# sxyu/volrend

Measured on AMD Instinct MI355X. Metric: Mrays/s at 800x800, NeRF-synthetic-like SH16 (synthetic C1), higher is better.
Workload: dtype f32; 1 GPU; C1: synthetic lego-like PlenOctree, depth 9, SH16, 2025715 nodes, 2.24 GB in HBM, 800x800, fx=fy=1111.111, 200-pose orbit, default RenderOptions; fp_mode=strict, launches=38, pcie_inclusive=False, launch_streams=1, parallelism=single GPU

## Files before the change

include/volrend_hip.h:

```cpp
#ifndef VOLREND_HIP_H_
#define VOLREND_HIP_H_

#include <stddef.h>
#include <stdint.h>

#ifdef __cplusplus
extern "C" {
#endif

#define VR_ABI_VERSION 3

enum {
    VR_OK = 0,
    VR_ERR_INVALID_ARGUMENT = 1,
    VR_ERR_HIP = 2,
    VR_ERR_NO_DEVICE = 3,
    VR_ERR_BAD_TREE = 4,
    VR_ERR_UNSUPPORTED = 5,
    VR_ERR_OUT_OF_MEMORY = 6
};

enum { VR_FORMAT_RGBA = 0, VR_FORMAT_SH = 1, VR_FORMAT_SG = 2, VR_FORMAT_ASG = 3 };

enum { VR_FP_STRICT = 0, VR_FP_FMA = 1 };

#define VR_MAX_BASIS 25

typedef struct VrTreeOpaque* vr_tree_t;

typedef struct VrTreeDesc {
    const int32_t* child;
    const uint16_t* data;
    const float* extra;
    uint64_t extra_count;
    float offset[3];
    float scale[3];
    int32_t N;
    int64_t capacity;
    int32_t data_dim;
    int32_t format;
    int32_t basis_dim;
    float ndc_width;
    float ndc_height;
    float ndc_focal;
    int32_t memory;
} VrTreeDesc;

typedef struct VrQuantDesc {
    const uint16_t* quant_colors;
    const uint16_t* quant_map;
    const uint16_t* sigma;
    const uint16_t* data_retained;
    int32_t n_quant;
    int32_t n_retained;
} VrQuantDesc;

typedef struct VrTreeInfo {
    int64_t capacity;
    int32_t N, data_dim, format, basis_dim;
    int32_t max_depth;
    int32_t device;
    uint64_t device_bytes;
    uint64_t leaf_stride;
    int32_t query_mode;
    int32_t top_levels;
    int32_t brick_levels;
    int32_t brick_blocked;
} VrTreeInfo;

#define VR_QUERY_LOOKUP 0
#define VR_QUERY_DESCENT 1
int vr_query_mode_for(int N, int max_depth, int64_t capacity);

typedef struct VrCamera {
    float transform[12];
    int32_t width, height;
    float fx, fy;
} VrCamera;

typedef struct VrRenderOptions {
    float step_size;
    float sigma_thresh;
    float stop_thresh;
    float background_brightness;
    float render_bbox[6];
    int32_t basis_minmax[2];
    float rot_dirs[3];
    int32_t show_grid;
    int32_t grid_max_depth;
    int32_t render_depth;
    int32_t enable_probe;
    float probe[3];
    int32_t probe_disp_size;
} VrRenderOptions;

enum { VR_LAYOUT_FRAME = 0, VR_LAYOUT_COMPACT = 1 };

typedef struct VrFrame {
    void* rgba;
    int64_t pitch;
    const float* depth;
    float* accum;
    int32_t offscreen;
    int32_t layout;
    int32_t tile_w, tile_h;
    int32_t rank, world;
    int32_t fp_mode;
    int32_t reserved;
    uint64_t* counters;
} VrFrame;

typedef struct VrCounters {
    uint64_t rays, rays_hit_box, samples, child_reads, hit_samples, alg_bytes, early_stops;
} VrCounters;

int vr_abi_version(void);
const char* vr_last_error(void);
int vr_device_count(int* count);
int vr_set_device(int device);
int vr_device_name(int device, char* name, size_t name_len);

void vr_default_tree_desc(VrTreeDesc* desc);
int vr_tree_upload(const VrTreeDesc* desc, vr_tree_t* out);
int vr_tree_upload_quantized(const VrTreeDesc* desc, const VrQuantDesc* quant, vr_tree_t* out);
int vr_decode_quantized(const VrTreeDesc* desc, const VrQuantDesc* quant, uint16_t* data_out);
int vr_tree_clone(vr_tree_t src, int device, vr_tree_t* out);
int vr_tree_free(vr_tree_t tree);
int vr_tree_info(vr_tree_t tree, VrTreeInfo* info);
enum { VR_DATA_F16 = 0, VR_DATA_F32 = 1 };
int vr_tree_update_data(vr_tree_t tree, const void* data_dev, int dtype, void* stream);
int vr_tree_read_data(vr_tree_t tree, void* data_dev, int dtype, void* stream);
enum { VR_STEP_SGD = 0, VR_STEP_ADAM = 1 };
typedef struct VrStep {
    float*    master;
    float*    grad;
    uint32_t* touched;
    float*    m;
    float*    v;
    int32_t   kind;
    float     lr, lr_sigma;
    float     beta1, beta2, eps;
    int32_t   step;
} VrStep;
int vr_tree_step(vr_tree_t tree, const VrStep* s, void* stream);
enum { VR_REFINE_COPY = 0, VR_REFINE_ZERO = 1 };
#define VR_REFINE_MAX_ARRAYS 8
typedef struct VrRefineArray {
    const void* src;
    void*       dst;
    int32_t elem_bytes;
    int32_t dim;
    int32_t fill;
    int32_t reserved;
} VrRefineArray;
typedef struct VrRefine {
    const int32_t*  child;
    const uint32_t* sel;
    int32_t* child_out;
    int32_t* src_slot;
    const VrRefineArray* arrays;
    void*   workspace;
    int64_t workspace_bytes;
    int64_t capacity;
    int64_t n_new;
    int32_t N;
    int32_t n_arrays;
} VrRefine;
int64_t vr_refine_workspace(int N, int64_t capacity);
int vr_refine_plan(const VrRefine* r, int64_t* n_new, void* stream);
int vr_refine_apply(const VrRefine* r, void* stream);

void vr_default_options(VrRenderOptions* opt);
void vr_default_frame(VrFrame* frame);
int64_t vr_compact_bytes(int width, int height, int tile_w, int tile_h, int world);
int vr_render(vr_tree_t tree, const VrCamera* cam, const VrRenderOptions* opt,
              const VrFrame* frame, void* stream);
#define VR_MAX_BATCH 512
int vr_render_batch(vr_tree_t tree, int n_frames, const VrCamera* cams,
                    const VrRenderOptions* opt, const VrFrame* frames, void* stream);
enum { VR_DEPTH_TREE = 0, VR_DEPTH_WORLD = 1 };
typedef struct VrAov {
    float*  depth;
    float*  transmittance;
    int64_t pitch;
} VrAov;
int vr_render_aov(vr_tree_t tree, int n_frames, const VrCamera* cams, const VrRenderOptions* opt,
                  const VrFrame* frames, const VrAov* aovs, int depth_units, void* stream);
typedef struct VrLeafWeights {
    float*    max_weight;
    uint32_t* hits;
} VrLeafWeights;
int vr_accumulate_weights(vr_tree_t tree, int n_frames, const VrCamera* cams,
                          const VrRenderOptions* opt, int fp_mode, const VrLeafWeights* out, void* stream);
int vr_render_backward(vr_tree_t tree, int n_frames, const VrCamera* cams, const VrRenderOptions* opt,
                       int fp_mode, const float* grad_accum, float* grad_data, void* stream);
typedef struct VrRays {
    const float* origins;
    const float* dirs;
} VrRays;
typedef struct VrRayOut {
    void*  rgba;
    float* accum;
} VrRayOut;
int vr_render_rays(vr_tree_t tree, int64_t n, const VrRays* rays, const VrRenderOptions* opt, int fp_mode,
                   const VrRayOut* out, void* stream);
int vr_accumulate_weights_rays(vr_tree_t tree, int64_t n, const VrRays* rays, const VrRenderOptions* opt,
                               int fp_mode, const VrLeafWeights* out, void* stream);
int vr_render_backward_rays(vr_tree_t tree, int64_t n, const VrRays* rays, const VrRenderOptions* opt,
                            int fp_mode, const float* grad_accum, float* grad_data, void* stream);
int vr_render_backward_touched(vr_tree_t tree, int n_frames, const VrCamera* cams, const VrRenderOptions* opt,
                               int fp_mode, const float* grad_accum, float* grad_data, uint32_t* touched,
                               void* stream);
int vr_render_backward_rays_touched(vr_tree_t tree, int64_t n, const VrRays* rays, const VrRenderOptions* opt,
                                    int fp_mode, const float* grad_accum, float* grad_data, uint32_t* touched,
                                    void* stream);
typedef struct VrFit {
    const float* target;
    float        grad_scale;
    float*       grad_data;
    uint32_t*    touched;
    float*       sq_err;
    float*       accum;
} VrFit;
int vr_fit_rays(vr_tree_t tree, int64_t n, const VrRays* rays, const VrRenderOptions* opt,
                int fp_mode, const VrFit* fit, void* stream);
typedef struct VrRayOrder {
    int          bits;
    uint32_t*    order;
    uint32_t*    keys;
    float*       origins_out;
    float*       dirs_out;
    const float* payload;
    float*       payload_out;
    int          payload_dim;
} VrRayOrder;
int64_t vr_order_rays_workspace(int64_t n);
int vr_order_rays(vr_tree_t tree, int64_t n, const VrRays* rays, const VrRenderOptions* opt, int fp_mode,
                  const VrRayOrder* out, void* workspace, size_t workspace_bytes, void* stream);
int vr_reserve_rays(vr_tree_t tree, int64_t n, int n_slots);
int vr_reserve(vr_tree_t tree, int width, int height, int n_frames);
int vr_reserve_tiles(vr_tree_t tree, int width, int height, int n_frames, int tile_w, int tile_h,
                     int world, int n_slots);
int vr_tree_status(vr_tree_t tree, uint32_t* status, int reset);
int vr_tree_status_on(vr_tree_t tree, uint32_t* status, int reset, void* stream);
int vr_set_tuning(const char* key, int value);
int vr_tree_set_tuning(vr_tree_t tree, const char* key, int value);
int vr_sched_stats(vr_tree_t tree, uint64_t out[8], int reset);
int vr_tree_cull_stats(vr_tree_t tree, uint64_t out[2], int reset);
int vr_touch_enable(vr_tree_t tree, int enable);
int vr_touch_count(vr_tree_t tree, uint64_t out[4], int reset);
int vr_touch_read(vr_tree_t tree, int which, uint32_t* host_words, uint64_t n_words,
                  uint64_t* bitmap_words, uint64_t* granule_bytes);
int vr_assemble_tiles(void* frame_rgba, int64_t pitch, const void* gathered, int width,
                      int height, int tile_w, int tile_h, int world, void* stream);
int vr_assemble_tiles_batch(void* frames_rgba, int64_t frame_stride, int64_t pitch,
                            const void* gathered, int64_t rank_stride, int64_t in_frame_stride,
                            int n_frames, int width, int height, int tile_w, int tile_h, int world,
                            void* stream);
int vr_probe_coeffs(vr_tree_t tree, const VrRenderOptions* opt, float* out_dev, void* stream);

enum { VR_SPACE_WORLD = 0, VR_SPACE_TREE = 1 };

typedef struct VrQueryOut {
    float* sigma;
    int32_t* depth;
    float* local;
    float* coeffs;
    float* rgb;
} VrQueryOut;

int vr_query_points(vr_tree_t tree, int64_t n, const float* xyz_dev, const float* dirs_dev, int space,
                    const VrQueryOut* out, void* stream);
int vr_query_grid(vr_tree_t tree, const float lo[3], const float hi[3], const int32_t res[3],
                  const float dir[3], int space, const VrQueryOut* out, void* stream);

int vr_read_back(void* host_rgba, const void* dev_rgba, int64_t pitch, int width, int height,
                 void* stream);
int vr_stream_sync(void* stream);

#ifdef __cplusplus
}
#endif
#endif
```

volrend_amd/_abi.py:

```python
from __future__ import annotations

import ctypes as C
import os

HERE = os.path.dirname(os.path.abspath(__file__))
LIB_PATH = os.environ.get("VOLREND_HIP_LIB") or os.path.join(HERE, "libvolrend_hip.so")

VR_OK = 0
FORMAT_RGBA, FORMAT_SH, FORMAT_SG, FORMAT_ASG = 0, 1, 2, 3
FORMATS = {"RGBA": FORMAT_RGBA, "SH": FORMAT_SH, "SG": FORMAT_SG, "ASG": FORMAT_ASG}
FP_STRICT, FP_FMA = 0, 1
QUERY_LOOKUP, QUERY_DESCENT = 0, 1
LAYOUT_FRAME, LAYOUT_COMPACT = 0, 1
SPACE_WORLD, SPACE_TREE = 0, 1
SPACES = {"world": SPACE_WORLD, "tree": SPACE_TREE}
DEPTH_TREE, DEPTH_WORLD = 0, 1
DEPTH_UNITS = {"tree": DEPTH_TREE, "world": DEPTH_WORLD}
DATA_F16, DATA_F32 = 0, 1
STEP_SGD, STEP_ADAM = 0, 1
STEP_KINDS = {"sgd": STEP_SGD, "adam": STEP_ADAM}
MAX_BASIS = 25
ORDER_MAX_BITS, ORDER_MAX_PAYLOAD = 5, 8
REFINE_COPY, REFINE_ZERO = 0, 1
REFINE_FILLS = {"copy": REFINE_COPY, "zero": REFINE_ZERO}
REFINE_MAX_ARRAYS = 8


class VrTreeDesc(C.Structure):
    _fields_ = [("child", C.c_void_p), ("data", C.c_void_p), ("extra", C.c_void_p),
                ("extra_count", C.c_uint64), ("offset", C.c_float * 3), ("scale", C.c_float * 3),
                ("N", C.c_int32), ("capacity", C.c_int64), ("data_dim", C.c_int32),
                ("format", C.c_int32), ("basis_dim", C.c_int32), ("ndc_width", C.c_float),
                ("ndc_height", C.c_float), ("ndc_focal", C.c_float), ("memory", C.c_int32)]


class VrQuantDesc(C.Structure):
    _fields_ = [("quant_colors", C.c_void_p), ("quant_map", C.c_void_p), ("sigma", C.c_void_p),
                ("data_retained", C.c_void_p), ("n_quant", C.c_int32), ("n_retained", C.c_int32)]


class VrTreeInfo(C.Structure):
    _fields_ = [("capacity", C.c_int64), ("N", C.c_int32), ("data_dim", C.c_int32),
                ("format", C.c_int32), ("basis_dim", C.c_int32), ("max_depth", C.c_int32),
                ("device", C.c_int32), ("device_bytes", C.c_uint64), ("leaf_stride", C.c_uint64),
                ("query_mode", C.c_int32), ("top_levels", C.c_int32), ("brick_levels", C.c_int32),
                ("brick_blocked", C.c_int32)]


class VrCamera(C.Structure):
    _fields_ = [("transform", C.c_float * 12), ("width", C.c_int32), ("height", C.c_int32),
                ("fx", C.c_float), ("fy", C.c_float)]


class VrRenderOptions(C.Structure):
    _fields_ = [("step_size", C.c_float), ("sigma_thresh", C.c_float), ("stop_thresh", C.c_float),
                ("background_brightness", C.c_float), ("render_bbox", C.c_float * 6),
                ("basis_minmax", C.c_int32 * 2), ("rot_dirs", C.c_float * 3),
                ("show_grid", C.c_int32), ("grid_max_depth", C.c_int32),
                ("render_depth", C.c_int32), ("enable_probe", C.c_int32),
                ("probe", C.c_float * 3), ("probe_disp_size", C.c_int32)]


class VrFrame(C.Structure):
    _fields_ = [("rgba", C.c_void_p), ("pitch", C.c_int64), ("depth", C.c_void_p),
                ("accum", C.c_void_p), ("offscreen", C.c_int32), ("layout", C.c_int32),
                ("tile_w", C.c_int32), ("tile_h", C.c_int32), ("rank", C.c_int32),
                ("world", C.c_int32), ("fp_mode", C.c_int32), ("reserved", C.c_int32),
                ("counters", C.c_void_p)]


class VrAov(C.Structure):
    _fields_ = [("depth", C.c_void_p), ("transmittance", C.c_void_p), ("pitch", C.c_int64)]


class VrLeafWeights(C.Structure):
    _fields_ = [("max_weight", C.c_void_p), ("hits", C.c_void_p)]


class VrRays(C.Structure):
    _fields_ = [("origins", C.c_void_p), ("dirs", C.c_void_p)]


class VrRayOut(C.Structure):
    _fields_ = [("rgba", C.c_void_p), ("accum", C.c_void_p)]


class VrFit(C.Structure):
    _fields_ = [("target", C.c_void_p), ("grad_scale", C.c_float), ("grad_data", C.c_void_p),
                ("touched", C.c_void_p), ("sq_err", C.c_void_p), ("accum", C.c_void_p)]


class VrRayOrder(C.Structure):
    _fields_ = [("bits", C.c_int), ("order", C.c_void_p), ("keys", C.c_void_p), ("origins_out", C.c_void_p),
                ("dirs_out", C.c_void_p), ("payload", C.c_void_p), ("payload_out", C.c_void_p),
                ("payload_dim", C.c_int)]


class VrStep(C.Structure):
    _fields_ = [("master", C.c_void_p), ("grad", C.c_void_p), ("touched", C.c_void_p), ("m", C.c_void_p),
                ("v", C.c_void_p), ("kind", C.c_int32), ("lr", C.c_float), ("lr_sigma", C.c_float),
                ("beta1", C.c_float), ("beta2", C.c_float), ("eps", C.c_float), ("step", C.c_int32)]


class VrRefineArray(C.Structure):
    _fields_ = [("src", C.c_void_p), ("dst", C.c_void_p), ("elem_bytes", C.c_int32), ("dim", C.c_int32),
                ("fill", C.c_int32), ("reserved", C.c_int32)]


class VrRefine(C.Structure):
    _fields_ = [("child", C.c_void_p), ("sel", C.c_void_p), ("child_out", C.c_void_p), ("src_slot", C.c_void_p),
                ("arrays", C.POINTER(VrRefineArray)), ("workspace", C.c_void_p), ("workspace_bytes", C.c_int64),
                ("capacity", C.c_int64), ("n_new", C.c_int64), ("N", C.c_int32), ("n_arrays", C.c_int32)]


class VrQueryOut(C.Structure):
    _fields_ = [("sigma", C.c_void_p), ("depth", C.c_void_p), ("local", C.c_void_p),
                ("coeffs", C.c_void_p), ("rgb", C.c_void_p)]


ABI_VERSION = 3
MAX_BATCH = 512

COUNTER_FIELDS = ("rays", "rays_hit_box", "samples", "child_reads", "hit_samples", "alg_bytes",
                  "early_stops")


PROTOTYPES = {
    "vr_abi_version": (C.c_int, []),
    "vr_last_error": (C.c_char_p, []),
    "vr_device_count": (C.c_int, [C.POINTER(C.c_int)]),
    "vr_set_device": (C.c_int, [C.c_int]),
    "vr_device_name": (C.c_int, [C.c_int, C.c_char_p, C.c_size_t]),
    "vr_default_tree_desc": (None, [C.POINTER(VrTreeDesc)]),
    "vr_tree_upload": (C.c_int, [C.POINTER(VrTreeDesc), C.POINTER(C.c_void_p)]),
    "vr_tree_upload_quantized": (C.c_int, [C.POINTER(VrTreeDesc), C.POINTER(VrQuantDesc),
                                           C.POINTER(C.c_void_p)]),
    "vr_decode_quantized": (C.c_int, [C.POINTER(VrTreeDesc), C.POINTER(VrQuantDesc), C.c_void_p]),
    "vr_tree_clone": (C.c_int, [C.c_void_p, C.c_int, C.POINTER(C.c_void_p)]),
    "vr_tree_free": (C.c_int, [C.c_void_p]),
    "vr_tree_info": (C.c_int, [C.c_void_p, C.POINTER(VrTreeInfo)]),
    "vr_tree_update_data": (C.c_int, [C.c_void_p, C.c_void_p, C.c_int, C.c_void_p]),
    "vr_tree_read_data": (C.c_int, [C.c_void_p, C.c_void_p, C.c_int, C.c_void_p]),
    "vr_query_mode_for": (C.c_int, [C.c_int, C.c_int, C.c_int64]),
    "vr_default_options": (None, [C.POINTER(VrRenderOptions)]),
    "vr_default_frame": (None, [C.POINTER(VrFrame)]),
    "vr_compact_bytes": (C.c_int64, [C.c_int, C.c_int, C.c_int, C.c_int, C.c_int]),
    "vr_render": (C.c_int, [C.c_void_p, C.POINTER(VrCamera), C.POINTER(VrRenderOptions),
                            C.POINTER(VrFrame), C.c_void_p]),
    "vr_render_batch": (C.c_int, [C.c_void_p, C.c_int, C.POINTER(VrCamera),
                                  C.POINTER(VrRenderOptions), C.POINTER(VrFrame), C.c_void_p]),
    "vr_render_aov": (C.c_int, [C.c_void_p, C.c_int, C.POINTER(VrCamera), C.POINTER(VrRenderOptions),
                                C.POINTER(VrFrame), C.POINTER(VrAov), C.c_int, C.c_void_p]),
    "vr_accumulate_weights": (C.c_int, [C.c_void_p, C.c_int, C.POINTER(VrCamera), C.POINTER(VrRenderOptions),
                                        C.c_int, C.POINTER(VrLeafWeights), C.c_void_p]),
    "vr_render_backward": (C.c_int, [C.c_void_p, C.c_int, C.POINTER(VrCamera), C.POINTER(VrRenderOptions),
                                     C.c_int, C.c_void_p, C.c_void_p, C.c_void_p]),
    "vr_render_backward_touched": (C.c_int, [C.c_void_p, C.c_int, C.POINTER(VrCamera), C.POINTER(VrRenderOptions),
                                             C.c_int, C.c_void_p, C.c_void_p, C.c_void_p, C.c_void_p]),
    "vr_render_backward_rays_touched": (C.c_int, [C.c_void_p, C.c_int64, C.POINTER(VrRays), C.POINTER(VrRenderOptions),
                                                  C.c_int, C.c_void_p, C.c_void_p, C.c_void_p, C.c_void_p]),
    "vr_tree_step": (C.c_int, [C.c_void_p, C.POINTER(VrStep), C.c_void_p]),
    "vr_refine_workspace": (C.c_int64, [C.c_int, C.c_int64]),
    "vr_refine_plan": (C.c_int, [C.POINTER(VrRefine), C.POINTER(C.c_int64), C.c_void_p]),
    "vr_refine_apply": (C.c_int, [C.POINTER(VrRefine), C.c_void_p]),
    "vr_render_rays": (C.c_int, [C.c_void_p, C.c_int64, C.POINTER(VrRays), C.POINTER(VrRenderOptions), C.c_int,
                                 C.POINTER(VrRayOut), C.c_void_p]),
    "vr_accumulate_weights_rays": (C.c_int, [C.c_void_p, C.c_int64, C.POINTER(VrRays), C.POINTER(VrRenderOptions),
                                             C.c_int, C.POINTER(VrLeafWeights), C.c_void_p]),
    "vr_render_backward_rays": (C.c_int, [C.c_void_p, C.c_int64, C.POINTER(VrRays), C.POINTER(VrRenderOptions),
                                          C.c_int, C.c_void_p, C.c_void_p, C.c_void_p]),
    "vr_fit_rays": (C.c_int, [C.c_void_p, C.c_int64, C.POINTER(VrRays), C.POINTER(VrRenderOptions), C.c_int,
                              C.POINTER(VrFit), C.c_void_p]),
    "vr_order_rays_workspace": (C.c_int64, [C.c_int64]),
    "vr_order_rays": (C.c_int, [C.c_void_p, C.c_int64, C.POINTER(VrRays), C.POINTER(VrRenderOptions), C.c_int,
                                C.POINTER(VrRayOrder), C.c_void_p, C.c_size_t, C.c_void_p]),
    "vr_reserve_rays": (C.c_int, [C.c_void_p, C.c_int64, C.c_int]),
    "vr_reserve": (C.c_int, [C.c_void_p, C.c_int, C.c_int, C.c_int]),
    "vr_reserve_tiles": (C.c_int, [C.c_void_p, C.c_int, C.c_int, C.c_int, C.c_int, C.c_int, C.c_int,
                                   C.c_int]),
    "vr_tree_status": (C.c_int, [C.c_void_p, C.POINTER(C.c_uint32), C.c_int]),
    "vr_tree_status_on": (C.c_int, [C.c_void_p, C.POINTER(C.c_uint32), C.c_int, C.c_void_p]),
    "vr_set_tuning": (C.c_int, [C.c_char_p, C.c_int]),
    "vr_tree_set_tuning": (C.c_int, [C.c_void_p, C.c_char_p, C.c_int]),
    "vr_sched_stats": (C.c_int, [C.c_void_p, C.POINTER(C.c_uint64 * 8), C.c_int]),
    "vr_tree_cull_stats": (C.c_int, [C.c_void_p, C.POINTER(C.c_uint64 * 2), C.c_int]),
    "vr_touch_enable": (C.c_int, [C.c_void_p, C.c_int]),
    "vr_touch_count": (C.c_int, [C.c_void_p, C.POINTER(C.c_uint64 * 4), C.c_int]),
    "vr_touch_read": (C.c_int, [C.c_void_p, C.c_int, C.c_void_p, C.c_uint64, C.POINTER(C.c_uint64),
                                C.POINTER(C.c_uint64)]),
    "vr_assemble_tiles": (C.c_int, [C.c_void_p, C.c_int64, C.c_void_p, C.c_int, C.c_int, C.c_int,
                                    C.c_int, C.c_int, C.c_void_p]),
    "vr_assemble_tiles_batch": (C.c_int, [C.c_void_p, C.c_int64, C.c_int64, C.c_void_p, C.c_int64,
                                          C.c_int64, C.c_int, C.c_int, C.c_int, C.c_int, C.c_int,
                                          C.c_int, C.c_void_p]),
    "vr_probe_coeffs": (C.c_int, [C.c_void_p, C.POINTER(VrRenderOptions), C.c_void_p, C.c_void_p]),
    "vr_query_points": (C.c_int, [C.c_void_p, C.c_int64, C.c_void_p, C.c_void_p, C.c_int,
                                  C.POINTER(VrQueryOut), C.c_void_p]),
    "vr_query_grid": (C.c_int, [C.c_void_p, C.POINTER(C.c_float * 3), C.POINTER(C.c_float * 3),
                                C.POINTER(C.c_int32 * 3), C.POINTER(C.c_float * 3), C.c_int,
                                C.POINTER(VrQueryOut), C.c_void_p]),
    "vr_read_back": (C.c_int, [C.c_void_p, C.c_void_p, C.c_int64, C.c_int, C.c_int, C.c_void_p]),
    "vr_stream_sync": (C.c_int, [C.c_void_p]),
}

_lib = None


class VolrendError(RuntimeError):
    def __init__(self, code: int, msg: str):
        super().__init__(f"volrend_hip error {code}: {msg}")
        self.code = code


def lib():
    global _lib
    if _lib is None:
        if not os.path.exists(LIB_PATH):
            raise RuntimeError(
                f"{LIB_PATH} not found: the HIP library is mandatory (no CPU fallback). "
                "Build it with `python -m volrend_amd.build`.")
        L = C.CDLL(LIB_PATH)
        for name, (res, args) in PROTOTYPES.items():
            fn = getattr(L, name)
            fn.restype = res
            fn.argtypes = args
        if L.vr_abi_version() != ABI_VERSION:
            raise RuntimeError("libvolrend_hip.so ABI version mismatch")
        _lib = L
    return _lib


def check(rc: int) -> None:
    if rc != VR_OK:
        raise VolrendError(rc, (lib().vr_last_error() or b"").decode("utf-8", "replace"))
```

volrend_amd/_tree.py:

```python
from __future__ import annotations

import ctypes as C
import os

import numpy as np

from . import _abi, _ops
from ._args import F16, I32, Buf, _stream_ptr, check


class _CurrentDevice:

    def info(self) -> dict:
        import torch
        return {"device": int(torch.cuda.current_device())}


def parse_data_format(s: str):
    idx = next((i for i, ch in enumerate(s) if not ch.isalpha()), -1)
    if idx < 0:
        return "RGBA", -1
    head = s[:idx]
    try:
        dim = int("".join(ch for ch in s[idx:] if ch.isdigit() or ch == "-") or "0")
    except ValueError:
        dim = 0
    return (head if head in ("ASG", "SG", "SH") else "RGBA"), dim


class N3Tree:

    def __init__(self, path: str | None = None, upload: bool = True):
        self.N = 0
        self.data_dim = 0
        self.data_format = ("RGBA", -1)
        self.capacity = 0
        self.scale = np.zeros(3, np.float32)
        self.offset = np.zeros(3, np.float32)
        self.use_ndc = False
        self.ndc_width = self.ndc_height = self.ndc_focal = 0.0
        self.child_ = None
        self.data_ = None
        self.extra_ = None
        self.quant_ = None
        self._handle = C.c_void_p()
        self._loaded = False
        if path is not None:
            self.open(path, upload=upload)

    @classmethod
    def from_arrays(cls, child, data, offset, invradius3, data_format: str, extra=None,
                    ndc=None, upload: bool = True) -> "N3Tree":
        t = cls()
        t._set_arrays(child, data, offset, invradius3, data_format, extra)
        if ndc:
            t.use_ndc = True
            t.ndc_width, t.ndc_height, t.ndc_focal = map(float, ndc)
        if upload:
            t.load_device()
        return t

    @classmethod
    def from_synth(cls, tree, upload: bool = True, ndc=None) -> "N3Tree":
        return cls.from_arrays(tree.child, tree.data, tree.offset, tree.invradius3,
                               tree.data_format, tree.extra, ndc=ndc, upload=upload)

    def _set_arrays(self, child, data, offset, invradius3, data_format, extra, data_dim=None):
        child = np.ascontiguousarray(child, dtype=np.int32)
        if child.ndim != 4 or not (child.shape[1] == child.shape[2] == child.shape[3]):
            raise RuntimeError("child must be int32 [capacity, N, N, N]")
        self.N = int(child.shape[1])
        self.capacity = int(child.shape[0])
        self.child_ = child.reshape(self.capacity, self.N, self.N, self.N)
        self.quant_ = None
        if data is None:
            self.data_ = None
            self.data_dim = int(data_dim)
        else:
            data = np.asarray(data)
            if data.dtype != np.float16:
                raise RuntimeError("data must be stored in half precision")
            self.data_ = np.ascontiguousarray(data)
            self.data_dim = int(self.data_.shape[-1])
            if self.data_.size != self.capacity * self.N ** 3 * self.data_dim:
                raise RuntimeError("data does not have capacity * N^3 * data_dim values")
        self.data_format = parse_data_format(data_format)
        self.scale = np.asarray(invradius3, dtype=np.float32).reshape(3).copy()
        self.offset = np.asarray(offset, dtype=np.float32).reshape(3).copy()
        self.extra_ = None if extra is None else np.ascontiguousarray(extra, dtype=np.float32)

    def open(self, path: str, upload: bool = True, device_decode: bool = True) -> None:
        if not path.endswith(".npz"):
            raise ValueError("tree file must end in .npz")
        if not os.path.exists(path):
            raise FileNotFoundError(f"Can't load because file does not exist: {path}")
        z = np.load(path)
        data_dim = int(z["data_dim"])
        if "data_format" in z.files:
            fmt = str(z["data_format"])
        else:
            fmt = "RGBA" if data_dim == 4 else f"SH{(data_dim - 1) // 3}"
        if "invradius3" in z.files:
            scale = z["invradius3"].astype(np.float32)
        else:
            scale = np.full(3, float(z["invradius"]), dtype=np.float32)
        child = z["child"]
        extra = z["extra_data"] if "extra_data" in z.files else None
        if "quant_colors" in z.files and upload and device_decode:
            self._set_arrays(child, None, z["offset"], scale, fmt, extra, data_dim=data_dim)
            self.quant_ = _quant_arrays(z, child)
        else:
            if "quant_colors" in z.files:
                data = _decode_quantised(z, child, data_dim)
            else:
                data = z["data"]
            self._set_arrays(child, data, z["offset"], scale, fmt, extra)
            if self.data_dim != data_dim:
                raise RuntimeError("data_dim does not match the data array")
        pb = path[:-4] + "_poses_bounds.npy"
        if os.path.exists(pb):
            arr = np.load(pb).reshape(-1)
            self.use_ndc = True
            self.ndc_height, self.ndc_width, self.ndc_focal = float(arr[4]), float(arr[9]), float(
                arr[14])
        if upload:
            self.load_device()

    @classmethod
    def from_device_arrays(cls, child_dev, data_dev, offset, invradius3, data_format: str, extra=None,
                           ndc=None) -> "N3Tree":
        shape = tuple(getattr(child_dev, "shape", ()))
        if len(shape) != 4 or not (shape[1] == shape[2] == shape[3]):
            raise ValueError("child_dev must be an int32 tensor [capacity, N, N, N]")
        dshape = tuple(getattr(data_dev, "shape", ()))
        if len(dshape) != 5 or dshape[:4] != shape or dshape[4] < 1:
            raise ValueError(f"data_dev must be a float16 tensor [capacity, N, N, N, data_dim] over {shape}, not {dshape}")
        c = check(_CurrentDevice(), [Buf("child_dev", child_dev, (I32,), shape), Buf("data_dev", data_dev, (F16,), dshape)])
        t = cls()
        t.capacity, t.N, t.data_dim = int(shape[0]), int(shape[1]), int(dshape[4])
        t.child_ = child_dev.cpu().numpy().reshape(shape)
        t.data_format = parse_data_format(data_format) if isinstance(data_format, str) else tuple(data_format)
        t.scale = np.asarray(invradius3, dtype=np.float32).reshape(3).copy()
        t.offset = np.asarray(offset, dtype=np.float32).reshape(3).copy()
        t.extra_ = None if extra is None else np.ascontiguousarray(extra, dtype=np.float32)
        if ndc:
            t.use_ndc = True
            t.ndc_width, t.ndc_height, t.ndc_focal = map(float, ndc)
        t._upload(c.ptr["child_dev"], c.ptr["data_dev"], memory=1)
        return t

    def load_device(self) -> None:
        self.free_device()
        if self.data_ is None and self.quant_ is None:
            raise RuntimeError("tree has no data (clear_cpu_memory was called)")
        self._upload(self.child_.ctypes.data, None if self.data_ is None else self.data_.ctypes.data, memory=0)

    def _upload(self, child_ptr, data_ptr, memory: int) -> None:
        L = _abi.lib()
        self.free_device()
        d = _abi.VrTreeDesc()
        L.vr_default_tree_desc(C.byref(d))
        d.child = child_ptr
        if data_ptr is not None:
            d.data = data_ptr
        if self.extra_ is not None:
            d.extra = self.extra_.ctypes.data
            d.extra_count = self.extra_.size
        for i in range(3):
            d.offset[i] = float(self.offset[i])
            d.scale[i] = float(self.scale[i])
        d.N = self.N
        d.capacity = self.capacity
        d.data_dim = self.data_dim
        d.format = _abi.FORMATS[self.data_format[0]]
        d.basis_dim = self.data_format[1]
        d.ndc_width = self.ndc_width if self.use_ndc else -1.0
        d.ndc_height = self.ndc_height
        d.ndc_focal = self.ndc_focal
        d.memory = memory
        h = C.c_void_p()
        if data_ptr is None:
            _abi.check(L.vr_tree_upload_quantized(C.byref(d), C.byref(self._quant_desc()),
                                                  C.byref(h)))
        else:
            _abi.check(L.vr_tree_upload(C.byref(d), C.byref(h)))
        self._handle = h
        self._loaded = True

    def _quant_desc(self) -> "_abi.VrQuantDesc":
        q = _abi.VrQuantDesc()
        a = self.quant_
        q.n_quant = a["quant_map"].shape[0]
        q.quant_colors = a["quant_colors"].ctypes.data
        q.quant_map = a["quant_map"].ctypes.data
        q.sigma = a["sigma"].ctypes.data
        if a["data_retained"] is not None:
            q.n_retained = a["data_retained"].shape[0]
            q.data_retained = a["data_retained"].ctypes.data
        return q

    def decode_host(self, on_device: bool = False) -> np.ndarray:
        if self.data_ is None and self.quant_ is not None:
            shape = (self.capacity, self.N, self.N, self.N, self.data_dim)
            if on_device:
                d = _abi.VrTreeDesc()
                _abi.lib().vr_default_tree_desc(C.byref(d))
                d.N, d.capacity, d.data_dim, d.memory = self.N, self.capacity, self.data_dim, 0
                out = np.empty(shape, np.float16)
                _abi.check(_abi.lib().vr_decode_quantized(C.byref(d), C.byref(self._quant_desc()),
                                                          out.ctypes.data))
                self.data_ = out
            else:
                a = self.quant_
                self.data_ = _decode_arrays(a["quant_colors"], a["quant_map"], a["sigma"],
                                            a["data_retained"], self.data_dim).reshape(shape)
        return self.data_

    def clone_to(self, device: int) -> "N3Tree":
        t = N3Tree()
        for k in ("N", "data_dim", "data_format", "capacity", "scale", "offset", "use_ndc",
                  "ndc_width", "ndc_height", "ndc_focal", "child_"):
            setattr(t, k, getattr(self, k))
        h = C.c_void_p()
        _abi.check(_abi.lib().vr_tree_clone(self.handle, int(device), C.byref(h)))
        t._handle = h
        t._loaded = True
        return t

    def free_device(self) -> None:
        if self._handle:
            _abi.lib().vr_tree_free(self._handle)
            self._handle = C.c_void_p()
        self._loaded = False

    def is_device_loaded(self) -> bool:
        return self._loaded

    def clear_cpu_memory(self) -> None:
        self.data_ = None
        self.quant_ = None

    def sched_stats(self, reset: bool = True) -> dict:
        out = (C.c_uint64 * 8)()
        _abi.check(_abi.lib().vr_sched_stats(self._handle, C.byref(out), 1 if reset else 0))
        names = ("march_rounds", "march_lanes", "shade_rounds", "shade_lanes", "distinct_leaves",
                 "retire_rounds", "retired", "iterations")
        return dict(zip(names, [int(v) for v in out]))

    def cull_stats(self, reset: bool = True) -> dict:
        out = (C.c_uint64 * 2)()
        _abi.check(_abi.lib().vr_tree_cull_stats(self.handle, C.byref(out), 1 if reset else 0))
        return {"blocks": int(out[0]), "culled": int(out[1])}

    def touch_enable(self, enable: bool = True) -> None:
        _abi.check(_abi.lib().vr_touch_enable(self.handle, 1 if enable else 0))

    def touch_count(self, reset: bool = True) -> dict:
        out = (C.c_uint64 * 4)()
        _abi.check(_abi.lib().vr_touch_count(self.handle, C.byref(out), 1 if reset else 0))
        return dict(zip(("leaves", "nodes", "top", "bricks"), [int(v) for v in out]))

    def touch_read(self, which: int):
        words, gran = C.c_uint64(0), C.c_uint64(0)
        _abi.check(_abi.lib().vr_touch_read(self.handle, int(which), None, 0, C.byref(words), C.byref(gran)))
        out = np.zeros(int(words.value), dtype=np.uint32)
        if out.size:
            _abi.check(_abi.lib().vr_touch_read(self.handle, int(which), out.ctypes.data, out.size, None, None))
        return out, int(gran.value)

    def reserve(self, width: int, height: int, n_frames: int, shard: "TileShard | None" = None,
                n_slots: int = 2) -> None:
        if shard is None and n_slots == 2:
            _abi.check(_abi.lib().vr_reserve(self.handle, int(width), int(height), int(n_frames)))
        else:
            tw, th, world = (shard.tile_w, shard.tile_h, shard.world) if shard else (0, 0, 1)
            _abi.check(_abi.lib().vr_reserve_tiles(self.handle, int(width), int(height),
                                                   int(n_frames), tw, th, world, int(n_slots)))

    def set_tuning(self, **kw) -> None:
        for k, v in kw.items():
            _abi.check(_abi.lib().vr_tree_set_tuning(self.handle, k.encode(), int(v)))

    def status(self, reset: bool = False, stream=None) -> int:
        out = C.c_uint32(0)
        if stream is not None:
            _abi.check(_abi.lib().vr_tree_status_on(self.handle, C.byref(out), 1 if reset else 0,
                                                    _stream_ptr(stream)))
        else:
            _abi.check(_abi.lib().vr_tree_status(self.handle, C.byref(out), 1 if reset else 0))
        return int(out.value)

    def reserve_rays(self, n: int, n_slots: int = 2) -> None:
        _abi.check(_abi.lib().vr_reserve_rays(self.handle, int(n), int(n_slots)))

    query, query_grid = _ops.query_points, _ops.query_grid
    accumulate_weights, render_backward = _ops.accumulate_weights, _ops.render_backward
    render_rays, accumulate_weights_rays = _ops.render_rays, _ops.accumulate_weights_rays
    render_backward_rays, touched_words = _ops.render_backward_rays, _ops.touched_words
    fit_rays, order_rays = _ops.fit_rays, _ops.order_rays
    step, update_data, read_data = _ops.tree_step, _ops.update_data, _ops.read_data
    refine = _ops.refine

    def info(self) -> dict:
        i = _abi.VrTreeInfo()
        _abi.check(_abi.lib().vr_tree_info(self._handle, C.byref(i)))
        return {n: int(getattr(i, n)) for n, _ in i._fields_}

    @property
    def handle(self):
        if not self._loaded:
            raise RuntimeError("tree is not on the device (call load_device)")
        return self._handle

    def __del__(self):
        try:
            self.free_device()
        except Exception:
            pass


def _quant_arrays(z, child) -> dict:
    qc = z["quant_colors"]
    if qc.dtype != np.float16:
        raise RuntimeError("codebook must be stored in half precision")
    qm = z["quant_map"]
    n_q = qm.shape[0]
    if qc.shape[0] != n_q:
        raise RuntimeError("codebook and map basis numbers does not match")
    cap, N = qm.shape[1], child.shape[1]
    if cap != child.shape[0] or qc.shape[1:] != (65536, 3):
        raise RuntimeError("quantised arrays do not match the tree")
    n_slots = cap * N * N * N
    retained = z["data_retained"] if "data_retained" in z.files else None
    return dict(
        quant_colors=np.ascontiguousarray(qc),
        quant_map=np.ascontiguousarray(qm.reshape(n_q, n_slots), dtype=np.uint16),
        sigma=np.ascontiguousarray(z["sigma"].reshape(n_slots), dtype=np.float16),
        data_retained=None if retained is None else np.ascontiguousarray(
            retained.reshape(retained.shape[0], n_slots, 3), dtype=np.float16))


def _decode_arrays(qc, qm, sigma, retained, data_dim: int) -> np.ndarray:
    n_q, n_slots = qm.shape
    n_ret = 0 if retained is None else retained.shape[0]
    n_basis = n_q + n_ret
    data = np.zeros((n_slots, data_dim), dtype=np.float16)
    for j in range(n_q):
        cols = qc[j][qm[j].astype(np.int64)]
        for c in range(3):
            data[:, j + n_ret + c * n_basis] = cols[:, c]
    data[:, data_dim - 1] = sigma
    for j in range(n_ret):
        for c in range(3):
            data[:, j + c * n_basis] = retained[j, :, c]
    return data


def _decode_quantised(z, child, data_dim: int) -> np.ndarray:
    a = _quant_arrays(z, child)
    cap, N = child.shape[0], child.shape[1]
    return _decode_arrays(a["quant_colors"], a["quant_map"], a["sigma"], a["data_retained"],
                          data_dim).reshape(cap, N, N, N, data_dim)
```

volrend_amd/csrc/vr_api.cpp:

```cpp
#include <hip/hip_runtime.h>

#include <climits>
#include <cstdarg>
#include <cstdio>
#include <cstdlib>
#include <cstring>
#include <mutex>

#include "vr_host.h"
#include "vr_tree_walk.h"

namespace {

thread_local char g_err[512] = "";

enum KnobRange { kClamp, kClamp64, kFlag, kAutoFlag };
struct Knob { const char *key, *env; int Tuning::*field; KnobRange range; int lo, hi; bool fixed_at_upload; };
const Knob kKnobs[] = {
    {"march_max", "VR_MARCH_MAX", &Tuning::march_max, kClamp, 1, INT_MAX, false},
    {"refill_min", "VR_REFILL_MIN", &Tuning::refill_min, kClamp, 1, 64, false},
    {"drain_flush", "VR_DRAIN_FLUSH", &Tuning::drain_flush, kClamp, 0, 64, false},
    {"waves_per_cu", "VR_WAVES_PER_CU", &Tuning::waves_per_cu, kClamp, 0, 64, false},
    {"frame_group", "VR_FRAME_GROUP", &Tuning::frame_group, kClamp, 0, INT_MAX, false},
    {"super_block", "VR_SUPER_BLOCK", &Tuning::super_block, kClamp, 0, 64, false},
    {"records_nt", "VR_RECORDS_NT", &Tuning::records_nt, kAutoFlag, 0, 0, false},
    {"xcd_queues", "VR_XCD_QUEUES", &Tuning::xcd_queues, kFlag, 0, 0, false},
    {"chunk_max", "VR_CHUNK_MAX", &Tuning::chunk_max, kClamp64, 0, INT_MAX, false},
    {"raygen_waves", "VR_RAYGEN_WAVES", &Tuning::raygen_waves, kClamp, 0, INT_MAX, false},
    {"top_levels", "VR_TOP_LEVELS", &Tuning::top_levels, kClamp, INT_MIN, INT_MAX, true},
    {"brick_levels", "VR_BRICK_LEVELS", &Tuning::brick_levels, kClamp, INT_MIN, INT_MAX, true},
    {"brick_blocked", "VR_BRICK_BLOCKED", &Tuning::brick_blocked, kAutoFlag, 0, 0, true},
    {"max_iter", "VR_MAX_ITER", &Tuning::max_iter, kClamp, 1, INT_MAX, false},
    {"weights_check", "VR_WEIGHTS_CHECK", &Tuning::weights_check, kFlag, 0, 0, false},
    {"block_cull", "VR_BLOCK_CULL", &Tuning::block_cull, kFlag, 0, 0, false},
};

const Knob* find_knob(const char* key) {
    for (const Knob& k : kKnobs)
        if (!strcmp(key, k.key)) return &k;
    return nullptr;
}

void set_knob(Tuning& tn, const Knob& k, int v) {
    const int clamped = v < k.lo ? k.lo : (v > k.hi ? k.hi : v);
    tn.*k.field = k.range == kFlag       ? v != 0
                  : k.range == kAutoFlag ? (v < 0 ? -1 : v != 0)
                  : k.range == kClamp64  ? (clamped > 0 && clamped < 64 ? 64 : clamped & ~63)
                                         : clamped;
}

std::mutex g_tuning_mutex;
Tuning& default_tuning_locked() {
    static Tuning tn = [] {
        Tuning x;
        for (const Knob& k : kKnobs)
            if (const char* e = getenv(k.env)) set_knob(x, k, atoi(e));
        return x;
    }();
    return tn;
}

uint64_t touch_granule(int which) {
    return which == 0 ? (1ull << vr::kTouchLeafShift) : 128ull;
}
size_t touch_words(uint64_t array_bytes, int which) {
    const uint64_t g = touch_granule(which);
    return (size_t)(((array_bytes + g - 1) / g + 31) / 32);
}

}

int fail(int code, const char* fmt, ...) {
    va_list ap;
    va_start(ap, fmt);
    vsnprintf(g_err, sizeof(g_err), fmt, ap);
    va_end(ap);
    return code;
}

Tuning default_tuning() {
    std::lock_guard<std::mutex> g(g_tuning_mutex);
    return default_tuning_locked();
}

extern "C" {

int vr_abi_version(void) { return VR_ABI_VERSION; }

const char* vr_last_error(void) { return g_err; }

int vr_device_count(int* count) {
    if (!count) return fail(VR_ERR_INVALID_ARGUMENT, "count is NULL");
    int n = 0;
    hipError_t e = hipGetDeviceCount(&n);
    if (e != hipSuccess) {
        *count = 0;
        return fail(VR_ERR_NO_DEVICE, "hipGetDeviceCount: %s", hipGetErrorString(e));
    }
    *count = n;
    return VR_OK;
}

int vr_set_device(int device) {
    if (device < 0) return VR_OK;
    HIP_TRY(hipSetDevice(device));
    return VR_OK;
}

int vr_device_name(int device, char* name, size_t name_len) {
    if (!name || name_len == 0) return fail(VR_ERR_INVALID_ARGUMENT, "name buffer is NULL");
    hipDeviceProp_t prop;
    if (device < 0) HIP_TRY(hipGetDevice(&device));
    HIP_TRY(hipGetDeviceProperties(&prop, device));
    snprintf(name, name_len, "%s", prop.gcnArchName);
    return VR_OK;
}

void vr_default_tree_desc(VrTreeDesc* d) {
    if (!d) return;
    memset(d, 0, sizeof(*d));
    d->N = 2;
    d->format = VR_FORMAT_RGBA;
    d->basis_dim = -1;
    d->ndc_width = -1.f;
}

int vr_tree_info(vr_tree_t t, VrTreeInfo* info) {
    if (!t || !info) return fail(VR_ERR_INVALID_ARGUMENT, "tree/info is NULL");
    info->capacity = t->desc.capacity;
    info->N = t->desc.N;
    info->data_dim = t->desc.data_dim;
    info->format = t->desc.format;
    info->basis_dim = t->desc.basis_dim;
    info->max_depth = t->max_depth;
    info->device = t->device;
    info->device_bytes = t->device_bytes;
    info->leaf_stride = (uint64_t)t->leaf_stride_h * 2u;
    info->query_mode = t->top_levels > 0 ? VR_QUERY_LOOKUP : VR_QUERY_DESCENT;
    info->top_levels = t->top_levels;
    info->brick_levels = t->brick_levels;
    info->brick_blocked = t->brick_blocked;
    return VR_OK;
}

int vr_query_mode_for(int N, int max_depth, int64_t capacity) {
    return lookup_applies(N, max_depth, capacity) ? VR_QUERY_LOOKUP : VR_QUERY_DESCENT;
}

void vr_default_options(VrRenderOptions* o) {
    if (!o) return;
    memset(o, 0, sizeof(*o));
    o->step_size = 1e-4f;
    o->sigma_thresh = 1e-2f;
    o->stop_thresh = 1e-2f;
    o->background_brightness = 1.f;
    o->render_bbox[3] = o->render_bbox[4] = o->render_bbox[5] = 1.f;
    o->basis_minmax[0] = 0;
    o->basis_minmax[1] = VR_MAX_BASIS - 1;
    o->grid_max_depth = 4;
    o->probe[2] = 1.f;
    o->probe_disp_size = 100;
}

void vr_default_frame(VrFrame* f) {
    if (!f) return;
    memset(f, 0, sizeof(*f));
    f->offscreen = 1;
    f->layout = VR_LAYOUT_FRAME;
    f->world = 1;
    f->fp_mode = VR_FP_STRICT;
}

int64_t vr_compact_bytes(int width, int height, int tile_w, int tile_h, int world) {
    vr::KParams g;
    if (tile_geometry(width, height, tile_w, tile_h, 0, world, g) != VR_OK) return -1;
    return (int64_t)g.n_local_tiles * g.tile_w * g.tile_h * 4;
}

int vr_set_tuning(const char* key, int value) {
    if (!key) return fail(VR_ERR_INVALID_ARGUMENT, "key is NULL");
    const Knob* k = find_knob(key);
    if (!k) return fail(VR_ERR_INVALID_ARGUMENT, "unknown tuning key '%s'", key);
    std::lock_guard<std::mutex> g(g_tuning_mutex);
    set_knob(default_tuning_locked(), *k, value);
    return VR_OK;
}

int vr_tree_set_tuning(vr_tree_t t, const char* key, int value) {
    if (!t || !key) return fail(VR_ERR_INVALID_ARGUMENT, "tree/key is NULL");
    const Knob* k = find_knob(key);
    if (!k) return fail(VR_ERR_INVALID_ARGUMENT, "unknown tuning key '%s'", key);
    if (k->fixed_at_upload)
        return fail(VR_ERR_INVALID_ARGUMENT, "'%s' is fixed at upload (vr_set_tuning before it)", key);
    std::lock_guard<std::mutex> g(t->launch_mutex);
    set_knob(t->tn, *k, value);
    return VR_OK;
}

int vr_sched_stats(vr_tree_t t, uint64_t out[vr::kSchedStats], int reset) {
    if (!t || !out) return fail(VR_ERR_INVALID_ARGUMENT, "NULL argument");
    DeviceGuard guard(t->device);
    HIP_TRY(hipMemcpy(out, t->sched_stats.get(), vr::kSchedStats * sizeof(uint64_t), hipMemcpyDeviceToHost));
    if (reset) HIP_TRY(hipMemset(t->sched_stats.get(), 0, vr::kSchedStats * sizeof(uint64_t)));
    return VR_OK;
}

int vr_tree_cull_stats(vr_tree_t t, uint64_t out[2], int reset) {
    if (!t || !out) return fail(VR_ERR_INVALID_ARGUMENT, "NULL argument");
    DeviceGuard guard(t->device);
    uint64_t lines[vr::kCullStatLines * vr::kCullStatStride];
    HIP_TRY(hipMemcpy(lines, t->cull_stats.get(), sizeof(lines), hipMemcpyDeviceToHost));
    if (reset) HIP_TRY(hipMemset(t->cull_stats.get(), 0, sizeof(lines)));
    out[0] = out[1] = 0;
    for (int i = 0; i < vr::kCullStatLines; ++i) {
        out[0] += lines[i * vr::kCullStatStride];
        out[1] += lines[i * vr::kCullStatStride + 1];
    }
    return VR_OK;
}

int vr_tree_status(vr_tree_t t, uint32_t* status, int reset) {
    if (!t || !status) return fail(VR_ERR_INVALID_ARGUMENT, "NULL argument");
    DeviceGuard guard(t->device);
    HIP_TRY(hipMemcpy(status, t->status.get(), sizeof(uint32_t), hipMemcpyDeviceToHost));
    if (reset) HIP_TRY(hipMemset(t->status.get(), 0, sizeof(uint32_t)));
    return VR_OK;
}

int vr_tree_status_on(vr_tree_t t, uint32_t* status, int reset, void* stream) {
    if (!t || !status) return fail(VR_ERR_INVALID_ARGUMENT, "NULL argument");
    DeviceGuard guard(t->device);
    hipStream_t hs = static_cast<hipStream_t>(stream);
    thread_local uint32_t* pinned = nullptr;
    if (!pinned) HIP_TRY(hipHostMalloc((void**)&pinned, sizeof(uint32_t), hipHostMallocPortable));
    HIP_TRY(hipMemcpyAsync(pinned, t->status.get(), sizeof(uint32_t), hipMemcpyDeviceToHost, hs));
    if (reset) HIP_TRY(hipMemsetAsync(t->status.get(), 0, sizeof(uint32_t), hs));
    HIP_TRY(hipStreamSynchronize(hs));
    *status = *pinned;
    return VR_OK;
}

int vr_touch_enable(vr_tree_t t, int enable) {
    if (!t) return fail(VR_ERR_INVALID_ARGUMENT, "tree is NULL");
    DeviceGuard guard(t->device);
    std::lock_guard<std::mutex> lock(t->launch_mutex);
    HIP_TRY(hipDeviceSynchronize());
    for (int i = 0; i < 4; ++i) {
        HIP_TRY(t->touch[i].reset());
        const size_t words = touch_words(t->arrays[i].bytes(), i);
        if (enable && words) {
            HIP_TRY(t->touch[i].alloc(words * sizeof(uint32_t)));
            HIP_TRY(hipMemset(t->touch[i].get(), 0, words * sizeof(uint32_t)));
        }
    }
    if (enable && !t->touch_out) HIP_TRY(t->touch_out.alloc(4 * sizeof(unsigned long long)));
    return VR_OK;
}

int vr_touch_count(vr_tree_t t, uint64_t out[4], int reset) {
    if (!t || !out) return fail(VR_ERR_INVALID_ARGUMENT, "NULL argument");
    if (!t->touch_out) return fail(VR_ERR_INVALID_ARGUMENT, "vr_touch_enable(tree, 1) first");
    DeviceGuard guard(t->device);
    std::lock_guard<std::mutex> lock(t->launch_mutex);
    HIP_TRY(hipDeviceSynchronize());
    HIP_TRY(hipMemset(t->touch_out.get(), 0, 4 * sizeof(unsigned long long)));
    for (int i = 0; i < 4; ++i) {
        if (!t->touch[i]) continue;
        const size_t words = touch_words(t->arrays[i].bytes(), i);
        HIP_TRY(vr::launch_popcount(t->touch[i].get<uint32_t>(), words,
                                    t->touch_out.get<unsigned long long>() + i, nullptr));
        if (reset) HIP_TRY(hipMemsetAsync(t->touch[i].get(), 0, words * sizeof(uint32_t), nullptr));
    }
    HIP_TRY(hipMemcpy(out, t->touch_out.get(), 4 * sizeof(uint64_t), hipMemcpyDeviceToHost));
    return VR_OK;
}

int vr_touch_read(vr_tree_t t, int which, uint32_t* host_words, uint64_t n_words,
                  uint64_t* bitmap_words, uint64_t* granule_bytes) {
    if (!t || which < 0 || which > 3) return fail(VR_ERR_INVALID_ARGUMENT, "tree / array index");
    if (!t->touch_out) return fail(VR_ERR_INVALID_ARGUMENT, "vr_touch_enable(tree, 1) first");
    DeviceGuard guard(t->device);
    std::lock_guard<std::mutex> lock(t->launch_mutex);
    const uint64_t words = t->touch[which] ? touch_words(t->arrays[which].bytes(), which) : 0;
    if (bitmap_words) *bitmap_words = words;
    if (granule_bytes) *granule_bytes = touch_granule(which);
    const uint64_t n = n_words < words ? n_words : words;
    if (host_words && n) {
        HIP_TRY(hipDeviceSynchronize());
        HIP_TRY(hipMemcpy(host_words, t->touch[which].get(), n * sizeof(uint32_t), hipMemcpyDeviceToHost));
    }
    return VR_OK;
}

int vr_assemble_tiles(void* frame_rgba, int64_t pitch, const void* gathered, int width, int height,
                      int tile_w, int tile_h, int world, void* stream) {
    if (world < 1) world = 1;
    const int64_t rank_bytes = vr_compact_bytes(width, height, tile_w, tile_h, world);
    if (rank_bytes < 0) return VR_ERR_INVALID_ARGUMENT;
    return vr_assemble_tiles_batch(frame_rgba, 0, pitch, gathered, rank_bytes, 0, 1, width, height,
                                   tile_w, tile_h, world, stream);
}

int vr_assemble_tiles_batch(void* frames_rgba, int64_t frame_stride, int64_t pitch,
                            const void* gathered, int64_t rank_stride, int64_t in_frame_stride,
                            int n_frames, int width, int height, int tile_w, int tile_h, int world,
                            void* stream) {
    if (!frames_rgba || !gathered) return fail(VR_ERR_INVALID_ARGUMENT, "NULL buffer");
    if (n_frames < 1) return fail(VR_ERR_INVALID_ARGUMENT, "n_frames must be positive");
    if (world < 1) world = 1;
    vr::KParams g;
    if (int rc = tile_geometry(width, height, tile_w, tile_h, 0, world, g)) return rc;
    HIP_TRY(vr::launch_assemble(static_cast<uint8_t*>(frames_rgba),
                                pitch ? pitch : (int64_t)width * 4,
                                static_cast<const uint8_t*>(gathered), width, height, g.tile_w, g.tile_h, world,
                                n_frames, frame_stride, rank_stride, in_frame_stride,
                                static_cast<hipStream_t>(stream)));
    return VR_OK;
}

int vr_probe_coeffs(vr_tree_t t, const VrRenderOptions* opt, float* out_dev, void* stream) {
    if (!t || !opt || !out_dev) return fail(VR_ERR_INVALID_ARGUMENT, "NULL argument");
    DeviceGuard guard(t->device);
    vr::KParams k;
    memset(&k, 0, sizeof(k));
    fill_tree_params(k, t);
    HIP_TRY(vr::launch_probe(k, opt->probe, out_dev, static_cast<hipStream_t>(stream)));
    return VR_OK;
}

int vr_read_back(void* host_rgba, const void* dev_rgba, int64_t pitch, int width, int height,
                 void* stream) {
    if (!host_rgba || !dev_rgba) return fail(VR_ERR_INVALID_ARGUMENT, "NULL buffer");
    if (pitch == 0) pitch = (int64_t)width * 4;
    HIP_TRY(hipMemcpy2DAsync(host_rgba, (size_t)width * 4, dev_rgba, (size_t)pitch,
                             (size_t)width * 4, (size_t)height, hipMemcpyDeviceToHost,
                             static_cast<hipStream_t>(stream)));
    return VR_OK;
}

int vr_stream_sync(void* stream) {
    HIP_TRY(hipStreamSynchronize(static_cast<hipStream_t>(stream)));
    return VR_OK;
}

}
```

volrend_amd/csrc/vr_dev_march.h:

```cpp
#pragma once
#include <type_traits>
#include "vr_device_math.h"
#include "vr_internal.h"
#include "vr_dev_layout.h"
#include "vr_dev_query.h"
#include "vr_dev_rays.h"

namespace vr {

namespace {

enum { kQueryN2 = 0, kQueryN2Blocked = 1, kQueryGeneric = 2 };
inline int query_kind(const KParams& p) {
    return !uses_lookup(p) ? kQueryGeneric : (p.brick_blocked ? kQueryN2Blocked : kQueryN2);
}
template <typename F>
void dispatch_query(int query, F&& f) {
    if (query == kQueryGeneric) f(std::integral_constant<int, kQueryGeneric>());
    else if (query == kQueryN2Blocked) f(std::integral_constant<int, kQueryN2Blocked>());
    else f(std::integral_constant<int, kQueryN2>());
}

struct WeightRecord {
    static constexpr int kWords = kWeightRayWords;
    static constexpr bool kShade = false;
};
struct GradRecord {
    static constexpr int kWords = kGradRayWords;
    static constexpr bool kShade = true;
};

template <int GW, typename Record>
__device__ __forceinline__ void store_march_record(const KParams& p, bool valid, int lane, int wave, const Ray& nr,
                                                   const float* vdir, uint32_t pixel) {
    const unsigned long long m_valid = __builtin_amdgcn_ballot_w64(valid);
    const uint32_t my_base = reserve_ray_slots<GW>(p, m_valid, lane, wave);
    if (!valid) return;
    uint32_t* rb = ray_slot(p.ray_buf_rw, Record::kWords, my_base + lane_rank(m_valid));
    store_march_words(rb, nr);
    if constexpr (Record::kShade) {
#pragma unroll
        for (int i = 0; i < 3; ++i) ray_word(rb, kGradRayVdir + i) = f2u(vdir[i]);
        ray_word(rb, kGradRayPixel) = pixel;
    }
}

template <int FMA, int GW, typename Record>
__global__ __launch_bounds__(kWave* GW) void march_raygen_kernel(const KParams p) {
    const int lane = threadIdx.x & (kWave - 1);
    const int wave = threadIdx.x >> 6;
    const uint32_t id = (uint32_t)(((int64_t)blockIdx.x * GW + wave) * kWave + lane);
    bool valid = false;
    Ray nr;
    nr.alive = false;
    float vdir[3] = {0.f, 0.f, 0.f};
    uint32_t pixel = 0;
    if (id < p.total_rays) {
        const PixelRef r = locate(p, id);
        if (r.in_image) {
            setup_ray<FMA>(p, r, nr, vdir);
            valid = nr.alive;
            pixel = ((uint32_t)r.frame * (uint32_t)p.height + (uint32_t)r.y) * (uint32_t)p.width + (uint32_t)r.x;
        }
    }
    store_march_record<GW, Record>(p, valid, lane, wave, nr, vdir, pixel);
}

template <int FMA, int GW, typename Record>
__global__ __launch_bounds__(kWave* GW) void march_raygen_rays_kernel(const KParams p, const RayList rl) {
    const int lane = threadIdx.x & (kWave - 1);
    const int wave = threadIdx.x >> 6;
    uint32_t id;
    Ray nr;
    float vdir[3] = {0.f, 0.f, 0.f};
    const bool valid = list_ray<FMA, GW>(p, rl, lane, wave, id, nr, vdir) && nr.alive;
    store_march_record<GW, Record>(p, valid, lane, wave, nr, vdir, id);
}

template <typename Launch>
void launch_raygen_waves(const KParams& p, int gen_waves, Launch&& launch) {
    const int gw = gen_waves >= 16 ? 16 : 4;
    const dim3 grid((unsigned)((p.n_wave_blocks * p.n_frames + gw - 1) / gw)), block(kWave * gw);
    if (gw == 16) launch(std::integral_constant<int, 16>(), grid, block);
    else launch(std::integral_constant<int, 4>(), grid, block);
}
template <int FMA, typename Record>
void launch_march_raygen(const KParams& p, int gen_waves, hipStream_t s, const RayList* rays) {
    launch_raygen_waves(p, gen_waves, [&](auto gw, dim3 grid, dim3 block) {
        constexpr int GW = decltype(gw)::value;
        if (rays) hipLaunchKernelGGL((march_raygen_rays_kernel<FMA, GW, Record>), grid, block, 0, s, p, *rays);
        else hipLaunchKernelGGL((march_raygen_kernel<FMA, GW, Record>), grid, block, 0, s, p);
    });
}

struct MarchFeed {
    bool exhausted;
    uint32_t chunk_next, chunk_end;
    uint32_t progress_round;
};
template <typename Load, typename Reset>
__device__ __forceinline__ MarchFeed march_refill(const KParams& p, int lane, int ray_words, uint32_t rounds,
                                                  MarchFeed feed, bool& active, float* cen, float* dir, float* invdir,
                                                  float& t, float& tmax, float& delta_scale, float& light, Cursor& cur,
                                                  Load&& load, Reset&& reset) {
    const bool done = active && !(t < tmax);
    const unsigned long long m_done = __builtin_amdgcn_ballot_w64(done);
    const unsigned long long m_busy = __builtin_amdgcn_ballot_w64(t < tmax);
    const int n_avail = kWave - __builtin_popcountll(m_busy);
    if (!(n_avail > 0 && (m_busy == 0ull || (!feed.exhausted && n_avail >= p.refill_min)))) return feed;
    if (m_done != 0ull) feed.progress_round = (uint32_t)__builtin_amdgcn_readfirstlane((int)rounds);
    if (!feed.exhausted && feed.chunk_next >= feed.chunk_end) {
        uint32_t lo, hi;
        grab_chunk(p, lane, lo, hi);
        lo = __builtin_amdgcn_readfirstlane(lo);
        hi = __builtin_amdgcn_readfirstlane(hi);
        if (hi == lo) {
            feed.exhausted = true;
        } else {
            feed.chunk_next = lo;
            feed.chunk_end = hi;
        }
    }
    const bool vacant = !(t < tmax);
    bool take = false;
    if (!feed.exhausted) {
        const uint32_t r = feed.chunk_next + lane_rank(~m_busy);
        const uint32_t c_end = feed.chunk_end;
        const uint32_t left = feed.chunk_end - feed.chunk_next;
        feed.chunk_next += (uint32_t)n_avail < left ? (uint32_t)n_avail : left;
        if (vacant && r < c_end) {
            take = true;
            const uint32_t* rs = ray_slot(p.ray_buf, ray_words, r);
#pragma unroll
            for (int i = 0; i < 3; ++i) {
                cen[i] = u2f(ray_word(rs, kRayCen + i));
                dir[i] = u2f(ray_word(rs, kRayDir + i));
                invdir[i] = u2f(ray_word(rs, kRayInvDir + i));
            }
            t = u2f(ray_word(rs, kRayT));
            tmax = u2f(ray_word(rs, kRayTmax));
            delta_scale = u2f(ray_word(rs, kRayDeltaScale));
            load(rs, r);
        }
    }
    if (vacant) {
        active = take;
        if (!take) {
            t = 0.f;
            tmax = -1.f;
        }
        light = 1.f;
        cur = Cursor();
        reset();
    }
    return feed;
}

__device__ __forceinline__ bool sample_guard(const KParams& p, uint32_t rounds, uint32_t& progress_round, float& t,
                                             float tmax) {
    if (rounds - progress_round < (uint32_t)p.max_iter) return false;
    progress_round = rounds;
    if (!(t < tmax)) return false;
    t = tmax;
    if (p.status) atomicOr(p.status, 1u);
    return true;
}

template <int FMA, int QUERY>
__device__ __forceinline__ uint32_t march_sample(const KParams& p, float t, const float* cen, const float* dir,
                                                 const float* invdir, Cursor& cur, float& delta_t, float& sigma) {
    using P = Policy<FMA>;
    constexpr bool N2 = QUERY != kQueryGeneric;
    float pos[3];
    pos[0] = P::madd(t, dir[0], cen[0]);
    pos[1] = P::madd(t, dir[1], cen[1]);
    pos[2] = P::madd(t, dir[2], cen[2]);
    float cube_sz = 0.f;
    int levels;
    uint32_t word, leaf;
    if (N2) leaf = query_n2<false, (QUERY == kQueryN2Blocked ? 1 : 0)>(p, pos, &levels, &word, cur);
    else leaf = (uint32_t)query_generic<FMA, false>(p, pos, &cube_sz, &levels, &word);
    const float dda = dda_unit<FMA>(pos, invdir);
    const float t_subcube = N2 ? __builtin_amdgcn_ldexpf(dda, -levels) : dda / cube_sz;
    delta_t = t_subcube + p.step_size;
    sigma = h2f((uint16_t)(word & 0xFFFFu));
    return leaf;
}

__device__ __forceinline__ float sample_weight(float light, float delta_t, float delta_scale, float sigma, float& att) {
    att = vr_expf_nonan(-delta_t * delta_scale * sigma);
    return light * (1.f - att);
}

template <bool N2>
__device__ __forceinline__ uint32_t file_node_index(const KParams& p, uint32_t leaf) {
    return N2 ? (leaf >> 3) : leaf / (uint32_t)p.N3;
}
template <bool N2>
__device__ __forceinline__ uint32_t file_slot(const KParams& p, uint32_t node, uint32_t leaf) {
    return N2 ? ((node << 3) | (leaf & 7u)) : node * (uint32_t)p.N3 + leaf % (uint32_t)p.N3;
}

}

}
```

volrend_amd/csrc/vr_host.h:

```cpp
#pragma once
#include <hip/hip_runtime.h>

#include <mutex>
#include <vector>

#include "vr_internal.h"
#include "vr_launch_plan.h"

#pragma GCC visibility push(hidden)

#include "volrend/internal/hip_owners.hpp"
using volrend::internal::DeviceBuffer;
using volrend::internal::DeviceEvent;
using volrend::internal::DeviceGuard;

int fail(int code, const char* fmt, ...);
inline int hip_code(hipError_t e) { return e == hipErrorOutOfMemory ? VR_ERR_OUT_OF_MEMORY : VR_ERR_HIP; }

#define HIP_TRY(expr)                                                                                 \
    do {                                                                                              \
        hipError_t e_ = (expr);                                                                       \
        if (e_ != hipSuccess)                                                                         \
            return fail(hip_code(e_), "%s failed: %s (%s:%d)", #expr, hipGetErrorString(e_), __FILE__, \
                        __LINE__);                                                                    \
    } while (0)

Tuning default_tuning();

constexpr unsigned kLaunchSlots = 8;

struct LaunchSlot {
    DeviceEvent done;
    bool used = false;
    hipStream_t last_stream = nullptr;
    bool growing = false;
    DeviceBuffer rays;
};

enum TreeArray { kLeaves = 0, kNodes = 1, kTop = 2, kBricks = 3 };

struct TreeShape {
    VrTreeDesc desc{};
    int32_t max_depth = 0;
    int leaf_stride_h = 0;
    int top_levels = 0, brick_levels = 0, n_bricks = 0;
    int brick_blocked = 0;
    int occ_levels = -1;
    uint64_t device_bytes = 0;
};

struct VrTreeOpaque : TreeShape {
    int device = 0;
    DeviceBuffer arrays[4];
    DeviceBuffer extra, status, sched_stats;
    DeviceBuffer occ;
    DeviceBuffer cull_stats;
    DeviceBuffer touch[4];
    DeviceBuffer touch_out;
    DeviceBuffer probe_buf;
    DeviceBuffer slot_frames;
    DeviceBuffer slot_heads;
    DeviceBuffer slot_aovs;
    std::vector<int32_t> file_node;
    DeviceBuffer file_node_dev;
    std::vector<int32_t> brick_root;
    DeviceBuffer brick_root_dev;
    DeviceBuffer node_of_file_dev;
    LaunchSlot slots[kLaunchSlots];
    unsigned launch_seq = 0;
    std::mutex launch_mutex;
    Tuning tn;
    int n_cus = 256;
};

void fill_tree_params(vr::KParams& k, const VrTreeOpaque* t);

int tile_geometry(int width, int height, int tile_w, int tile_h, int rank, int world, vr::KParams& k);
int launch_geometry(int width, int height, int tile_w, int tile_h, int rank, int world, int n_frames,
                    vr::KParams& k);
int list_geometry(const char* what, int64_t n, vr::KParams& k);

inline size_t ray_buffer_bytes(uint32_t total_rays, int words_per_ray) {
    return vr::ray_slots(total_rays) * (size_t)words_per_ray * sizeof(uint32_t);
}
inline size_t list_pixel_bytes(uint32_t total_rays) { return (size_t)total_rays * 4; }
inline uint32_t block_mask_words(const vr::KParams& k) {
    const uint64_t blocks = (uint64_t)k.tiles_x * (uint64_t)(k.tile_w / 8) * (uint64_t)k.tiles_y * (uint64_t)(k.tile_h / 8);
    return (uint32_t)(((blocks + 127) / 128) * 4);
}
inline size_t block_mask_bytes(const vr::KParams& k, int n_frames) {
    return (size_t)block_mask_words(k) * sizeof(uint32_t) * (size_t)n_frames;
}
hipError_t refresh_occupancy(const VrTreeOpaque* t, hipStream_t hs);

int acquire_slot(VrTreeOpaque* t, std::unique_lock<std::mutex>& guard, hipStream_t hs, vr::KParams& k,
                 size_t need, unsigned& slot);

class SlotTurn {
    LaunchSlot* slot_ = nullptr;
    hipStream_t stream_ = nullptr;
public:
    int begin(LaunchSlot& ls, hipStream_t hs);
    ~SlotTurn();
};

int ensure_device_table(VrTreeOpaque* t, DeviceBuffer& dev, const std::vector<int32_t>& host, size_t entries,
                        const char* name);
int ensure_file_nodes(VrTreeOpaque* t);

#pragma GCC visibility pop
```

volrend_amd/csrc/vr_internal.h:

```cpp
#pragma once
#include <hip/hip_runtime.h>
#include <stdint.h>

#include "volrend_hip.h"

namespace vr {

constexpr int kMaxBatch = 512;
constexpr int kTableChunk = 48;
constexpr int kTouchLeafShift = 7;

enum { BASIS_RGBA = -1, BASIS_1 = 1, BASIS_4 = 4, BASIS_9 = 9, BASIS_16 = 16, BASIS_25 = 25 };
__host__ __device__ inline int basis_flavour(int format, int basis_dim) {
    if (format == VR_FORMAT_RGBA || basis_dim < 0) return BASIS_RGBA;
    switch (basis_dim) {
        case 25: return BASIS_25;
        case 16: return BASIS_16;
        case 9: return BASIS_9;
        case 4: return BASIS_4;
        default: return BASIS_1;
    }
}
__host__ __device__ inline int basis_words(int flavour) { return flavour == BASIS_RGBA ? 0 : flavour; }
__host__ __device__ inline bool ray_vdir(int format, int flavour) {
    return format == VR_FORMAT_SH && basis_words(flavour) > 3;
}
__host__ __device__ inline int ray_tail_words(int format, int flavour) {
    return ray_vdir(format, flavour) ? 3 : basis_words(flavour);
}

enum {
    kRayCen = 0,
    kRayDir = 3,
    kRayInvDir = 6,
    kRayT = 9,
    kRayTmax = 10,
    kRayDeltaScale = 11,
    kRayXy = 12,
    kRayPixelLo = 13,
    kRayPixelHi = 14,
    kRayFrame = 15,
    kRayWords = 16,
    kRayTail = kRayWords,
};
__host__ __device__ inline uint32_t ray_groups16(uint32_t total_rays) { return ((total_rays >> 6) + 15u) >> 4; }
__host__ __device__ inline size_t ray_slots(uint32_t total_rays) { return (size_t)ray_groups16(total_rays) * 16 * 64; }

constexpr int kMaxQueues = 8;
constexpr int kMaxQueuesShift = 3;
constexpr int kQueueStride = 16;
constexpr int kQueueHead = 0;
constexpr int kQueueCount = 1;
constexpr int kSlotHeaderWords = 16;
constexpr int kSlotWords = 160;
static_assert(kMaxQueues == 1 << kMaxQueuesShift, "queues are picked with shifts and masks");
static_assert(kSlotWords >= kSlotHeaderWords + kMaxQueues * kQueueStride, "a slot holds its header and every queue");

enum {
    kStatMarchRounds = 0,
    kStatMarchLanes,
    kStatShadeRounds,
    kStatShadeLanes,
    kStatDistinctLeaves,
    kStatRetireRounds,
    kStatRetiredRays,
    kStatIterations,
    kSchedStats
};
static_assert(kSchedStats == 8, "vr_sched_stats(out[8]) is public ABI");

struct FrameDesc {
    float xf[12];
    uint8_t* rgba;
    float* accum;
    const float* depth;
    VrCounters* counters;
};

struct FrameTable {
    int32_t first;
    int32_t n;
    FrameDesc f[kTableChunk];
};

struct KParams {
    const uint32_t* nodes;
    const uint16_t* leaves;
    const uint2* top;
    const uint32_t* bricks;
    const float* extra;
    float offset[3];
    float scale[3];
    int32_t N, N3;
    int64_t capacity;
    int32_t data_dim;
    int32_t format;
    int32_t basis_dim;
    int32_t leaf_stride_h;
    int32_t max_depth;
    int32_t top_levels;
    int32_t brick_levels;
    int32_t brick_blocked;
    float ndc_width, ndc_height, ndc_focal;
    int32_t width, height;
    float fx, fy;
    float step_size, sigma_thresh, stop_thresh, background_brightness;
    float bbox[6];
    int32_t basis_min, basis_max;
    int32_t render_depth;
    int32_t enable_probe;
    int32_t probe_disp_size;
    const float* probe_coeffs;
    int32_t rot_enabled;
    float rot_k[3];
    float rot_cos, rot_sin;
    const FrameDesc* frames;
    int32_t n_frames;
    int64_t pitch;
    int32_t offscreen;
    int32_t layout;
    int32_t tile_w, tile_h;
    int32_t tiles_x, tiles_y;
    int32_t rank, world;
    int32_t n_local_tiles;
    int32_t wblocks_per_tile_x;
    int32_t wblocks_per_tile;
    int64_t n_wave_blocks;
    uint32_t total_rays;
    uint32_t* queue_head;
    int32_t n_queues;
    int32_t chunk_max;
    const uint32_t* ray_buf;
    uint32_t* ray_buf_rw;
    int32_t basis_words;
    int32_t ray_tail_words;
    int32_t ray_vdir;
    int32_t refill_min;
    int32_t march_max;
    int32_t drain_flush;
    int32_t max_iter;
    int32_t instrumented;
    int32_t any_accum;
    int32_t records_nt;
    int32_t frame_group;
    int32_t super_block;
    uint32_t* status;
    unsigned long long* sched_stats;
    uint32_t* touch[4];
};

inline bool uses_lookup(const KParams& p) { return p.N == 2 && p.top_levels > 0; }
inline bool needs_full(const KParams& p) {
    return p.format == VR_FORMAT_SG || p.format == VR_FORMAT_ASG || p.instrumented || p.render_depth;
}

inline unsigned persistent_grid(int64_t total_blocks, int n_cus, int waves_per_cu) {
    int64_t want = total_blocks / 2;
    if (want < 256) want = 256;
    if (want > total_blocks) want = total_blocks;
    const int64_t cap = (int64_t)n_cus * waves_per_cu;
    return (unsigned)(want < cap ? want : cap);
}

struct AovDesc {
    float* depth;
    float* transmittance;
};
struct AovParams {
    const AovDesc* planes;
    int64_t pitch;
    int32_t depth_world;
};
struct AovTable {
    int32_t first;
    int32_t n;
    AovDesc f[kTableChunk];
};

constexpr int kOccMaxLevels = 7;
constexpr int kOccHeaderWords = 4;
constexpr int kCullStatLines = 16;
constexpr int kCullStatStride = 8;
constexpr int kMaskMaxWords = 4096;
__host__ __device__ inline size_t occ_bitmap_words(int g) { return g >= 2 ? ((size_t)1 << (3 * g)) / 32 : 1; }
__host__ __device__ inline size_t occ_words(int g) { return kOccHeaderWords + occ_bitmap_words(g) + ((size_t)1 << (3 * g)); }
struct CullParams {
    const uint32_t* mask;
    uint32_t words_per_frame;
    uint32_t nbx;
    unsigned long long* stats;
};
struct MaskParams {
    uint32_t* mask;
    uint32_t words_per_frame, nbx, nby;
    const uint32_t* occ;
    int32_t levels;
    int32_t groups_per_frame;
};
hipError_t launch_block_mask(const KParams& p, const MaskParams& m, hipStream_t stream);
hipError_t launch_build_occupancy(const uint32_t* nodes, int levels, uint32_t* occ, hipStream_t stream);

constexpr int kWeightRayWords = kRayDeltaScale + 1;
static_assert(kWeightRayWords <= kRayWords, "a slot reserved for colour rays holds the weight rays of the same shape");
struct WeightParams {
    uint32_t* max_weight;
    uint32_t* hits;
    const int32_t* file_node;
};

constexpr int kRayListShift = 15;
constexpr int kRayListWidth = 1 << kRayListShift;
struct RayList {
    const float* origins;
    const float* dirs;
    int64_t n;
};
__host__ __device__ inline uint32_t ray_list_slots(int64_t n) { return (uint32_t)(((n + 63) >> 6) << 6); }

hipError_t launch_weights(const KParams& p, const WeightParams& w, int fp_mode, int n_cus, int waves_override,
                          int gen_waves, bool check_first, hipStream_t stream, const RayList* rays = nullptr);

enum {
    kGradRayVdir = kWeightRayWords,
    kGradRayPixel = kGradRayVdir + 3,
    kGradRayWords = kGradRayPixel + 1,
};
static_assert(kGradRayWords <= kRayWords, "a slot reserved for colour rays holds the backward rays of the same shape");
struct GradParams {
    const float* grad_accum;
    float* grad_data;
    const int32_t* file_node;
    uint32_t* touched;
};

hipError_t launch_grad(const KParams& p, const GradParams& g, int fp_mode, int n_cus, int waves_override,
                       int gen_waves, hipStream_t stream, const RayList* rays = nullptr);

struct FitParams {
    const float* target;
    float* grad_data;
    const int32_t* file_node;
    uint32_t* touched;
    float* sq_err;
    float* accum;
    float bg, grad_scale;
};
hipError_t launch_fit(const KParams& p, const FitParams& f, int fp_mode, int n_cus, int waves_override, int gen_waves,
                      hipStream_t stream, const RayList* rays);

struct UpdateArgs {
    uint32_t* nodes;
    uint16_t* leaves;
    const int32_t* file_node;
    void* data;
    int64_t capacity;
    int32_t N3, data_dim;
    int32_t stride_h;
    int32_t f32;
};
hipError_t launch_update_values(const UpdateArgs& a, int n_cus, hipStream_t stream);
hipError_t launch_read_values(const UpdateArgs& a, int n_cus, hipStream_t stream);
hipError_t launch_refresh_lookup(const uint32_t* nodes, const int32_t* brick_root, int n_bricks, uint2* top,
                                 uint32_t* bricks, int top_levels, int brick_levels, hipStream_t stream);

struct StepArgs {
    uint32_t* nodes;
    uint16_t* leaves;
    const int32_t* node_of_file;
    float* master;
    float* grad;
    float* m;
    float* v;
    uint32_t* touched;
    int64_t n_words;
    int64_t n_slots;
    int32_t N3, data_dim;
    int32_t stride_h;
    int32_t adam;
    float lr, lr_sigma;
    float beta1, beta2, omb1, omb2, sbc2, eps;
};
hipError_t launch_step_values(const StepArgs& a, int n_cus, hipStream_t stream);

hipError_t launch_prepare_aov(const AovParams& a, const AovTable& tbl, hipStream_t stream);
hipError_t launch_render_aov(const KParams& p, const AovParams& a, const CullParams& cull, int fp_mode, int n_cus,
                             int waves_override, int gen_waves, hipStream_t stream);
hipError_t launch_prepare(const KParams& p, const FrameTable& tbl, hipStream_t stream, uint32_t* mask = nullptr,
                          uint32_t words_per_frame = 0);
hipError_t launch_render(const KParams& p, const CullParams& cull, int fp_mode, int n_cus, int waves_override,
                         int gen_waves, hipStream_t stream, const RayList* rays = nullptr);
hipError_t launch_probe(const KParams& p, const float probe[3], float* out_dev,
                        hipStream_t stream);

int leaf_stride_halfs(int data_dim);
hipError_t launch_relayout(const int32_t* child, const uint16_t* data, const int32_t* perm,
                           uint32_t* nodes, uint16_t* leaves, int64_t n_slots, int N3,
                           int data_dim, int stride_h, hipStream_t stream);
hipError_t launch_decode_quant(const uint16_t* colors, const uint16_t* map, const uint16_t* sigma,
                               const uint16_t* retained, uint16_t* data, int64_t n_slots,
                               int n_quant, int n_ret, int data_dim, hipStream_t stream);
hipError_t launch_build_lookup(const uint32_t* nodes, const int32_t* brick_root, int n_bricks,
                               uint2* top, uint32_t* bricks, int top_levels, int brick_levels,
                               int brick_blocked, uint32_t* error_flag, hipStream_t stream);
hipError_t launch_popcount(const uint32_t* words, uint64_t n_words, unsigned long long* out,
                           hipStream_t stream);
hipError_t launch_assemble(uint8_t* frame, int64_t pitch, const uint8_t* gathered, int width,
                           int height, int tile_w, int tile_h, int world, int n_frames,
                           int64_t out_stride, int64_t rank_stride, int64_t in_stride,
                           hipStream_t stream);

}
```

volrend_amd/csrc/vr_launch.cpp:

```cpp
#include <hip/hip_runtime.h>

#include <cmath>
#include <cstring>
#include <mutex>

#include "vr_host.h"

static_assert(kPlanQueues == vr::kMaxQueues, "vr_launch_plan.h restates the queue count of vr_internal.h");

namespace {

float host_norm3(const float* d, int fma) {
    float s;
    if (fma) {
        s = std::fmaf(d[0], d[0], d[1] * d[1]);
        s = std::fmaf(d[2], d[2], s);
    } else {
        s = d[0] * d[0] + d[1] * d[1];
        s = d[2] * d[2] + s;
    }
    return std::sqrt(s);
}

}

void fill_tree_params(vr::KParams& k, const VrTreeOpaque* t) {
    k.nodes = t->arrays[kNodes].get<uint32_t>();
    k.leaves = t->arrays[kLeaves].get<uint16_t>();
    k.top = t->arrays[kTop].get<uint2>();
    k.bricks = t->arrays[kBricks].get<uint32_t>();
    k.top_levels = t->top_levels;
    k.brick_levels = t->brick_levels;
    k.brick_blocked = t->brick_blocked;
    k.extra = t->extra.get<float>();
    for (int i = 0; i < 3; ++i) {
        k.offset[i] = t->desc.offset[i];
        k.scale[i] = t->desc.scale[i];
    }
    k.N = t->desc.N;
    k.N3 = t->desc.N * t->desc.N * t->desc.N;
    k.capacity = t->desc.capacity;
    k.data_dim = t->desc.data_dim;
    k.format = t->desc.format;
    k.basis_dim = t->desc.basis_dim;
    k.leaf_stride_h = t->leaf_stride_h;
    k.max_depth = t->max_depth;
    k.ndc_width = t->desc.ndc_width;
    k.ndc_height = t->desc.ndc_height;
    k.ndc_focal = t->desc.ndc_focal;
    k.status = t->status.get<uint32_t>();
    k.sched_stats = t->sched_stats.get<unsigned long long>();
    for (int i = 0; i < 4; ++i) k.touch[i] = t->touch[i].get<uint32_t>();
}

int tile_geometry(int width, int height, int tile_w, int tile_h, int rank, int world, vr::KParams& k) {
    if (width <= 0 || height <= 0) return fail(VR_ERR_INVALID_ARGUMENT, "empty image");
    if (tile_w == 0 && tile_h == 0) {
        tile_w = (width + 7) & ~7;
        tile_h = (height + 7) & ~7;
    }
    if (tile_w <= 0 || tile_h <= 0 || (tile_w & 7) || (tile_h & 7))
        return fail(VR_ERR_INVALID_ARGUMENT, "tile size %dx%d must be positive multiples of 8",
                    tile_w, tile_h);
    k.tile_w = tile_w;
    k.tile_h = tile_h;
    k.tiles_x = (width + tile_w - 1) / tile_w;
    k.tiles_y = (height + tile_h - 1) / tile_h;
    k.rank = rank;
    k.world = world < 1 ? 1 : world;
    k.n_local_tiles = (int32_t)(((int64_t)k.tiles_x * k.tiles_y - rank + k.world - 1) / k.world);
    k.wblocks_per_tile_x = tile_w / 8;
    k.wblocks_per_tile = (tile_w / 8) * (tile_h / 8);
    k.n_wave_blocks = (int64_t)k.n_local_tiles * k.wblocks_per_tile;
    return VR_OK;
}

int launch_geometry(int width, int height, int tile_w, int tile_h, int rank, int world, int n_frames,
                    vr::KParams& k) {
    if (width < 1 || height < 1 || width > 65535 || height > 65535)
        return fail(VR_ERR_INVALID_ARGUMENT, "image size %dx%d outside [1, 65535]", width, height);
    if (int rc = tile_geometry(width, height, tile_w, tile_h, rank, world, k)) return rc;
    const int64_t total = k.n_wave_blocks * 64 * n_frames;
    if (total >= (1ll << 30))
        return fail(VR_ERR_INVALID_ARGUMENT, "batch of %lld rays exceeds the 2^30-ray queue",
                    (long long)total);
    k.total_rays = (uint32_t)total;
    return VR_OK;
}

int list_geometry(const char* what, int64_t n, vr::KParams& k) {
    if (n < 0 || n >= (1ll << 30))
        return fail(VR_ERR_INVALID_ARGUMENT, "%s: n=%lld outside [0, 2^30)", what, (long long)n);
    k.total_rays = vr::ray_list_slots(n);
    k.n_wave_blocks = k.total_rays >> 6;
    k.n_frames = n > 0 ? 1 : 0;
    k.width = vr::kRayListWidth;
    k.height = (int32_t)((n + vr::kRayListWidth - 1) >> vr::kRayListShift);
    k.fx = k.fy = 1.f;
    k.pitch = (int64_t)k.width * 4;
    k.tile_w = k.width;
    k.tile_h = (k.height + 7) & ~7;
    k.tiles_x = k.tiles_y = k.world = k.n_local_tiles = 1;
    return VR_OK;
}

namespace {

struct Views {
    const VrCamera* cams = nullptr;
    int n_frames = 0;
    vr::RayList list{};
    bool is_list = false;
    const vr::RayList* rays() const { return is_list ? &list : nullptr; }
};

int check_focal(const VrCamera& cam) {
    if (!(cam.fx != 0.f) || !(cam.fy != 0.f)) return fail(VR_ERR_INVALID_ARGUMENT, "focal length must be non-zero");
    return VR_OK;
}
int check_intrinsics(const VrCamera* cams, int i) {
    if (cams[i].width != cams[0].width || cams[i].height != cams[0].height || cams[i].fx != cams[0].fx ||
        cams[i].fy != cams[0].fy)
        return fail(VR_ERR_INVALID_ARGUMENT, "frame %d: intrinsics differ within the batch", i);
    return VR_OK;
}

int check_step_size(const VrRenderOptions* opt) {
    if (!(opt->step_size > 0.f))
        return fail(VR_ERR_INVALID_ARGUMENT, "step_size must be positive (got %g)", (double)opt->step_size);
    return VR_OK;
}

int pose_geometry(const VrCamera& cam, int tile_w, int tile_h, int rank, int world, int n_frames, vr::KParams& k) {
    if (int rc = launch_geometry(cam.width, cam.height, tile_w, tile_h, rank, world, n_frames, k)) return rc;
    k.width = cam.width;
    k.height = cam.height;
    k.fx = cam.fx;
    k.fy = cam.fy;
    k.n_frames = n_frames;
    return VR_OK;
}

int validate_batch(vr_tree_t t, int n_frames, const VrCamera* cams, const VrRenderOptions* opt,
                   const VrFrame* frames, vr::KParams& k) {
    if (!t || !cams || !opt || !frames) return fail(VR_ERR_INVALID_ARGUMENT, "NULL argument");
    if (n_frames < 1 || n_frames > VR_MAX_BATCH)
        return fail(VR_ERR_INVALID_ARGUMENT, "n_frames=%d outside [1,%d]", n_frames, VR_MAX_BATCH);
    const VrFrame* f = &frames[0];
    const VrCamera* cam = &cams[0];
    if (f->fp_mode != VR_FP_STRICT && f->fp_mode != VR_FP_FMA)
        return fail(VR_ERR_INVALID_ARGUMENT, "unknown fp_mode %d", f->fp_mode);
    if (f->layout != VR_LAYOUT_FRAME && f->layout != VR_LAYOUT_COMPACT)
        return fail(VR_ERR_INVALID_ARGUMENT, "unknown layout %d", f->layout);
    const int world = f->world < 1 ? 1 : f->world;
    if (f->rank < 0 || f->rank >= world)
        return fail(VR_ERR_INVALID_ARGUMENT, "rank %d outside world %d", f->rank, world);
    if (int rc = pose_geometry(*cam, f->tile_w, f->tile_h, f->rank, world, n_frames, k))
        return rc;
    k.pitch = f->pitch ? f->pitch : (int64_t)cam->width * 4;
    if (k.pitch < (int64_t)cam->width * 4 || k.pitch * cam->height >= (1ll << 32))
        return fail(VR_ERR_INVALID_ARGUMENT, "pitch %lld unusable for a %dx%d frame",
                    (long long)k.pitch, cam->width, cam->height);
    if (int rc = check_focal(*cam)) return rc;

    bool instrumented = false, any_accum = false;
    for (int i = 0; i < n_frames; ++i) {
        const VrFrame& fi = frames[i];
        if (!fi.rgba) return fail(VR_ERR_INVALID_ARGUMENT, "frame %d: rgba is NULL", i);
        if (int rc = check_intrinsics(cams, i)) return rc;
        if (fi.pitch != f->pitch || fi.offscreen != f->offscreen || fi.layout != f->layout ||
            fi.tile_w != f->tile_w || fi.tile_h != f->tile_h || fi.rank != f->rank ||
            fi.world != f->world || fi.fp_mode != f->fp_mode)
            return fail(VR_ERR_INVALID_ARGUMENT, "frame %d: layout/shard/fp_mode differ within the batch", i);
        instrumented = instrumented || fi.counters != nullptr;
        any_accum = any_accum || fi.accum != nullptr;
    }

    if (int rc = check_step_size(opt)) return rc;
    k.instrumented = instrumented ? 1 : 0;
    k.any_accum = any_accum ? 1 : 0;
    return VR_OK;
}

void fill_march_params(vr::KParams& k, const VrRenderOptions* opt) {
    k.step_size = opt->step_size;
    k.sigma_thresh = opt->sigma_thresh;
    k.stop_thresh = opt->stop_thresh;
    memcpy(k.bbox, opt->render_bbox, sizeof(k.bbox));
}

void fill_caller_params(vr::KParams& k, const VrRenderOptions* opt, const VrFrame* f) {
    fill_march_params(k, opt);
    k.background_brightness = opt->background_brightness;
    k.basis_min = opt->basis_minmax[0];
    k.basis_max = opt->basis_minmax[1];
    k.render_depth = opt->render_depth != 0;
    k.enable_probe = opt->enable_probe != 0;
    k.probe_disp_size = opt->probe_disp_size;

    const float angle = host_norm3(opt->rot_dirs, f->fp_mode == VR_FP_FMA);
    if ((double)angle < 1e-6) {
        k.rot_enabled = 0;
    } else {
        k.rot_enabled = 1;
        for (int i = 0; i < 3; ++i) k.rot_k[i] = opt->rot_dirs[i] / angle;
        k.rot_cos = cosf(angle);
        k.rot_sin = sinf(angle);
    }
    k.offscreen = f->offscreen != 0;
    k.layout = f->layout;
}

void fill_tuning_params(vr::KParams& k, const VrTreeOpaque* t, const Tuning& tn, const LaunchPlan& plan) {
    k.records_nt = plan.records_nt;
    k.march_max = tn.march_max;
    k.refill_min = tn.refill_min;
    k.drain_flush = tn.drain_flush;
    k.max_iter = tn.max_iter;
    k.frame_group = plan.frame_group;
    k.super_block = plan.super_block;
    k.n_queues = plan.n_queues;
    k.chunk_max = plan.chunk_max;
    const int flavour = vr::basis_flavour(t->desc.format, t->desc.basis_dim);
    k.basis_words = vr::basis_words(flavour);
    k.ray_tail_words = vr::ray_tail_words(t->desc.format, flavour);
    k.ray_vdir = vr::ray_vdir(t->desc.format, flavour) ? 1 : 0;
}

int record_words(LaunchKind kind, int ray_tail_words) {
    return kind == LaunchKind::kWeights ? vr::kWeightRayWords
           : kind == LaunchKind::kBackward ? vr::kGradRayWords : vr::kRayWords + ray_tail_words;
}
bool needs_file_order(LaunchKind kind) { return kind == LaunchKind::kWeights || kind == LaunchKind::kBackward; }

struct Turn { const vr::KParams& k; const Tuning& tn; int gen_waves; unsigned slot; hipStream_t hs; void* extra; };

template <typename Enqueue>
int run_launch(VrTreeOpaque* t, LaunchKind kind, const Views& v, size_t extra_bytes, vr::KParams& k, void* stream,
               Enqueue&& enqueue) {
    DeviceGuard device_guard(t->device);
    hipStream_t hs = static_cast<hipStream_t>(stream);
    std::unique_lock<std::mutex> guard(t->launch_mutex);
    if (needs_file_order(kind))
        if (int rc = ensure_file_nodes(t)) return rc;
    if (k.n_frames == 0) return VR_OK;
    const Tuning tn = t->tn;
    const LaunchPlan plan = plan_launch(kind, v.is_list ? RaySource::kList : RaySource::kFrames, k.n_frames, v.list.n,
                                        tn, t->arrays[kTop].bytes() + t->arrays[kBricks].bytes());
    fill_tuning_params(k, t, tn, plan);
    const size_t records = ray_buffer_bytes(k.total_rays, record_words(kind, k.ray_tail_words));
    unsigned slot;
    if (int rc = acquire_slot(t, guard, hs, k, records + extra_bytes, slot)) return rc;
    fill_tree_params(k, t);
    SlotTurn turn;
    if (int rc = turn.begin(t->slots[slot], hs)) return rc;
    void* const extra = extra_bytes ? t->slots[slot].rays.get<char>() + records : nullptr;
    return enqueue(Turn{k, tn, plan.raygen_waves, slot, hs, extra});
}

int validate_aov(int n_frames, const VrCamera* cams, const VrRenderOptions* opt, const VrFrame* frames,
                 const VrAov* aovs, int depth_units, vr::AovParams& a) {
    if (!aovs) return fail(VR_ERR_INVALID_ARGUMENT, "aovs is NULL");
    if (depth_units != VR_DEPTH_TREE && depth_units != VR_DEPTH_WORLD)
        return fail(VR_ERR_INVALID_ARGUMENT, "unknown depth_units %d", depth_units);
    const int64_t row = (int64_t)cams[0].width * 4;
    const int64_t pitch = aovs[0].pitch ? aovs[0].pitch : row;
    for (int i = 0; i < n_frames; ++i) {
        if (!aovs[i].depth && !aovs[i].transmittance)
            return fail(VR_ERR_INVALID_ARGUMENT, "frame %d: both AOV planes are NULL", i);
        const int64_t pi = aovs[i].pitch ? aovs[i].pitch : row;
        if (pi < row || (pi & 3))
            return fail(VR_ERR_INVALID_ARGUMENT, "frame %d: AOV pitch %lld unusable for rows of %d floats", i,
                        (long long)aovs[i].pitch, cams[0].width);
        if (pi != pitch) return fail(VR_ERR_INVALID_ARGUMENT, "frame %d: AOV pitch differs within the batch", i);
    }
    if (opt->render_depth)
        return fail(VR_ERR_UNSUPPORTED, "vr_render_aov with render_depth: the depth visualisation already is that launch");
    if (opt->enable_probe)
        return fail(VR_ERR_UNSUPPORTED, "vr_render_aov with enable_probe: pixels under the probe disc are not traced");
    for (int i = 0; i < n_frames; ++i)
        if (frames[i].counters)
            return fail(VR_ERR_UNSUPPORTED, "frame %d: vr_render_aov has no instrumented flavour (counters)", i);
    a.pitch = pitch;
    a.depth_world = depth_units == VR_DEPTH_WORLD;
    return VR_OK;
}

int enqueue_tables(const vr::KParams& k, const Views& v, hipStream_t hs, const VrFrame* frames = nullptr,
                   const VrAov* aovs = nullptr, const vr::AovParams& a = vr::AovParams{},
                   const vr::MaskParams& m = vr::MaskParams{}) {
    for (int first = 0; first < k.n_frames; first += vr::kTableChunk) {
        vr::FrameTable tbl;
        memset(&tbl, 0, sizeof(tbl));
        tbl.first = first;
        tbl.n = k.n_frames - first < vr::kTableChunk ? k.n_frames - first : vr::kTableChunk;
        for (int i = 0; i < tbl.n; ++i) {
            if (!v.is_list) memcpy(tbl.f[i].xf, v.cams[first + i].transform, sizeof(tbl.f[i].xf));
            if (!frames) continue;
            tbl.f[i].rgba = static_cast<uint8_t*>(frames[first + i].rgba);
            tbl.f[i].accum = frames[first + i].accum;
            tbl.f[i].depth = frames[first + i].depth;
            tbl.f[i].counters = reinterpret_cast<VrCounters*>(frames[first + i].counters);
        }
        HIP_TRY(vr::launch_prepare(k, tbl, hs, m.mask, m.words_per_frame));
        if (aovs) {
            vr::AovTable at;
            memset(&at, 0, sizeof(at));
            at.first = first;
            at.n = tbl.n;
            for (int i = 0; i < at.n; ++i) {
                at.f[i].depth = aovs[first + i].depth;
                at.f[i].transmittance = aovs[first + i].transmittance;
            }
            HIP_TRY(vr::launch_prepare_aov(a, at, hs));
        }
    }
    return VR_OK;
}

bool culls_blocks(const VrTreeOpaque* t, const vr::KParams& k, const Tuning& tn, const VrRenderOptions* opt) {
    if (!tn.block_cull || !t->occ || !vr::uses_lookup(k) || vr::needs_full(k)) return false;
    if (opt->sigma_thresh < 0.f || k.ndc_width > 0) return false;
    for (int i = 0; i < 3; ++i)
        if (!(opt->render_bbox[i] >= 0.f) || !(opt->render_bbox[i + 3] <= 1.f)) return false;
    return block_mask_words(k) <= (uint32_t)vr::kMaskMaxWords;
}

int render_launch(vr_tree_t t, int n_frames, const VrCamera* cams, const VrRenderOptions* opt,
                  const VrFrame* frames, const VrAov* aovs, int depth_units, bool want_aov, void* stream) {
    vr::KParams k;
    memset(&k, 0, sizeof(k));
    vr::AovParams a;
    memset(&a, 0, sizeof(a));
    if (int rc = validate_batch(t, n_frames, cams, opt, frames, k)) return rc;
    if (want_aov)
        if (int rc = validate_aov(n_frames, cams, opt, frames, aovs, depth_units, a)) return rc;
    fill_caller_params(k, opt, &frames[0]);
    const Views v{cams, n_frames};
    const size_t mask_bytes = t->occ ? block_mask_bytes(k, n_frames) : 0;
    return run_launch(t, want_aov ? LaunchKind::kAov : LaunchKind::kColour, v, mask_bytes, k, stream, [&](const Turn& u) -> int {
        a.planes = t->slot_aovs.get<vr::AovDesc>() + (size_t)u.slot * vr::kMaxBatch;
        if (u.k.enable_probe)
            HIP_TRY(vr::launch_probe(u.k, opt->probe, const_cast<float*>(u.k.probe_coeffs), u.hs));
        vr::MaskParams m{};
        vr::CullParams cull{};
        if (u.extra && culls_blocks(t, u.k, u.tn, opt)) {
            m.mask = static_cast<uint32_t*>(u.extra);
            m.words_per_frame = block_mask_words(u.k);
            m.nbx = (uint32_t)(u.k.tiles_x * (u.k.tile_w / 8));
            m.nby = (uint32_t)(u.k.tiles_y * (u.k.tile_h / 8));
            m.occ = t->occ.get<uint32_t>();
            m.levels = t->occ_levels;
            const int groups = 2048 / n_frames;
            m.groups_per_frame = groups < 4 ? 4 : (groups > 128 ? 128 : groups);
            cull = vr::CullParams{m.mask, m.words_per_frame, m.nbx, t->cull_stats.get<unsigned long long>()};
        }
        if (int rc = enqueue_tables(u.k, v, u.hs, frames, want_aov ? aovs : nullptr, a, m)) return rc;
        if (m.mask) HIP_TRY(vr::launch_block_mask(u.k, m, u.hs));
        if (want_aov)
            HIP_TRY(vr::launch_render_aov(u.k, a, cull, frames[0].fp_mode, t->n_cus, u.tn.waves_per_cu, u.gen_waves, u.hs));
        else
            HIP_TRY(vr::launch_render(u.k, cull, frames[0].fp_mode, t->n_cus, u.tn.waves_per_cu, u.gen_waves, u.hs));
        return VR_OK;
    });
}

int validate_march(int n_frames, const VrCamera* cams, const VrRenderOptions* opt, int fp_mode, vr::KParams& k) {
    if (fp_mode != VR_FP_STRICT && fp_mode != VR_FP_FMA)
        return fail(VR_ERR_INVALID_ARGUMENT, "unknown fp_mode %d", fp_mode);
    if (n_frames < 0 || n_frames > VR_MAX_BATCH)
        return fail(VR_ERR_INVALID_ARGUMENT, "n_frames=%d outside [0,%d]", n_frames, VR_MAX_BATCH);
    if (int rc = check_step_size(opt)) return rc;
    if (n_frames == 0) return VR_OK;
    if (int rc = pose_geometry(cams[0], 0, 0, 0, 1, n_frames, k)) return rc;
    if (int rc = check_focal(cams[0])) return rc;
    for (int i = 1; i < n_frames; ++i)
        if (int rc = check_intrinsics(cams, i)) return rc;
    return VR_OK;
}

int validate_weights(vr_tree_t t, int n_frames, const VrCamera* cams, const VrRenderOptions* opt, int fp_mode,
                     const VrLeafWeights* out, vr::KParams& k) {
    if (!t || !opt || !out || (n_frames > 0 && !cams)) return fail(VR_ERR_INVALID_ARGUMENT, "NULL argument");
    if (!out->max_weight && !out->hits) return fail(VR_ERR_INVALID_ARGUMENT, "both outputs are NULL");
    return validate_march(n_frames, cams, opt, fp_mode, k);
}

int validate_rays(const char* what, vr_tree_t t, int64_t n, const VrRays* rays, const VrRenderOptions* opt,
                  int fp_mode, const void* out, vr::KParams& k, Views& v) {
    if (!t || !rays || !rays->origins || !rays->dirs || !opt || !out)
        return fail(VR_ERR_INVALID_ARGUMENT, "%s: NULL argument", what);
    if (fp_mode != VR_FP_STRICT && fp_mode != VR_FP_FMA)
        return fail(VR_ERR_INVALID_ARGUMENT, "%s: unknown fp_mode %d", what, fp_mode);
    if (int rc = list_geometry(what, n, k)) return rc;
    if (int rc = check_step_size(opt)) return rc;
    v.list = vr::RayList{rays->origins, rays->dirs, n};
    v.is_list = true;
    return VR_OK;
}

template <typename Launch>
int march_launch(vr_tree_t t, LaunchKind kind, const Views& v, const VrRenderOptions* opt, vr::KParams& k, void* stream,
                 Launch&& launch) {
    fill_march_params(k, opt);
    k.offscreen = 1;
    k.layout = VR_LAYOUT_FRAME;
    k.pitch = (int64_t)k.width * 4;
    return run_launch(t, kind, v, 0, k, stream, [&](const Turn& u) -> int {
        if (int rc = enqueue_tables(u.k, v, u.hs)) return rc;
        HIP_TRY(launch(u));
        return VR_OK;
    });
}

int weights_launch(vr_tree_t t, const Views& v, const VrRenderOptions* opt, int fp_mode, const VrLeafWeights* out,
                   vr::KParams& k, void* stream) {
    return march_launch(t, LaunchKind::kWeights, v, opt, k, stream, [&](const Turn& u) {
        vr::WeightParams w;
        w.max_weight = reinterpret_cast<uint32_t*>(out->max_weight);
        w.hits = out->hits;
        w.file_node = t->file_node_dev.get<int32_t>();
        return vr::launch_weights(u.k, w, fp_mode, t->n_cus, u.tn.waves_per_cu, u.gen_waves, u.tn.weights_check != 0,
                                  u.hs, v.rays());
    });
}


int check_backward_options(const char* what, const VrRenderOptions* opt) {
    if (opt->render_depth)
        return fail(VR_ERR_UNSUPPORTED, "%s with render_depth: the depth visualisation has no derivative here", what);
    if (opt->enable_probe)
        return fail(VR_ERR_UNSUPPORTED, "%s with enable_probe: pixels under the probe disc are not traced", what);
    if (!(opt->rot_dirs[0] == 0.f) || !(opt->rot_dirs[1] == 0.f) || !(opt->rot_dirs[2] == 0.f))
        return fail(VR_ERR_UNSUPPORTED, "%s with rot_dirs: the view direction is not rotated", what);
    return VR_OK;
}

int validate_backward(const char* what, vr_tree_t t, int n_frames, const VrCamera* cams, const VrRenderOptions* opt,
                      int fp_mode, const float* grad_accum, const float* grad_data, vr::KParams& k) {
    if (!t || !opt || !grad_accum || !grad_data || (n_frames > 0 && !cams))
        return fail(VR_ERR_INVALID_ARGUMENT, "NULL argument");
    if (int rc = validate_march(n_frames, cams, opt, fp_mode, k)) return rc;
    return check_backward_options(what, opt);
}

int check_backward_tree(const VrTreeOpaque* t, const VrRenderOptions* opt, const char* what) {
    const int format = t->desc.format, basis_dim = t->desc.basis_dim;
    if (format == VR_FORMAT_SG || format == VR_FORMAT_ASG)
        return fail(VR_ERR_UNSUPPORTED, "%s: SG / ASG trees are not supported", what);
    if (vr::basis_flavour(format, basis_dim) != vr::BASIS_RGBA &&
        (opt->basis_minmax[0] > 0 || opt->basis_minmax[1] < basis_dim - 1))
        return fail(VR_ERR_UNSUPPORTED, "%s: basis_minmax [%d, %d] leaves out basis functions of the tree (%d)", what,
                    opt->basis_minmax[0], opt->basis_minmax[1], basis_dim);
    return VR_OK;
}

int backward_launch(const char* what, vr_tree_t t, const Views& v, const VrRenderOptions* opt, int fp_mode,
                    const float* grad_accum, float* grad_data, uint32_t* touched, vr::KParams& k, void* stream) {
    if (int rc = check_backward_tree(t, opt, what)) return rc;
    return march_launch(t, LaunchKind::kBackward, v, opt, k, stream, [&](const Turn& u) {
        vr::GradParams g;
        g.grad_accum = grad_accum;
        g.grad_data = grad_data;
        g.file_node = t->file_node_dev.get<int32_t>();
        g.touched = touched;
        return vr::launch_grad(u.k, g, fp_mode, t->n_cus, u.tn.waves_per_cu, u.gen_waves, u.hs, v.rays());
    });
}

int backward_rays(const char* what, vr_tree_t t, int64_t n, const VrRays* rays, const VrRenderOptions* opt,
                  int fp_mode, const float* grad_accum, float* grad_data, uint32_t* touched, void* stream) {
    vr::KParams k;
    memset(&k, 0, sizeof(k));
    Views v;
    if (!grad_accum) return fail(VR_ERR_INVALID_ARGUMENT, "%s: NULL argument", what);
    if (int rc = validate_rays(what, t, n, rays, opt, fp_mode, grad_data, k, v)) return rc;
    if (int rc = check_backward_options(what, opt)) return rc;
    return backward_launch(what, t, v, opt, fp_mode, grad_accum, grad_data, touched, k, stream);
}

}

extern "C" {

int vr_render_backward(vr_tree_t t, int n_frames, const VrCamera* cams, const VrRenderOptions* opt, int fp_mode,
                       const float* grad_accum, float* grad_data, void* stream) {
    vr::KParams k;
    memset(&k, 0, sizeof(k));
    if (int rc = validate_backward("vr_render_backward", t, n_frames, cams, opt, fp_mode, grad_accum, grad_data, k)) return rc;
    return backward_launch("vr_render_backward", t, Views{cams, n_frames}, opt, fp_mode, grad_accum, grad_data, nullptr,
                           k, stream);
}

int vr_render_backward_touched(vr_tree_t t, int n_frames, const VrCamera* cams, const VrRenderOptions* opt, int fp_mode,
                               const float* grad_accum, float* grad_data, uint32_t* touched, void* stream) {
    vr::KParams k;
    memset(&k, 0, sizeof(k));
    if (!touched) return fail(VR_ERR_INVALID_ARGUMENT, "vr_render_backward_touched: NULL argument");
    if (int rc = validate_backward("vr_render_backward_touched", t, n_frames, cams, opt, fp_mode, grad_accum, grad_data, k))
        return rc;
    return backward_launch("vr_render_backward_touched", t, Views{cams, n_frames}, opt, fp_mode, grad_accum, grad_data,
                           touched, k, stream);
}

int vr_render_backward_rays(vr_tree_t t, int64_t n, const VrRays* rays, const VrRenderOptions* opt, int fp_mode,
                            const float* grad_accum, float* grad_data, void* stream) {
    return backward_rays("vr_render_backward_rays", t, n, rays, opt, fp_mode, grad_accum, grad_data, nullptr, stream);
}

int vr_render_backward_rays_touched(vr_tree_t t, int64_t n, const VrRays* rays, const VrRenderOptions* opt, int fp_mode,
                                    const float* grad_accum, float* grad_data, uint32_t* touched, void* stream) {
    if (!touched) return fail(VR_ERR_INVALID_ARGUMENT, "vr_render_backward_rays_touched: NULL argument");
    return backward_rays("vr_render_backward_rays_touched", t, n, rays, opt, fp_mode, grad_accum, grad_data, touched,
                         stream);
}

int vr_fit_rays(vr_tree_t t, int64_t n, const VrRays* rays, const VrRenderOptions* opt, int fp_mode, const VrFit* fit,
                void* stream) {
    const char* const what = "vr_fit_rays";
    vr::KParams k;
    memset(&k, 0, sizeof(k));
    Views v;
    if (int rc = validate_rays(what, t, n, rays, opt, fp_mode, fit, k, v)) return rc;
    if (!fit->target || !fit->grad_data) return fail(VR_ERR_INVALID_ARGUMENT, "%s: NULL argument", what);
    if (!std::isfinite(fit->grad_scale))
        return fail(VR_ERR_INVALID_ARGUMENT, "%s: grad_scale must be finite (got %g)", what, (double)fit->grad_scale);
    if (int rc = check_backward_options(what, opt)) return rc;
    if (int rc = check_backward_tree(t, opt, what)) return rc;
    return march_launch(t, LaunchKind::kBackward, v, opt, k, stream, [&](const Turn& u) {
        vr::FitParams f;
        f.target = fit->target;
        f.grad_data = fit->grad_data;
        f.file_node = t->file_node_dev.get<int32_t>();
        f.touched = fit->touched;
        f.sq_err = fit->sq_err;
        f.accum = fit->accum;
        f.bg = opt->background_brightness;
        f.grad_scale = fit->grad_scale;
        return vr::launch_fit(u.k, f, fp_mode, t->n_cus, u.tn.waves_per_cu, u.gen_waves, u.hs, v.rays());
    });
}

int vr_accumulate_weights(vr_tree_t t, int n_frames, const VrCamera* cams, const VrRenderOptions* opt,
                          int fp_mode, const VrLeafWeights* out, void* stream) {
    vr::KParams k;
    memset(&k, 0, sizeof(k));
    if (int rc = validate_weights(t, n_frames, cams, opt, fp_mode, out, k)) return rc;
    return weights_launch(t, Views{cams, n_frames}, opt, fp_mode, out, k, stream);
}

int vr_accumulate_weights_rays(vr_tree_t t, int64_t n, const VrRays* rays, const VrRenderOptions* opt, int fp_mode,
                               const VrLeafWeights* out, void* stream) {
    vr::KParams k;
    memset(&k, 0, sizeof(k));
    Views v;
    if (int rc = validate_rays("vr_accumulate_weights_rays", t, n, rays, opt, fp_mode, out, k, v)) return rc;
    if (!out->max_weight && !out->hits)
        return fail(VR_ERR_INVALID_ARGUMENT, "vr_accumulate_weights_rays: both outputs are NULL");
    return weights_launch(t, v, opt, fp_mode, out, k, stream);
}

int vr_render_rays(vr_tree_t t, int64_t n, const VrRays* rays, const VrRenderOptions* opt, int fp_mode,
                   const VrRayOut* out, void* stream) {
    vr::KParams k;
    memset(&k, 0, sizeof(k));
    Views v;
    if (int rc = validate_rays("vr_render_rays", t, n, rays, opt, fp_mode, out, k, v)) return rc;
    if (!out->rgba && !out->accum) return fail(VR_ERR_INVALID_ARGUMENT, "vr_render_rays: both outputs are NULL");
    if (opt->render_depth)
        return fail(VR_ERR_UNSUPPORTED, "vr_render_rays with render_depth: the depth visualisation is not what a ray list is for");
    if (opt->enable_probe)
        return fail(VR_ERR_UNSUPPORTED, "vr_render_rays with enable_probe: the probe disc is a set of pixel positions");
    if (n == 0) return VR_OK;
    VrFrame f;
    memset(&f, 0, sizeof(f));
    f.offscreen = 1;
    f.layout = VR_LAYOUT_FRAME;
    f.fp_mode = fp_mode;
    f.accum = out->accum;
    fill_caller_params(k, opt, &f);
    k.any_accum = out->accum ? 1 : 0;
    const size_t pixel_bytes = out->rgba ? 0 : list_pixel_bytes(k.total_rays);
    return run_launch(t, LaunchKind::kColour, v, pixel_bytes, k, stream, [&](const Turn& u) -> int {
        f.rgba = out->rgba ? out->rgba : u.extra;
        if (int rc = enqueue_tables(u.k, v, u.hs, &f)) return rc;
        HIP_TRY(vr::launch_render(u.k, vr::CullParams{}, fp_mode, t->n_cus, u.tn.waves_per_cu, u.gen_waves, u.hs, v.rays()));
        return VR_OK;
    });
}

int vr_render_batch(vr_tree_t t, int n_frames, const VrCamera* cams, const VrRenderOptions* opt,
                    const VrFrame* frames, void* stream) {
    return render_launch(t, n_frames, cams, opt, frames, nullptr, 0, false, stream);
}

int vr_render_aov(vr_tree_t t, int n_frames, const VrCamera* cams, const VrRenderOptions* opt,
                  const VrFrame* frames, const VrAov* aovs, int depth_units, void* stream) {
    return render_launch(t, n_frames, cams, opt, frames, aovs, depth_units, true, stream);
}

int vr_render(vr_tree_t t, const VrCamera* cam, const VrRenderOptions* opt, const VrFrame* f,
              void* stream) {
    return vr_render_batch(t, 1, cam, opt, f, stream);
}

}
```

volrend_amd/csrc/vr_launch_plan.cpp:

```cpp
#include "vr_launch_plan.h"

namespace {

constexpr int kColourChunkCap = 256, kGuidedChunkCap = 4096;

int raygen_waves(const Tuning& tn, int n_frames) {
    return tn.raygen_waves > 0 ? tn.raygen_waves : (n_frames <= 2 ? 4 : 16);
}
constexpr int64_t kRayListSmall = 2 * 800 * 800;
int raygen_waves_list(const Tuning& tn, int64_t n) {
    return tn.raygen_waves > 0 ? (tn.raygen_waves >= 16 ? 16 : 4) : (n <= kRayListSmall ? 4 : 16);
}

}

LaunchPlan plan_launch(LaunchKind kind, RaySource source, int n_frames, int64_t list_rays, const Tuning& tn,
                       uint64_t lookup_bytes) {
    const bool colour = kind == LaunchKind::kColour || kind == LaunchKind::kAov;
    const bool list = source == RaySource::kList;
    LaunchPlan p;
    p.chunk_max = tn.chunk_max > 0 ? tn.chunk_max : colour ? kColourChunkCap : kGuidedChunkCap;
    p.super_block = tn.super_block > 0 ? tn.super_block : (colour && !list && n_frames > 2) ? 4 : 1;
    p.raygen_waves = list ? raygen_waves_list(tn, list_rays) : raygen_waves(tn, n_frames);
    p.records_nt = tn.records_nt >= 0 ? tn.records_nt : lookup_bytes > (128ull << 20);
    p.frame_group = tn.frame_group < 1 || tn.frame_group > n_frames ? n_frames : tn.frame_group;
    p.n_queues = tn.xcd_queues ? kPlanQueues : 1;
    return p;
}
```

volrend_amd/csrc/vr_launch_plan.h:

```cpp
#pragma once
#include <cstdint>

#pragma GCC visibility push(hidden)

struct Tuning {
    int march_max = 12;
    int refill_min = 20;
    int drain_flush = 16;
    int waves_per_cu = 0;
    int frame_group = 0;
    int super_block = 0;
    int records_nt = -1;
    int xcd_queues = 1;
    int chunk_max = 0;
    int raygen_waves = 0;
    int top_levels = 0;
    int brick_levels = 3;
    int brick_blocked = -1;
    int max_iter = 1 << 22;
    int weights_check = 1;
    int block_cull = 1;
};

enum class LaunchKind { kColour, kAov, kWeights, kBackward };
enum class RaySource { kFrames, kList };

constexpr int kPlanQueues = 8;

struct LaunchPlan {
    int chunk_max, super_block, records_nt, frame_group, n_queues;
    int raygen_waves;
};

LaunchPlan plan_launch(LaunchKind kind, RaySource source, int n_frames, int64_t list_rays, const Tuning& tn,
                       uint64_t lookup_bytes);

#pragma GCC visibility pop
```

volrend_amd/csrc/vr_render.hip:

```cpp
#include "vr_device_math.h"
#include "vr_internal.h"
#include "vr_dev_layout.h"
#include "vr_dev_shade.h"
#include "vr_dev_query.h"
#include "vr_dev_rays.h"

namespace vr {

namespace {

constexpr int kSh16Waves = 5;
constexpr int kSh25Waves = 4;
constexpr int kSh9Waves = 7;
constexpr int kSh16Rows = 64;

constexpr int kRing = 128;

template <int BASIS>
struct Stage {
    static constexpr bool kEnabled = BASIS > 1;
    static constexpr int kVec = kEnabled ? RecTraits<BASIS>::kDwords / 4 : 1;
    static constexpr int kRow = kVec * 16;
    static constexpr int kPerInstr = kWave / kVec;
    static constexpr int kPass = !kEnabled ? kWave
                                 : (kRow * kWave <= 5504 ? kWave
                                    : (BASIS == BASIS_16 ? kSh16Rows : kWave / 2));
    static constexpr int kPasses = (BASIS == BASIS_25) ? 2 : 1;
    static constexpr int kShade = kPass * kPasses;
    static constexpr int kInstr = (kPass + kPerInstr - 1) / kPerInstr;
    static constexpr int kBytes = (kEnabled && kPass * kRow > 768) ? kPass * kRow : 768;
};
typedef __attribute__((address_space(1))) const void* vr_gptr_t;
typedef __attribute__((address_space(3))) void* vr_lptr_t;
constexpr int kOwnerQ = 4;

template <int BASIS, bool NT, int RING = kRing>
__device__ __forceinline__ void issue_records(const KParams& p, char* stage, const uint32_t* it_leaf,
                                              uint32_t ring_head, int lane, int n, int pass) {
    using ST = Stage<BASIS>;
#pragma unroll
    for (int k = 0; k < ST::kInstr; ++k) {
        const int rin = k * ST::kPerInstr + lane / ST::kVec;
        const int item = pass * ST::kPass + rin;
        if (lane < ST::kPerInstr * ST::kVec && rin < ST::kPass && item < n) {
            const uint32_t leaf = it_leaf[(ring_head + (uint32_t)item) & (RING - 1)];
            const char* src = reinterpret_cast<const char*>(p.leaves) +
                              (uint64_t)leaf * (uint32_t)(p.leaf_stride_h * 2) + (lane % ST::kVec) * 16;
            __builtin_amdgcn_global_load_lds(
                (vr_gptr_t)src,
                (vr_lptr_t)((__attribute__((address_space(3))) char*)stage + k * ST::kPerInstr * ST::kRow),
                16, 0, NT ? 2  : 0);
        }
    }
}

template <int BASIS, int MODE>
constexpr int min_waves_per_eu() {
    if (MODE != MODE_FAST) return BASIS == BASIS_25 ? 3 : 4;
    return BASIS == BASIS_25 ? kSh25Waves : BASIS == BASIS_16 ? kSh16Waves : BASIS == BASIS_9 ? kSh9Waves : 8;
}
template <int BASIS, int MODE>
constexpr bool aov_depth_in_lds() {
    return MODE == MODE_FAST && (BASIS == BASIS_9 || BASIS == BASIS_16 || BASIS == BASIS_25);
}
template <int BASIS, int MODE, bool AOV = false>
constexpr int waves_per_cu() {
    const int lds = ((kRing * 9 + kWave * 4 + (AOV && aov_depth_in_lds<BASIS, MODE>() ? kWave * 4 : 0) +
                      Stage<BASIS>::kBytes + 511) / 512) * 512;
    const int by_lds = 163840 / lds, by_reg = 4 * min_waves_per_eu<BASIS, MODE>();
    return by_lds < by_reg ? by_lds : by_reg;
}

__device__ __forceinline__ void store_aov(const AovParams& a, int frame, uint32_t xy, float d, float tr) {
    const AovDesc pl = a.planes[frame];
    const int64_t off = (int64_t)(xy >> 16) * a.pitch + (int64_t)(xy & 0xFFFFu) * 4;
    typedef __attribute__((address_space(1))) float vr_gfloat_t;
    if (pl.depth) *(vr_gfloat_t*)(reinterpret_cast<char*>(pl.depth) + off) = d;
    if (pl.transmittance) *(vr_gfloat_t*)(reinterpret_cast<char*>(pl.transmittance) + off) = tr;
}

template <int FMA, bool FULL>
__device__ __forceinline__ void store_colour_ray(const KParams& p, uint32_t slot, const Ray& nr, uint32_t xy,
                                                 uint8_t* px, int frame, const float* vdir) {
    uint32_t* rb = ray_slot(p.ray_buf_rw, kRayWords + p.ray_tail_words, slot);
#pragma unroll
    for (int i = 0; i < 3; ++i) {
        ray_word(rb, kRayCen + i) = f2u(nr.cen[i]);
        ray_word(rb, kRayDir + i) = f2u(nr.dir[i]);
        ray_word(rb, kRayInvDir + i) = f2u(nr.invdir[i]);
    }
    ray_word(rb, kRayT) = f2u(nr.t);
    ray_word(rb, kRayTmax) = f2u(nr.tmax);
    ray_word(rb, kRayDeltaScale) = f2u(nr.delta_scale);
    ray_word(rb, kRayXy) = xy;
    ray_word(rb, kRayPixelLo) = (uint32_t)reinterpret_cast<uint64_t>(px);
    ray_word(rb, kRayPixelHi) = (uint32_t)(reinterpret_cast<uint64_t>(px) >> 32);
    ray_word(rb, kRayFrame) = (uint32_t)frame;
    if (p.ray_vdir) {
#pragma unroll
        for (int i = 0; i < 3; ++i) ray_word(rb, kRayTail + i) = f2u(vdir[i]);
    } else if (p.basis_words > 0) {
        float b[VR_MAX_BASIS];
#pragma unroll
        for (int i = 0; i < VR_MAX_BASIS; ++i) b[i] = 0.f;
        precalc_basis<FMA, FULL>(p, vdir, b);
#pragma unroll
        for (int i = 0; i < VR_MAX_BASIS; ++i)
            if (i < p.basis_words)
                ray_word(rb, kRayTail + i) = f2u((i < p.basis_min || i > p.basis_max) ? 0.f : b[i]);
    }
}

__device__ __forceinline__ AovParams aov_arg() { return AovParams{}; }
__device__ __forceinline__ const AovParams& aov_arg(const AovParams& a) { return a; }

template <int FMA, int BASIS, int MODE, bool BLK, typename... PLANES>
__global__ __launch_bounds__(kWave, (min_waves_per_eu<BASIS, MODE>()))
void render_kernel(const KParams p, const PLANES... planes) {
    constexpr bool AOV = sizeof...(PLANES) != 0;
    const AovParams aov = aov_arg(planes...);
    using P = Policy<FMA>;
    constexpr bool N2 = MODE != MODE_GENERIC;
    constexpr bool LOBES = MODE != MODE_FAST;
    constexpr bool COUNT = MODE != MODE_FAST;
    constexpr int NB = BASIS > 1 ? BASIS : 1;
    constexpr bool HAS_BASIS = BASIS != BASIS_RGBA;
    using ST = Stage<BASIS>;
    __shared__ uint32_t it_leaf[kRing];
    __shared__ float it_w[kRing];
    __shared__ uint8_t it_own[kRing];
    __shared__ __attribute__((aligned(16))) char stage[ST::kBytes];
    float* const res = reinterpret_cast<float*>(stage);
    float mybasis[NB];
#pragma unroll
    for (int i = 0; i < NB; ++i) mybasis[i] = 0.f;

    const int lane = threadIdx.x & (kWave - 1);
    Ray ray;
    ray.active = false;
    ray.alive = ray.entered = ray.stopped = false;
    __shared__ uint32_t ray_ids[kWave];
    ray.t = 0.f;
    ray.tmax = -1.f;
    ray.light = 1.f;
    ray.delta_scale = 1.f;
#pragma unroll
    for (int i = 0; i < 3; ++i) {
        ray.cen[i] = 0.f;
        ray.dir[i] = 0.f;
        ray.invdir[i] = 1.f;
    }
    ray.out[0] = ray.out[1] = ray.out[2] = ray.out[3] = 0.f;
    RayCounters rc;
    Cursor cur;
    uint32_t qpos = 0;
    uint32_t qsh = 32;
    uint32_t rounds = 0, progress_round = 0;
    bool exhausted = false;
    uint32_t chunk_next = 0, chunk_end = 0;
    uint32_t ring_head = 0, ring_tail = 0;
    const int wpr = kRayWords + p.ray_tail_words;
    uint32_t st_march_r = 0, st_march_l = 0, st_shade_r = 0, st_shade_l = 0, st_distinct = 0,
             st_fin_r = 0, st_fin_l = 0, st_iter = 0;
    constexpr bool D_LDS = AOV && aov_depth_in_lds<BASIS, MODE>();
    float d_reg = 0.f;
    float* d_lds = nullptr;
    if constexpr (D_LDS) {
        __shared__ float d_words[kWave];
        d_lds = d_words;
    }
    auto depth_get = [&]() -> float {
        if constexpr (D_LDS) return d_lds[lane_id_now()];
        else return d_reg;
    };
    auto depth_set = [&](float v) {
        if constexpr (D_LDS) d_lds[lane_id_now()] = v;
        else d_reg = v;
    };

    auto shade_chunk = [&](int n) {
        __syncthreads();
        if (COUNT) {
            st_shade_r++;
            st_shade_l += (uint32_t)n;
            const uint32_t myleaf =
                lane < n ? it_leaf[(ring_head + (uint32_t)lane) & (kRing - 1)] : 0xFFFFFFFFu;
            bool first = lane < n;
            for (int o = 0; o < kWave; ++o) {
                const uint32_t other = (uint32_t)__shfl((int)myleaf, o);
                if (o < lane && other == myleaf) first = false;
            }
            st_distinct += (uint32_t)__builtin_popcountll(__builtin_amdgcn_ballot_w64(first));
            if (lane < n)
                touch(p, TOUCH_LEAVES, (uint64_t)myleaf * (uint32_t)(p.leaf_stride_h * 2),
                      (uint32_t)(2 * (p.data_dim - 1)));
        }
        const bool have = lane < n;
        const uint32_t jmine = (ring_head + (uint32_t)lane) & (kRing - 1);
        const float weight = have ? it_w[jmine] : 0.f;
        const int own4 = (HAS_BASIS && have) ? (int)it_own[jmine] << 2 : lane << 2;
        auto basis_of = [&](int i) -> float {
            return u2f((uint32_t)__builtin_amdgcn_ds_bpermute(own4, (int)f2u(mybasis[i])));
        };
        float bfull[ST::kPasses > 1 ? NB : 1];
        if constexpr (ST::kPasses > 1) {
#pragma unroll
            for (int i = 0; i < NB; ++i) bfull[i] = basis_of(i);
        }
        auto basis_get = [&](int i) -> float {
            if constexpr (ST::kPasses > 1) return bfull[i];
            else return basis_of(i);
        };
        float r0 = 0.f, r1 = 0.f, r2 = 0.f;
        if constexpr (ST::kEnabled) {
#pragma unroll
            for (int pass = 0; pass < ST::kPasses; ++pass) {
                if (pass * ST::kPass < n) {
                    if (p.records_nt)
                        issue_records<BASIS, true>(p, stage, it_leaf, ring_head, lane, n, pass);
                    else
                        issue_records<BASIS, false>(p, stage, it_leaf, ring_head, lane, n, pass);
                    __syncthreads();
                    if (ST::kPasses == 1 || lane / ST::kPass == pass) {
                        const char* row = stage + (lane % ST::kPass) * ST::kRow;
                        float acc[3];
                        channel_sums<FMA, BASIS>(row, basis_get, acc);
                        const float2v s01 = weighted_sigmoid2(weight, acc[0], acc[1]);
                        r0 = s01.x;
                        r1 = s01.y;
                        r2 = weighted_sigmoid(weight, acc[2]);
                    }
                    if (ST::kPasses > 1) __syncthreads();
                }
            }
        } else {
          const float b0 = HAS_BASIS ? basis_of(0) : 0.f;
          if (have) {
            Record<BASIS> rec;
            load_record<BASIS>(p, it_leaf[jmine], rec);
            if (HAS_BASIS) {
                r0 = weighted_sigmoid(weight, b0 * rec.at(0));
                r1 = weighted_sigmoid(weight, b0 * rec.at(1));
                r2 = weighted_sigmoid(weight, b0 * rec.at(2));
            } else {
                r0 = rec.at(0);
                r1 = rec.at(1);
                r2 = rec.at(2);
            }
          }
        }
        __syncthreads();
        if (have) {
            res[0 * kWave + lane] = r0;
            res[1 * kWave + lane] = r1;
            res[2 * kWave + lane] = r2;
        }
        __syncthreads();
        const uint32_t head8 = ring_head & 0xFFu;
#pragma unroll
        for (int d = 0; d < kOwnerQ; ++d) {
            const uint32_t pos = __builtin_amdgcn_ubfe(qpos, qsh, 8u);
            const uint32_t idx = (pos - head8) & 0xFFu;
            if (qsh < 32u && idx < (uint32_t)n) {
                if (HAS_BASIS) {
                    ray.out[0] += res[0 * kWave + idx];
                    ray.out[1] += res[1 * kWave + idx];
                    ray.out[2] += res[2 * kWave + idx];
                } else {
                    const float w = it_w[pos & (kRing - 1)];
                    ray.out[0] = P::madd(res[0 * kWave + idx], w, ray.out[0]);
                    ray.out[1] = P::madd(res[1 * kWave + idx], w, ray.out[1]);
                    ray.out[2] = P::madd(res[2 * kWave + idx], w, ray.out[2]);
                }
                qsh += 8u;
            }
        }
        ring_head += (uint32_t)n;
    };

    for (;;) {
        const bool done = ray.active && !(ray.t < ray.tmax) && qsh == 32u;
        const unsigned long long m_done = __builtin_amdgcn_ballot_w64(done);
        const unsigned long long m_free = __builtin_amdgcn_ballot_w64(!ray.active);
        const unsigned long long m_busy =
            __builtin_amdgcn_ballot_w64(ray.active && (ray.t < ray.tmax || qsh < 32u));
        const int n_avail = __builtin_popcountll(m_done | m_free);
        if (COUNT) st_iter++;
        if (n_avail > 0 && (m_busy == 0ull || (!exhausted && n_avail >= p.refill_min))) {
            if (COUNT && m_done != 0ull) {
                st_fin_r++;
                st_fin_l += (uint32_t)__builtin_popcountll(m_done);
            }
            uint32_t px_lo = 0, px_hi = 0, fin_xy = 0, fin_frame = 0;
            float fin_d = 0.f;
            ray.stopped = ray.tmax < 0.f;
            if (done) {
                const uint32_t* rs = ray_slot(p.ray_buf, wpr, ray_ids[lane_id_now()]);
                px_lo = ray_word(rs, kRayPixelLo);
                px_hi = ray_word(rs, kRayPixelHi);
                if (COUNT || p.any_accum || AOV) {
                    fin_xy = ray_word(rs, kRayXy);
                    fin_frame = ray_word(rs, kRayFrame);
                }
                if constexpr (AOV) {
                    fin_d = depth_get();
                    if (aov.depth_world) fin_d = fin_d * ray.delta_scale;
                }
            }
            const bool vacant = done || !ray.active;
            bool take = false;
            if (m_done != 0ull) progress_round = (uint32_t)__builtin_amdgcn_readfirstlane((int)rounds);
            if (!exhausted && chunk_next >= chunk_end) {
                uint32_t lo, hi;
                grab_chunk(p, lane, lo, hi);
                lo = __builtin_amdgcn_readfirstlane(lo);
                hi = __builtin_amdgcn_readfirstlane(hi);
                if (hi == lo) {
                    exhausted = true;
                } else {
                    chunk_next = lo;
                    chunk_end = hi;
                }
            }
            if (!exhausted) {
                const unsigned long long idle = m_done | m_free;
                const uint32_t r = chunk_next + lane_rank(idle);
                const uint32_t c_end = chunk_end;
                const uint32_t left = chunk_end - chunk_next;
                chunk_next += (uint32_t)n_avail < left ? (uint32_t)n_avail : left;
                if (vacant && r < c_end) {
                    take = true;
                    const uint32_t* rs = ray_slot(p.ray_buf, wpr, r);
#pragma unroll
                    for (int i = 0; i < 3; ++i) {
                        ray.cen[i] = u2f(ray_word(rs, kRayCen + i));
                        ray.dir[i] = u2f(ray_word(rs, kRayDir + i));
                        ray.invdir[i] = u2f(ray_word(rs, kRayInvDir + i));
                    }
                    ray.t = u2f(ray_word(rs, kRayT));
                    ray.tmax = u2f(ray_word(rs, kRayTmax));
                    ray.delta_scale = u2f(ray_word(rs, kRayDeltaScale));
                    ray_ids[lane_id_now()] = r;
                    if (HAS_BASIS) {
                        if (BASIS > 1 && p.ray_vdir) {
                            float vd[3];
#pragma unroll
                            for (int i = 0; i < 3; ++i) vd[i] = u2f(ray_word(rs, kRayTail + i));
                            precalc_basis<FMA, false, (BASIS > 1 ? BASIS : 1)>(p, vd, mybasis);
#pragma unroll
                            for (int i = 0; i < NB; ++i)
                                if (i < p.basis_min || i > p.basis_max) mybasis[i] = 0.f;
                        } else {
#pragma unroll
                            for (int i = 0; i < NB; ++i)
                                mybasis[i] = u2f(ray_word(rs, kRayTail + i));
                        }
                    }
                }
            }
            if (done)
                finish_ray<FMA, COUNT>(
                    p, ray, rc,
                    reinterpret_cast<uint8_t*>(((uint64_t)px_hi << 32) | (uint64_t)px_lo), fin_xy,
                    (int)fin_frame);
            if constexpr (AOV) {
                if (done) store_aov(aov, (int)fin_frame, fin_xy, fin_d, ray.light);
                if (vacant) depth_set(0.f);
            }
            if (vacant) {
                ray.active = ray.entered = take;
                if (!take) {
                    ray.t = 0.f;
                    ray.tmax = -1.f;
                }
                ray.out[0] = ray.out[1] = ray.out[2] = ray.out[3] = 0.f;
                ray.light = 1.f;
                rc = RayCounters();
                cur = Cursor();
                qsh = 32u;
                qpos = 0;
            }
        }
        if (!wave_any(ray.active)) {
            if (exhausted) break;
            continue;
        }

        if (rounds - progress_round >= (uint32_t)p.max_iter) {
            if (ray.t < ray.tmax) {
                ray.t = ray.tmax;
                if (p.status) atomicOr(p.status, 1u);
            }
            progress_round = rounds;
        }
        int m = 0;
        for (; m < p.march_max; ++m) {
            const unsigned long long m_go = __builtin_amdgcn_ballot_w64(ray.t < ray.tmax) &
                                            __builtin_amdgcn_ballot_w64(qsh != 0u);
            if (m_go == 0ull) break;
            const bool go = ray.t < ray.tmax && qsh != 0u;
            if (COUNT) {
                st_march_r++;
                st_march_l += (uint32_t)__builtin_popcountll(__builtin_amdgcn_ballot_w64(go));
            }
            bool push = false;
            uint32_t leaf = 0;
            float weight = 0.f;
            if (go) {
                float pos[3];
                pos[0] = P::madd(ray.t, ray.dir[0], ray.cen[0]);
                pos[1] = P::madd(ray.t, ray.dir[1], ray.cen[1]);
                pos[2] = P::madd(ray.t, ray.dir[2], ray.cen[2]);
                float cube_sz = 0.f;
                int levels;
                uint32_t word;
                if (N2) {
                    leaf = query_n2<COUNT, (MODE == MODE_FAST ? (BLK ? 1 : 0) : -1)>(p, pos, &levels, &word, cur);
                } else {
                    leaf = (uint32_t)query_generic<FMA, COUNT>(p, pos, &cube_sz, &levels, &word);
                }
                if (COUNT) {
                    rc.samples++;
                    rc.child_reads += (uint32_t)levels;
                }
                const float dda = dda_unit<FMA>(pos, ray.invdir);
                const float t_subcube =
                    N2 ? __builtin_amdgcn_ldexpf(dda, -levels) : dda / cube_sz;
                const float delta_t = t_subcube + p.step_size;
                const float sigma = h2f((uint16_t)(word & 0xFFFFu));
                bool stop = false;
                if (sigma > p.sigma_thresh) {
                    if (COUNT) rc.hits++;
                    const float att = vr_expf_nonan(-delta_t * ray.delta_scale * sigma);
                    weight = ray.light * (1.f - att);
                    if constexpr (AOV) depth_set(P::madd(weight, ray.t, depth_get()));
                    if (COUNT && p.render_depth)
                        ray.out[0] = P::madd(weight, ray.t, ray.out[0]);
                    else
                        push = true;
                    ray.light *= att;
                    stop = ray.light < p.stop_thresh;
                }
                if (stop) {
                    ray.tmax = -1.f;
                    if (COUNT) rc.early++;
                } else {
                    ray.t += delta_t;
                }
            }
            const unsigned long long m_push = __builtin_amdgcn_ballot_w64(push);
            if (m_push != 0ull) {
                if (push) {
                    const uint32_t seq = ring_tail + lane_rank(m_push);
                    const uint32_t j = seq & (kRing - 1);
                    it_leaf[j] = leaf;
                    it_w[j] = weight;
                    it_own[j] = (uint8_t)lane;
                    qpos = __builtin_amdgcn_alignbit(seq, qpos, 8u);
                    qsh -= 8u;
                }
                ring_tail += (uint32_t)__builtin_popcountll(m_push);
                while (ring_tail - ring_head >= (uint32_t)ST::kShade) shade_chunk(ST::kShade);
            }
            if (exhausted) {
                const unsigned long long m_alive = __builtin_amdgcn_ballot_w64(ray.t < ray.tmax);
                if (__builtin_popcountll(m_alive) <= p.drain_flush &&
                    (m_alive & __builtin_amdgcn_ballot_w64(qsh == 0u)) != 0ull && ring_tail != ring_head) {
                    const uint32_t waiting = ring_tail - ring_head;
                    shade_chunk(waiting < (uint32_t)ST::kShade ? (int)waiting : ST::kShade);
                }
            }
        }
        rounds = (uint32_t)__builtin_amdgcn_readfirstlane((int)(rounds + (uint32_t)m));
        while (ring_tail != ring_head && !wave_any(ray.t < ray.tmax && qsh > 0u)) {
            const uint32_t waiting = ring_tail - ring_head;
            shade_chunk(waiting < (uint32_t)ST::kShade ? (int)waiting : ST::kShade);
        }
    }
    if (COUNT && p.sched_stats && lane == 0) {
        atomicAdd(&p.sched_stats[kStatMarchRounds], (unsigned long long)st_march_r);
        atomicAdd(&p.sched_stats[kStatMarchLanes], (unsigned long long)st_march_l);
        atomicAdd(&p.sched_stats[kStatShadeRounds], (unsigned long long)st_shade_r);
        atomicAdd(&p.sched_stats[kStatShadeLanes], (unsigned long long)st_shade_l);
        atomicAdd(&p.sched_stats[kStatDistinctLeaves], (unsigned long long)st_distinct);
        atomicAdd(&p.sched_stats[kStatRetireRounds], (unsigned long long)st_fin_r);
        atomicAdd(&p.sched_stats[kStatRetiredRays], (unsigned long long)st_fin_l);
        atomicAdd(&p.sched_stats[kStatIterations], (unsigned long long)st_iter);
    }
}



template <int FMA, bool FULL, int GW, typename... PLANES>
__global__ __launch_bounds__(kWave* GW)
void raygen_kernel(const KParams p, const PLANES... planes, const CullParams cull) {
    constexpr bool AOV = sizeof...(PLANES) != 0;
    const AovParams aov = aov_arg(planes...);
    const int lane = threadIdx.x & (kWave - 1);
    const int wave = threadIdx.x >> 6;
    const uint32_t id =
        (uint32_t)(((int64_t)blockIdx.x * GW + wave) * kWave + lane);
    bool valid = false;
    bool culled = false;
    Ray nr;
    uint8_t* px = nullptr;
    uint32_t xy = 0;
    int frame = 0;
    float vdir[3] = {0.f, 0.f, 1.f};
    if (id < p.total_rays) {
        const PixelRef r = locate(p, id);
        if constexpr (!FULL) {
            if (cull.mask) {
                const uint32_t b = (uint32_t)(r.y >> 3) * cull.nbx + (uint32_t)(r.x >> 3);
                const uint32_t w = cull.mask[(size_t)r.frame * cull.words_per_frame + (b >> 5)];
                culled = __builtin_amdgcn_readfirstlane((int)((w >> (b & 31u)) & 1u)) == 0;
            }
        }
        if (r.in_image) {
            frame = r.frame;
            xy = (uint32_t)r.x | ((uint32_t)r.y << 16);
            px = pixel_ptr(p, p.frames[r.frame], r);
            if (culled) reset_ray(nr);
            else setup_ray<FMA>(p, r, nr, vdir);
            if (nr.alive) {
                valid = true;
            } else {
                RayCounters z;
                finish_ray<FMA, FULL>(p, nr, z, px, xy, frame);
                if constexpr (AOV) store_aov(aov, frame, xy, 0.f, 1.f);
            }
        }
    }
    const unsigned long long m_valid = __builtin_amdgcn_ballot_w64(valid);
    __shared__ uint32_t wave_culled[GW];
    if constexpr (!FULL && GW > 1) {
        if (cull.mask && lane == 0) wave_culled[wave] = culled ? 1u : 0u;
    }
    const uint32_t my_base = reserve_ray_slots<GW>(p, m_valid, lane, wave);
    if constexpr (!FULL) {
        if (cull.mask && threadIdx.x < 2u) {
            const int64_t left = (int64_t)(p.total_rays >> 6) - (int64_t)blockIdx.x * GW;
            uint32_t n = (uint32_t)(left < 0 ? 0 : (left < GW ? left : GW));
            if (threadIdx.x == 1u) {
                if constexpr (GW > 1) {
                    n = 0;
#pragma unroll
                    for (int w = 0; w < GW; ++w) n += wave_culled[w];
                } else {
                    n = culled ? 1u : 0u;
                }
            }
            if (n)
                atomicAdd(cull.stats + (blockIdx.x & (uint32_t)(kCullStatLines - 1)) * kCullStatStride + threadIdx.x,
                          (unsigned long long)n);
        }
    }
    if (!valid) return;
    const uint32_t slot = my_base + lane_rank(m_valid);
    uint32_t* rb = ray_slot(p.ray_buf_rw, kRayWords + p.ray_tail_words, slot);
#pragma unroll
    for (int i = 0; i < 3; ++i) {
        ray_word(rb, kRayCen + i) = f2u(nr.cen[i]);
        ray_word(rb, kRayDir + i) = f2u(nr.dir[i]);
        ray_word(rb, kRayInvDir + i) = f2u(nr.invdir[i]);
    }
    ray_word(rb, kRayT) = f2u(nr.t);
    ray_word(rb, kRayTmax) = f2u(nr.tmax);
    ray_word(rb, kRayDeltaScale) = f2u(nr.delta_scale);
    ray_word(rb, kRayXy) = xy;
    ray_word(rb, kRayPixelLo) = (uint32_t)reinterpret_cast<uint64_t>(px);
    ray_word(rb, kRayPixelHi) = (uint32_t)(reinterpret_cast<uint64_t>(px) >> 32);
    ray_word(rb, kRayFrame) = (uint32_t)frame;
    if (p.ray_vdir) {
#pragma unroll
        for (int i = 0; i < 3; ++i) ray_word(rb, kRayTail + i) = f2u(vdir[i]);
    } else if (p.basis_words > 0) {
        float b[VR_MAX_BASIS];
#pragma unroll
        for (int i = 0; i < VR_MAX_BASIS; ++i) b[i] = 0.f;
        precalc_basis<FMA, FULL>(p, vdir, b);
#pragma unroll
        for (int i = 0; i < VR_MAX_BASIS; ++i)
            if (i < p.basis_words)
                ray_word(rb, kRayTail + i) = f2u((i < p.basis_min || i > p.basis_max) ? 0.f : b[i]);
    }
}

template <int FMA, bool FULL, int GW>
__global__ __launch_bounds__(kWave* GW) void raygen_rays_kernel(const KParams p, const RayList rl) {
    const int lane = threadIdx.x & (kWave - 1);
    const int wave = threadIdx.x >> 6;
    uint32_t id;
    Ray nr;
    float vdir[3] = {0.f, 0.f, 1.f};
    const bool has = list_ray<FMA, GW>(p, rl, lane, wave, id, nr, vdir);
    bool valid = false;
    uint8_t* px = nullptr;
    uint32_t xy = 0;
    if (has) {
        xy = (id & (uint32_t)(kRayListWidth - 1)) | ((id >> kRayListShift) << 16);
        px = p.frames[0].rgba + (int64_t)id * 4;
        if (nr.alive) {
            valid = true;
        } else {
            RayCounters z;
            finish_ray<FMA, false>(p, nr, z, px, xy, 0);
        }
    }
    const unsigned long long m_valid = __builtin_amdgcn_ballot_w64(valid);
    const uint32_t my_base = reserve_ray_slots<GW>(p, m_valid, lane, wave);
    if (!valid) return;
    store_colour_ray<FMA, FULL>(p, my_base + lane_rank(m_valid), nr, xy, px, 0, vdir);
}

__global__ void prepare_launch_kernel(FrameTable tbl, FrameDesc* frames, uint32_t* queue_head, uint32_t* mask,
                                      uint32_t words_per_frame) {
    const int i = threadIdx.x;
    if (i < tbl.n) frames[tbl.first + i] = tbl.f[i];
    if (tbl.first == 0 && i < kMaxQueues) {
        queue_head[i * kQueueStride + kQueueHead] = 0u;
        queue_head[i * kQueueStride + kQueueCount] = 0u;
    }
    if (mask) {
        uint4* const q = reinterpret_cast<uint4*>(mask + (size_t)tbl.first * words_per_frame);
        const uint32_t n = (uint32_t)tbl.n * (words_per_frame >> 2);
        for (uint32_t j = threadIdx.x; j < n; j += blockDim.x) q[j] = make_uint4(0u, 0u, 0u, 0u);
    }
}

__global__ __launch_bounds__(256) void block_mask_kernel(const KParams p, const MaskParams m) {
    __shared__ uint32_t bits[kMaskMaxWords];
    __shared__ uint32_t whole;
    const uint32_t wpf = m.words_per_frame;
    for (uint32_t i = threadIdx.x; i < wpf; i += blockDim.x) bits[i] = 0u;
    if (threadIdx.x == 0) whole = 0u;
    __syncthreads();
    const int frame = blockIdx.y;
    const int g = m.levels;
    const uint32_t count = m.occ[0];
    const uint32_t* const list = m.occ + kOccHeaderWords + occ_bitmap_words(g);
    const uint32_t per = (count + (uint32_t)m.groups_per_frame - 1u) / (uint32_t)m.groups_per_frame;
    const uint32_t lo = blockIdx.x * per;
    const uint32_t hi = lo + per < count ? lo + per : count;
    float xf[12];
#pragma unroll
    for (int i = 0; i < 12; ++i) xf[i] = p.frames[frame].xf[i];
    const float cell = u2f((uint32_t)(127 - g) << 23);
    float inv_scale[3], r2 = 0.f;
#pragma unroll
    for (int i = 0; i < 3; ++i) {
        inv_scale[i] = 1.f / p.scale[i];
        const float h = 0.5f * cell * inv_scale[i];
        r2 += h * h;
    }
    const float r = __builtin_sqrtf(r2) * 1.0001f;
    bool ok = r > 0.f && r < 1e30f;
#pragma unroll
    for (int a = 0; a < 3; ++a)
#pragma unroll
        for (int b = a; b < 3; ++b) {
            const float d = xf[3 * a] * xf[3 * b] + xf[3 * a + 1] * xf[3 * b + 1] + xf[3 * a + 2] * xf[3 * b + 2];
            if (!(__builtin_fabsf(d - (a == b ? 1.f : 0.f)) <= 1e-4f)) ok = false;
        }
    const float afx = __builtin_fabsf(p.fx), afy = __builtin_fabsf(p.fy);
    const uint32_t n_mask = (1u << g) - 1u;
    const float fnbx = (float)m.nbx, fnby = (float)m.nby;
    if (!ok && lo < hi) whole = 1u;
    for (uint32_t idx = lo + threadIdx.x; ok && idx < hi; idx += blockDim.x) {
        const uint32_t c = list[idx];
        const float tc[3] = {((float)((c >> (2 * g)) & n_mask) + 0.5f) * cell, ((float)((c >> g) & n_mask) + 0.5f) * cell,
                             ((float)(c & n_mask) + 0.5f) * cell};
        float d[3];
#pragma unroll
        for (int i = 0; i < 3; ++i) d[i] = (tc[i] - p.offset[i]) * inv_scale[i] - xf[9 + i];
        const float X = xf[0] * d[0] + xf[1] * d[1] + xf[2] * d[2];
        const float Y = xf[3] * d[0] + xf[4] * d[1] + xf[5] * d[2];
        const float depth = -(xf[6] * d[0] + xf[7] * d[1] + xf[8] * d[2]);
        if (!(depth - r > 0.01f * r)) {
            if (!(depth + r < 0.f)) whole = 1u;
            continue;
        }
        const float inv = 1.f / (depth * (depth - r));
        const float rx = afx * r * __builtin_sqrtf(depth * depth + X * X) * inv * 1.05f + 1.f;
        const float ry = afy * r * __builtin_sqrtf(depth * depth + Y * Y) * inv * 1.05f + 1.f;
        const float px = 0.5f * (float)p.width + p.fx * X / depth;
        const float py = 0.5f * (float)p.height - p.fy * Y / depth;
        const float fx0 = __builtin_floorf(__builtin_fmaxf((px - rx) * 0.125f, 0.f));
        const float fx1 = __builtin_floorf(__builtin_fminf((px + rx) * 0.125f, fnbx - 1.f));
        const float fy0 = __builtin_floorf(__builtin_fmaxf((py - ry) * 0.125f, 0.f));
        const float fy1 = __builtin_floorf(__builtin_fminf((py + ry) * 0.125f, fnby - 1.f));
        if (!(fx0 <= fx1) || !(fy0 <= fy1)) continue;
        const uint32_t bx0 = (uint32_t)fx0, bx1 = (uint32_t)fx1, by0 = (uint32_t)fy0, by1 = (uint32_t)fy1;
        for (uint32_t by = by0; by <= by1; ++by) {
            const uint32_t first = by * m.nbx + bx0, last = by * m.nbx + bx1;
            for (uint32_t w = first >> 5; w <= (last >> 5); ++w) {
                const uint32_t from = w == (first >> 5) ? (first & 31u) : 0u;
                const uint32_t to = w == (last >> 5) ? (last & 31u) : 31u;
                const uint32_t mask = (0xFFFFFFFFu >> (31u - to)) & (0xFFFFFFFFu << from);
                if ((bits[w] & mask) != mask) atomicOr(&bits[w], mask);
            }
        }
    }
    __syncthreads();
    uint32_t* const out = m.mask + (size_t)frame * wpf;
    const bool all = whole != 0u;
    for (uint32_t i = threadIdx.x; i < wpf; i += blockDim.x) {
        const uint32_t v = all ? 0xFFFFFFFFu : bits[i];
        if (v != 0u && (out[i] & v) != v) atomicOr(&out[i], v);
    }
}

__global__ void prepare_aov_kernel(AovTable tbl, AovDesc* planes) {
    const int i = threadIdx.x;
    if (i < tbl.n) planes[tbl.first + i] = tbl.f[i];
}

template <int FMA>
__global__ void probe_overlay_kernel(const KParams p) {
    using P = Policy<FMA>;
    const int side = p.probe_disp_size + 5;
    const int idx = blockIdx.x * blockDim.x + threadIdx.x;
    if (idx >= side * side) return;
    const int y = idx / side;
    const int x = p.width - side + (idx - y * side);
    if (x < 0 || x >= p.width || y >= p.height) return;
    const int tx = x / p.tile_w, ty = y / p.tile_h;
    const int tile = ty * p.tiles_x + tx;
    if (tile % p.world != p.rank) return;
    float cen[3], dir[3], out[4] = {0.f, 0.f, 0.f, 0.f};
    const int xx = x - (p.width - p.probe_disp_size) + 5;
    const int yy = y - 5;
    cen[0] = -((float)xx / (0.5f * (float)p.probe_disp_size) - 1.f);
    cen[1] = ((float)yy / (0.5f * (float)p.probe_disp_size) - 1.f);
    const float c = P::madd(cen[0], cen[0], cen[1] * cen[1]);
    if (!(c <= 1.f)) return;
    if (p.basis_dim >= 0) {
        float basis_fn[VR_MAX_BASIS];
#pragma unroll
        for (int i = 0; i < VR_MAX_BASIS; ++i) basis_fn[i] = 0.f;
        cen[2] = -__builtin_sqrtf(1 - c);
        float xf[9];
        for (int i = 0; i < 9; ++i) xf[i] = p.frames[blockIdx.y].xf[i];
        mv3<FMA>(xf, cen, dir);
        precalc_basis<FMA, true>(p, dir, basis_fn);
        int hi = p.basis_max;
        if (hi > p.basis_dim - 1) hi = p.basis_dim - 1;
        const int lo = p.basis_min < 0 ? 0 : p.basis_min;
        for (int tt = 0; tt < 3; ++tt) {
            const int off = tt * p.basis_dim;
            float tmp = 0.f;
            for (int i = lo; i <= hi; ++i) tmp = P::madd(basis_fn[i], p.probe_coeffs[off + i], tmp);
            out[tt] = sigmoid(tmp);
        }
    } else {
        for (int i = 0; i < 3; ++i) out[i] = p.probe_coeffs[i];
    }
    out[3] = 1.f;
    const int64_t pix = (int64_t)y * p.width + x;
    const FrameDesc& fd = p.frames[blockIdx.y];
    if (fd.accum) reinterpret_cast<float4*>(fd.accum)[pix] = make_float4(out[0], out[1], out[2], out[3]);
    uint8_t* const px = pixel_address(p, fd, tile / p.world, x - tx * p.tile_w, y - ty * p.tile_h, x, y);
    *reinterpret_cast<uint32_t*>(px) =
        quant8(out[0]) | (quant8(out[1]) << 8) | (quant8(out[2]) << 16) | 0xFF000000u;
}

__global__ void probe_kernel(const KParams p, float probe0, float probe1, float probe2,
                             float* out) {
    float cen[3] = {p.offset[0] + p.scale[0] * probe0, p.offset[1] + p.scale[1] * probe1,
                    p.offset[2] + p.scale[2] * probe2};
    float cube_sz;
    int levels;
    uint32_t word;
    const int64_t leaf = query_generic<0>(p, cen, &cube_sz, &levels, &word);
    const uint16_t* v = p.leaves + leaf * p.leaf_stride_h;
    for (int i = threadIdx.x; i < p.data_dim - 1; i += blockDim.x) out[i] = h2f(v[i]);
}

template <int FMA, int MODE, typename... PLANES>
hipError_t launch_basis(const KParams& p, int64_t total_blocks, int n_cus, int waves_override, hipStream_t s,
                        const PLANES&... planes) {
    const dim3 block(kWave);
    constexpr bool kAov = sizeof...(PLANES) != 0;
#define VR_LAUNCH(B)                                                                         \
    do {                                                                                     \
        const dim3 grid(persistent_grid(total_blocks, n_cus,                                 \
                                        waves_override > 0 ? waves_override : waves_per_cu<B, MODE, kAov>())); \
        constexpr bool kBlk = MODE == MODE_FAST;                                             \
        if (kBlk && p.brick_blocked)                                                         \
            hipLaunchKernelGGL((render_kernel<FMA, B, MODE, kBlk, PLANES...>), grid, block, 0, s, p, planes...); \
        else                                                                                 \
            hipLaunchKernelGGL((render_kernel<FMA, B, MODE, false, PLANES...>), grid, block, 0, s, p, planes...); \
    } while (0)
    switch (basis_flavour(p.format, p.basis_dim)) {
        case BASIS_RGBA: VR_LAUNCH(BASIS_RGBA); break;
        case BASIS_25: VR_LAUNCH(BASIS_25); break;
        case BASIS_16: VR_LAUNCH(BASIS_16); break;
        case BASIS_9: VR_LAUNCH(BASIS_9); break;
        case BASIS_4: VR_LAUNCH(BASIS_4); break;
        default: VR_LAUNCH(BASIS_1); break;
    }
#undef VR_LAUNCH
    return hipGetLastError();
}

template <int FMA, typename... PLANES>
hipError_t launch_fp(const KParams& p, int64_t total_blocks, int n_cus, int waves_override, hipStream_t s,
                     const PLANES&... planes) {
    if (!uses_lookup(p)) return launch_basis<FMA, MODE_GENERIC>(p, total_blocks, n_cus, waves_override, s, planes...);
    if (needs_full(p)) return launch_basis<FMA, MODE_FULL>(p, total_blocks, n_cus, waves_override, s, planes...);
    return launch_basis<FMA, MODE_FAST>(p, total_blocks, n_cus, waves_override, s, planes...);
}

template <typename... PLANES>
hipError_t launch_march(const KParams& p, const CullParams& cull, int fp_mode, int n_cus, int waves_override,
                        int gen_waves, hipStream_t stream, const RayList* rays, const PLANES&... planes) {
    const int64_t total_blocks = p.n_wave_blocks * p.n_frames;
    {
        const bool full = needs_full(p);
#define VR_GEN(FMA_, FULL_, GW_)                                                                    \
    do {                                                                                            \
        const dim3 grid_((unsigned)((total_blocks + GW_ - 1) / GW_)), block_(kWave * GW_);          \
        if (rays) {                                                                                 \
            if constexpr (sizeof...(PLANES) == 0 && GW_ >= 4)                                       \
                hipLaunchKernelGGL((raygen_rays_kernel<FMA_, FULL_, GW_>), grid_, block_, 0, stream, p, *rays); \
        }                                                                                           \
        else hipLaunchKernelGGL((raygen_kernel<FMA_, FULL_, GW_, PLANES...>), grid_, block_, 0, stream, p, planes..., cull); \
    } while (0)
#define VR_GEN_GW(FMA_, FULL_)                                                                      \
    do {                                                                                            \
        if (gen_waves >= 16) VR_GEN(FMA_, FULL_, 16);                                               \
        else if (gen_waves >= 4 || rays) VR_GEN(FMA_, FULL_, 4);             \
        else VR_GEN(FMA_, FULL_, 1);                                                                \
    } while (0)
        if (fp_mode == VR_FP_FMA) {
            if (full) VR_GEN_GW(1, true); else VR_GEN_GW(1, false);
        } else {
            if (full) VR_GEN_GW(0, true); else VR_GEN_GW(0, false);
        }
#undef VR_GEN_GW
#undef VR_GEN
    }
    return fp_mode == VR_FP_FMA ? launch_fp<1>(p, total_blocks, n_cus, waves_override, stream, planes...)
                                : launch_fp<0>(p, total_blocks, n_cus, waves_override, stream, planes...);
}

}

hipError_t launch_prepare(const KParams& p, const FrameTable& tbl, hipStream_t stream, uint32_t* mask,
                          uint32_t words_per_frame) {
    hipLaunchKernelGGL(prepare_launch_kernel, dim3(1), dim3(64), 0, stream, tbl,
                       const_cast<FrameDesc*>(p.frames), p.queue_head, mask, words_per_frame);
    return hipGetLastError();
}

hipError_t launch_block_mask(const KParams& p, const MaskParams& m, hipStream_t stream) {
    if (p.n_frames <= 0 || m.groups_per_frame <= 0) return hipSuccess;
    hipLaunchKernelGGL(block_mask_kernel, dim3((unsigned)m.groups_per_frame, (unsigned)p.n_frames), dim3(256), 0, stream,
                       p, m);
    return hipGetLastError();
}

hipError_t launch_render(const KParams& p, const CullParams& cull, int fp_mode, int n_cus, int waves_override,
                         int gen_waves, hipStream_t stream, const RayList* rays) {
    if (p.n_wave_blocks <= 0 || p.n_frames <= 0) return hipSuccess;
    const hipError_t e = launch_march(p, cull, fp_mode, n_cus, waves_override, gen_waves, stream, rays);
    if (e != hipSuccess || !p.enable_probe || p.probe_disp_size <= 0) return e;
    const int side = p.probe_disp_size + 5;
    const dim3 pgrid((unsigned)((side * side + 255) / 256), (unsigned)p.n_frames);
    if (fp_mode == VR_FP_FMA)
        hipLaunchKernelGGL(probe_overlay_kernel<1>, pgrid, dim3(256), 0, stream, p);
    else
        hipLaunchKernelGGL(probe_overlay_kernel<0>, pgrid, dim3(256), 0, stream, p);
    return hipGetLastError();
}

hipError_t launch_prepare_aov(const AovParams& a, const AovTable& tbl, hipStream_t stream) {
    hipLaunchKernelGGL(prepare_aov_kernel, dim3(1), dim3(64), 0, stream, tbl, const_cast<AovDesc*>(a.planes));
    return hipGetLastError();
}

hipError_t launch_render_aov(const KParams& p, const AovParams& a, const CullParams& cull, int fp_mode, int n_cus,
                             int waves_override, int gen_waves, hipStream_t stream) {
    if (p.n_wave_blocks <= 0 || p.n_frames <= 0) return hipSuccess;
    return launch_march(p, cull, fp_mode, n_cus, waves_override, gen_waves, stream,  nullptr, a);
}

hipError_t launch_probe(const KParams& p, const float probe[3], float* out_dev,
                        hipStream_t stream) {
    hipLaunchKernelGGL(probe_kernel, dim3(1), dim3(64), 0, stream, p, probe[0], probe[1],
                       probe[2], out_dev);
    return hipGetLastError();
}

}
```

volrend_amd/csrc/vr_upload.cpp:

```cpp
#include <hip/hip_runtime.h>

#include <algorithm>
#include <chrono>
#include <cstdio>
#include <cstdlib>
#include <future>
#include <memory>
#include <mutex>
#include <new>
#include <vector>

#include "vr_h2d.h"
#include "vr_host.h"
#include "vr_tree_walk.h"

namespace {

int check_quant(const VrTreeDesc* d, const VrQuantDesc* q) {
    if (q->n_quant < 0 || q->n_retained < 0 || q->n_quant + q->n_retained < 1)
        return fail(VR_ERR_INVALID_ARGUMENT, "quantised tree needs at least one basis function");
    if (3 * (q->n_quant + q->n_retained) + 1 > d->data_dim)
        return fail(VR_ERR_INVALID_ARGUMENT, "%d quantised + %d retained basis functions do not "
                    "fit data_dim=%d", q->n_quant, q->n_retained, d->data_dim);
    if (!q->sigma) return fail(VR_ERR_INVALID_ARGUMENT, "sigma is NULL");
    if (q->n_quant && (!q->quant_colors || !q->quant_map))
        return fail(VR_ERR_INVALID_ARGUMENT, "quant_colors/quant_map is NULL");
    if (q->n_retained && !q->data_retained)
        return fail(VR_ERR_INVALID_ARGUMENT, "data_retained is NULL");
    return VR_OK;
}

hipError_t decode_quant_on_device(const VrTreeDesc* d, const VrQuantDesc* q, size_t n_slots,
                                  uint16_t* d_data, int device) {
    const void* src[4] = {q->quant_colors, q->quant_map, q->sigma, q->data_retained};
    const size_t sz[4] = {(size_t)q->n_quant * 65536 * 3 * sizeof(uint16_t), (size_t)q->n_quant * n_slots * sizeof(uint16_t),
                          n_slots * sizeof(uint16_t), (size_t)q->n_retained * n_slots * 3 * sizeof(uint16_t)};
    DeviceBuffer tmp[4];
    const void* dev[4] = {nullptr, nullptr, nullptr, nullptr};
    hipError_t e = hipSuccess;
    CopySegment segs[4];
    int n_seg = 0;
    for (int i = 0; i < 4 && e == hipSuccess; ++i) {
        if (!sz[i]) continue;
        if (d->memory == 1) {
            dev[i] = src[i];
            continue;
        }
        e = tmp[i].alloc(sz[i]);
        segs[n_seg++] = CopySegment{tmp[i].get(), src[i], sz[i]};
        dev[i] = tmp[i].get();
    }
    if (e == hipSuccess && n_seg) e = staged_h2d_multi(segs, n_seg, device);
    if (e == hipSuccess)
        e = vr::launch_decode_quant((const uint16_t*)dev[0], (const uint16_t*)dev[1],
                                    (const uint16_t*)dev[2], (const uint16_t*)dev[3], d_data,
                                    (int64_t)n_slots, q->n_quant, q->n_retained, d->data_dim,
                                    nullptr);
    if (e == hipSuccess) e = hipDeviceSynchronize();
    return e;
}

int check_tree_desc(const VrTreeDesc* d, bool need_data) {
    if (!d->child || (need_data && !d->data))
        return fail(VR_ERR_INVALID_ARGUMENT, "child/data is NULL");
    if (d->N < 2 || d->N > 16) return fail(VR_ERR_INVALID_ARGUMENT, "N=%d out of range", d->N);
    if (d->capacity <= 0) return fail(VR_ERR_INVALID_ARGUMENT, "capacity must be positive");
    if (d->format < VR_FORMAT_RGBA || d->format > VR_FORMAT_ASG)
        return fail(VR_ERR_INVALID_ARGUMENT, "unknown data format %d", d->format);
    const int min_dim = d->format == VR_FORMAT_RGBA ? 4 : 3 * d->basis_dim + 1;
    if (d->format != VR_FORMAT_RGBA && (d->basis_dim < 1 || d->basis_dim > VR_MAX_BASIS))
        return fail(VR_ERR_INVALID_ARGUMENT, "basis_dim=%d out of range [1,%d]", d->basis_dim,
                    VR_MAX_BASIS);
    if (d->data_dim < min_dim)
        return fail(VR_ERR_INVALID_ARGUMENT, "data_dim=%d too small for the format (need %d)",
                    d->data_dim, min_dim);
    if (d->format == VR_FORMAT_SG && (!d->extra || d->extra_count < (uint64_t)d->basis_dim * 4))
        return fail(VR_ERR_INVALID_ARGUMENT, "SG needs basis_dim*4 extra floats");
    if (d->format == VR_FORMAT_ASG && (!d->extra || d->extra_count < (uint64_t)d->basis_dim * 11))
        return fail(VR_ERR_INVALID_ARGUMENT, "ASG needs basis_dim*11 extra floats");
    return VR_OK;
}

hipError_t alloc_launch_scratch(VrTreeOpaque* t) {
    hipError_t e = t->status.alloc(sizeof(uint32_t));
    if (e == hipSuccess) e = hipMemset(t->status.get(), 0, sizeof(uint32_t));
    if (e == hipSuccess) e = t->sched_stats.alloc(vr::kSchedStats * sizeof(unsigned long long));
    if (e == hipSuccess) e = hipMemset(t->sched_stats.get(), 0, vr::kSchedStats * sizeof(unsigned long long));
    const size_t cull_sz = (size_t)vr::kCullStatLines * vr::kCullStatStride * sizeof(unsigned long long);
    if (e == hipSuccess) e = t->cull_stats.alloc(cull_sz);
    if (e == hipSuccess) e = hipMemset(t->cull_stats.get(), 0, cull_sz);
    if (e == hipSuccess) e = t->probe_buf.alloc(sizeof(float) * (size_t)t->desc.data_dim * kLaunchSlots);
    for (unsigned i = 0; i < kLaunchSlots && e == hipSuccess; ++i) e = t->slots[i].done.create();
    if (e == hipSuccess) e = t->slot_frames.alloc(sizeof(vr::FrameDesc) * vr::kMaxBatch * kLaunchSlots);
    if (e == hipSuccess) e = t->slot_heads.alloc(sizeof(uint32_t) * vr::kSlotWords * kLaunchSlots);
    if (e == hipSuccess) e = t->slot_aovs.alloc(sizeof(vr::AovDesc) * vr::kMaxBatch * kLaunchSlots);
    int cus = 0;
    if (e == hipSuccess && hipDeviceGetAttribute(&cus, hipDeviceAttributeMultiprocessorCount, t->device) == hipSuccess &&
        cus > 0)
        t->n_cus = cus;
    return e;
}


struct UploadJob {
    const VrTreeDesc* d;
    const VrQuantDesc* q;
    const int32_t* host_child;
    int N3;
    size_t n_slots, child_sz, data_sz;
    bool from_host;
    bool timing;
    std::chrono::steady_clock::time_point t_start;
    void mark(const char* what) const {
        const std::chrono::duration<double, std::milli> ms = std::chrono::steady_clock::now() - t_start;
        if (timing) fprintf(stderr, "[volrend_hip] upload: %s at %.1f ms\n", what, ms.count());
    }
};

int check_upload_args(const VrTreeDesc* d, const VrQuantDesc* q, vr_tree_t* out) {
    if (!d || !out) return fail(VR_ERR_INVALID_ARGUMENT, "desc/out is NULL");
    *out = nullptr;
    if (int rc = check_tree_desc(d, q == nullptr)) return rc;
    return q ? check_quant(d, q) : VR_OK;
}

int fetch_child_words(UploadJob& j, std::vector<int32_t>& fetched) {
    if (j.from_host) return VR_OK;
    fetched.resize(j.n_slots);
    HIP_TRY(hipMemcpy(fetched.data(), j.d->child, j.child_sz, hipMemcpyDeviceToHost));
    j.host_child = fetched.data();
    return VR_OK;
}

struct Walk {
    int max_depth = -1;
    std::vector<uint8_t> level;
    char why[256] = "";
};
std::shared_future<Walk> start_walk(const UploadJob& j) {
    return std::async(std::launch::async, [&j] {
        Walk w;
        w.max_depth = validate_topology(j.host_child, j.d->capacity, j.N3, w.level, w.why, sizeof(w.why));
        j.mark("topology checked");
        return w;
    }).share();
}

struct Staged {
    hipError_t e = hipSuccess;
    DeviceBuffer child, data;
};
std::future<Staged> start_copies(const UploadJob& j, hipError_t e_dev, int device,
                                 std::shared_future<Walk> walk) {
    return std::async(std::launch::async, [&j, e_dev, device, walk] {
        Staged s;
        hipError_t& e = s.e;
        if ((e = e_dev) != hipSuccess) return s;
        e = hipSetDevice(device);
        if (j.from_host && e == hipSuccess) e = s.child.alloc(j.child_sz);
        if ((j.q || j.from_host) && e == hipSuccess) e = s.data.alloc(j.data_sz);
        if (j.from_host && e == hipSuccess) warm_upload_cache(device);
        j.mark("runtime + buffers ready");
        if (walk.get().max_depth < 0) return s;
        const CopySegment both[2] = {{s.child.get(), j.d->child, j.child_sz},
                                     {s.data.get(), j.d->data, j.data_sz}};
        if (j.q) {
            if (e == hipSuccess && j.from_host) e = staged_h2d_multi(both, 1, device);
            if (e == hipSuccess) e = decode_quant_on_device(j.d, j.q, j.n_slots, s.data.get<uint16_t>(), device);
        } else if (j.from_host && e == hipSuccess) {
            e = staged_h2d_multi(both, 2, device);
        }
        j.mark("copies done");
        return s;
    });
}

std::unique_ptr<VrTreeOpaque> new_tree(const UploadJob& j, int max_depth, int device, const Tuning& tn) {
    std::unique_ptr<VrTreeOpaque> t(new (std::nothrow) VrTreeOpaque());
    if (!t) return t;
    t->desc = *j.d;
    t->desc.child = nullptr;
    t->desc.data = nullptr;
    t->desc.extra = nullptr;
    t->max_depth = max_depth;
    t->device = device;
    t->tn = tn;
    t->leaf_stride_h = vr::leaf_stride_halfs(j.d->data_dim);
    return t;
}

hipError_t relayout(const UploadJob& j, const Staged& s, const std::vector<int32_t>& perm, VrTreeOpaque* t,
                    DeviceBuffer& d_perm) {
    const int32_t* src_child = j.from_host ? s.child.get<int32_t>() : j.d->child;
    const uint16_t* src_data = (j.q || j.from_host) ? s.data.get<uint16_t>() : j.d->data;
    const size_t leaves_sz = j.n_slots * (size_t)t->leaf_stride_h * sizeof(uint16_t);
    DeviceBuffer& nodes = t->arrays[kNodes];
    hipError_t e = nodes.alloc(j.child_sz);
    if (e == hipSuccess) e = t->arrays[kLeaves].alloc(leaves_sz);
    if (e == hipSuccess) e = alloc_launch_scratch(t);
    if (e == hipSuccess) e = d_perm.alloc(perm.size() * sizeof(int32_t));
    if (e == hipSuccess)
        e = hipMemcpy(d_perm.get(), perm.data(), perm.size() * sizeof(int32_t), hipMemcpyHostToDevice);
    if (e == hipSuccess)
        e = vr::launch_relayout(src_child, src_data, d_perm.get<int32_t>(), nodes.get<uint32_t>(),
                                t->arrays[kLeaves].get<uint16_t>(), (int64_t)j.n_slots, j.N3, j.d->data_dim,
                                t->leaf_stride_h, nullptr);
    t->device_bytes = j.child_sz + leaves_sz + sizeof(uint32_t);
    return e;
}

hipError_t build_lookup(const LookupPlan& plan, const std::vector<int32_t>& brick_roots, VrTreeOpaque* t,
                        DeviceBuffer& d_roots, uint32_t& flag) {
    const int G0 = plan.G0, BL = plan.BL;
    const size_t top_sz = ((size_t)1 << (3 * G0)) * sizeof(uint2);
    const int n_bricks = BL > 0 ? (int)brick_roots.size() : 0;
    const size_t brick_sz = ((size_t)n_bricks << (3 * BL)) * sizeof(uint32_t);
    hipError_t e = t->arrays[kTop].alloc(top_sz);
    if (e == hipSuccess && n_bricks) e = t->arrays[kBricks].alloc(brick_sz);
    if (e == hipSuccess && n_bricks) e = d_roots.alloc(n_bricks * sizeof(int32_t));
    if (e == hipSuccess && n_bricks)
        e = hipMemcpy(d_roots.get(), brick_roots.data(), n_bricks * sizeof(int32_t), hipMemcpyHostToDevice);
    const int blocked = (n_bricks && BL == 3)
                            ? (t->tn.brick_blocked >= 0 ? t->tn.brick_blocked
                                                        : (top_sz + brick_sz > (128ull << 20)))
                            : 0;
    if (e == hipSuccess)
        e = vr::launch_build_lookup(t->arrays[kNodes].get<uint32_t>(), d_roots.get<int32_t>(), n_bricks,
                                    t->arrays[kTop].get<uint2>(), t->arrays[kBricks].get<uint32_t>(),
                                    G0, BL, blocked, t->status.get<uint32_t>(), nullptr);
    if (e == hipSuccess) e = hipMemcpy(&flag, t->status.get(), sizeof(flag), hipMemcpyDeviceToHost);
    if (e == hipSuccess && flag == 0) {
        t->top_levels = G0;
        t->brick_levels = n_bricks ? BL : 0;
        t->brick_blocked = blocked;
        t->n_bricks = n_bricks;
        t->brick_root.assign(brick_roots.begin(), brick_roots.begin() + n_bricks);
        t->device_bytes += top_sz + brick_sz;
    }
    return e;
}

hipError_t build_occupancy(VrTreeOpaque* t) {
    if (t->top_levels <= 0) return hipSuccess;
    const int deepest = t->max_depth + 1;
    t->occ_levels = deepest < vr::kOccMaxLevels ? deepest : vr::kOccMaxLevels;
    const size_t bytes = vr::occ_words(t->occ_levels) * sizeof(uint32_t);
    hipError_t e = t->occ.alloc(bytes);
    if (e == hipSuccess) e = refresh_occupancy(t, nullptr);
    t->device_bytes += bytes;
    return e;
}

hipError_t upload_extra(const UploadJob& j, VrTreeOpaque* t) {
    if (!j.d->extra || !j.d->extra_count) return hipSuccess;
    const size_t esz = (size_t)j.d->extra_count * sizeof(float);
    hipError_t e = t->extra.alloc(esz);
    if (e == hipSuccess)
        e = hipMemcpy(t->extra.get(), j.d->extra, esz,
                      j.from_host ? hipMemcpyHostToDevice : hipMemcpyDeviceToDevice);
    t->device_bytes += esz;
    return e;
}

int upload_steps(const UploadJob& j, vr_tree_t* out) {
    std::shared_future<Walk> walk = start_walk(j);
    int device = 0;
    const hipError_t e_dev = hipGetDevice(&device);
    j.mark("HIP runtime up");
    std::future<void> prefault = std::async(std::launch::async, [&j] {
        if (j.from_host && !j.q) prefault_host_range(j.d->data, j.data_sz);
    });
    std::future<Staged> copies = start_copies(j, e_dev, device, walk);

    const Walk& w = walk.get();
    if (w.max_depth < 0) return fail(VR_ERR_BAD_TREE, "bad tree: %s", w.why);
    if (e_dev != hipSuccess)
        return fail(VR_ERR_HIP, "hipGetDevice failed: %s", hipGetErrorString(e_dev));
    const Tuning tn = default_tuning();
    const LookupPlan plan =
        plan_lookup(j.d->N, w.max_depth, j.d->capacity, tn.top_levels, tn.brick_levels, [&w](int l) {
            return (uint64_t)std::count(w.level.begin(), w.level.end(), (uint8_t)l);
        });
    std::unique_ptr<VrTreeOpaque> t = new_tree(j, w.max_depth, device, tn);
    if (!t) return fail(VR_ERR_OUT_OF_MEMORY, "host allocation failed");
    std::vector<int32_t> brick_roots;
    const std::vector<int32_t> perm =
        node_permutation(j.host_child, j.d->capacity, j.N3, plan.G0, plan.BL, w.level, brick_roots);
    t->file_node = inverse_permutation(perm);
    j.mark("host walks done");

    const Staged staged = copies.get();
    DeviceBuffer d_perm, d_roots;
    hipError_t e = staged.e;
    if (e == hipSuccess) e = relayout(j, staged, perm, t.get(), d_perm);
    uint32_t flag = 0;
    if (e == hipSuccess && plan.G0 > 0) e = build_lookup(plan, brick_roots, t.get(), d_roots, flag);
    if (e == hipSuccess && flag != 0)
        return fail(VR_ERR_BAD_TREE, "lookup structure build failed (flag %u)", flag);
    if (e == hipSuccess) e = build_occupancy(t.get());
    if (e == hipSuccess) e = hipDeviceSynchronize();
    if (e == hipSuccess) e = upload_extra(j, t.get());
    if (e != hipSuccess) return fail(hip_code(e), "tree upload failed: %s", hipGetErrorString(e));
    j.mark("device-ready");
    *out = t.release();
    return VR_OK;
}

int upload_body(const VrTreeDesc* d, const VrQuantDesc* q, vr_tree_t* out) {
    if (int rc = check_upload_args(d, q, out)) return rc;
    const int N3 = d->N * d->N * d->N;
    const size_t n_slots = (size_t)d->capacity * N3;
    UploadJob j{d, q, d->child, N3, n_slots, n_slots * sizeof(int32_t),
                n_slots * (size_t)d->data_dim * sizeof(uint16_t), d->memory != 1,
                getenv("VR_UPLOAD_TIMING") != nullptr, std::chrono::steady_clock::now()};
    std::vector<int32_t> fetched;
    if (int rc = fetch_child_words(j, fetched)) return rc;
    return upload_steps(j, out);
}

int upload_impl(const VrTreeDesc* d, const VrQuantDesc* q, vr_tree_t* out) {
    try {
        return upload_body(d, q, out);
    } catch (const std::bad_alloc&) {
        if (out) *out = nullptr;
        return fail(VR_ERR_OUT_OF_MEMORY, "tree upload: host allocation failed");
    } catch (const std::exception& e) {
        if (out) *out = nullptr;
        return fail(VR_ERR_OUT_OF_MEMORY, "tree upload: %s", e.what());
    }
}

}

hipError_t refresh_occupancy(const VrTreeOpaque* t, hipStream_t hs) {
    if (!t->occ) return hipSuccess;
    return vr::launch_build_occupancy(t->arrays[kNodes].get<uint32_t>(), t->occ_levels, t->occ.get<uint32_t>(), hs);
}

extern "C" {

int vr_tree_upload(const VrTreeDesc* d, vr_tree_t* out) { return upload_impl(d, nullptr, out); }

int vr_tree_upload_quantized(const VrTreeDesc* d, const VrQuantDesc* q, vr_tree_t* out) {
    if (!q) return fail(VR_ERR_INVALID_ARGUMENT, "quant desc is NULL");
    return upload_impl(d, q, out);
}

int vr_decode_quantized(const VrTreeDesc* d, const VrQuantDesc* q, uint16_t* data_out) {
    if (!d || !q || !data_out) return fail(VR_ERR_INVALID_ARGUMENT, "NULL argument");
    if (d->N < 2 || d->N > 16 || d->capacity <= 0 || d->data_dim < 1)
        return fail(VR_ERR_INVALID_ARGUMENT, "bad N / capacity / data_dim");
    if (int rc = check_quant(d, q)) return rc;
    const size_t n_slots = (size_t)d->capacity * d->N * d->N * d->N;
    const size_t data_sz = n_slots * (size_t)d->data_dim * sizeof(uint16_t);
    DeviceBuffer staging;
    hipError_t e = hipSuccess;
    if (d->memory != 1) e = staging.alloc(data_sz);
    uint16_t* d_data = d->memory != 1 ? staging.get<uint16_t>() : data_out;
    int device = 0;
    if (e == hipSuccess) e = hipGetDevice(&device);
    if (e == hipSuccess) e = decode_quant_on_device(d, q, n_slots, d_data, device);
    if (e == hipSuccess && d->memory != 1)
        e = hipMemcpy(data_out, d_data, data_sz, hipMemcpyDeviceToHost);
    if (e != hipSuccess) return fail(hip_code(e), "quantised decode failed: %s", hipGetErrorString(e));
    return VR_OK;
}

int vr_tree_clone(vr_tree_t src, int device, vr_tree_t* out) {
    if (!src || !out) return fail(VR_ERR_INVALID_ARGUMENT, "tree/out is NULL");
    *out = nullptr;
    int n_dev = 0;
    HIP_TRY(hipGetDeviceCount(&n_dev));
    if (device < 0 || device >= n_dev)
        return fail(VR_ERR_INVALID_ARGUMENT, "device %d outside [0,%d)", device, n_dev);
    std::lock_guard<std::mutex> src_lock(src->launch_mutex);
    {
        DeviceGuard g(src->device);
        HIP_TRY(hipDeviceSynchronize());
    }
    DeviceGuard guard(device);
    std::unique_ptr<VrTreeOpaque> t(new (std::nothrow) VrTreeOpaque());
    if (!t) return fail(VR_ERR_OUT_OF_MEMORY, "host allocation failed");
    static_cast<TreeShape&>(*t) = *src;
    t->device = device;
    t->tn = src->tn;
    t->file_node = src->file_node;
    t->brick_root = src->brick_root;
    t->device_bytes -= src->file_node_dev.bytes() + src->brick_root_dev.bytes() + src->node_of_file_dev.bytes();
    bool p2p = true;
    if (src->device != device) {
        int can = 0;
        if (hipDeviceCanAccessPeer(&can, device, src->device) != hipSuccess) can = 0;
        p2p = can != 0;
        if (p2p) {
            const hipError_t pe = hipDeviceEnablePeerAccess(src->device, 0);
            if (pe != hipSuccess && pe != hipErrorPeerAccessAlreadyEnabled) p2p = false;
        }
        (void)hipGetLastError();
    }
    auto copy = [&](DeviceBuffer& to, const DeviceBuffer& from) {
        if (!from) return hipSuccess;
        const hipError_t e = to.alloc(from.bytes());
        return e != hipSuccess ? e : hipMemcpyPeer(to.get(), device, from.get(), src->device, from.bytes());
    };
    hipError_t e = hipSuccess;
    for (int i = 0; i < 4 && e == hipSuccess; ++i) e = copy(t->arrays[i], src->arrays[i]);
    if (e == hipSuccess) e = copy(t->extra, src->extra);
    if (e == hipSuccess) e = copy(t->occ, src->occ);
    if (e == hipSuccess) e = alloc_launch_scratch(t.get());
    if (e == hipSuccess) e = hipDeviceSynchronize();
    if (e != hipSuccess)
        return fail(hip_code(e), "tree clone from device %d to device %d failed: %s%s", src->device, device,
                    hipGetErrorString(e),
                    p2p ? "" : " (the devices have NO peer access: check `rocm-smi --showtopo`, "
                               "IOMMU / ACS settings and HSA_ENABLE_IPC_MODE_LEGACY=0)");
    if (!p2p)
        fprintf(stderr, "[volrend_hip] note: devices %d and %d have no peer access; the clone was "
                        "staged through host memory\n", src->device, device);
    *out = t.release();
    return VR_OK;
}

int vr_tree_free(vr_tree_t t) {
    delete t;
    return VR_OK;
}

}
```

Measured before the change: 2855 Mrays/s.

## March empty lead-in space inside the raygen kernel before ray compaction

Adds a head march to the raygen kernel. While at least a minimum number of wave lanes are still active, each freshly set-up ray takes up to a fixed number of cheap lookup-only samples, advancing through empty space until it hits density above the threshold or leaves the volume. Rays that exit during this phase are finished in raygen and never written to the compacted ray buffer, so the main march kernel gets fewer rays, and the rays it does get start later along their path. The path is on by default only for N=2 colour frame renders with lookup arrays at or below 128 MB, and it also lowers the default raygen waves to 4. It adds device counters for rays entered, rays retired and samples taken, plus a stats API. The cost is a heavier, more divergent raygen kernel and extra atomics.

```diff
diff --git a/include/volrend_hip.h b/include/volrend_hip.h
--- a/include/volrend_hip.h
+++ b/include/volrend_hip.h
@@ -247,6 +247,7 @@
 int vr_tree_set_tuning(vr_tree_t tree, const char* key, int value);
 int vr_sched_stats(vr_tree_t tree, uint64_t out[8], int reset);
 int vr_tree_cull_stats(vr_tree_t tree, uint64_t out[2], int reset);
+int vr_tree_head_stats(vr_tree_t tree, uint64_t out[3], int reset);
 int vr_touch_enable(vr_tree_t tree, int enable);
 int vr_touch_count(vr_tree_t tree, uint64_t out[4], int reset);
 int vr_touch_read(vr_tree_t tree, int which, uint32_t* host_words, uint64_t n_words,
diff --git a/volrend_amd/_abi.py b/volrend_amd/_abi.py
--- a/volrend_amd/_abi.py
+++ b/volrend_amd/_abi.py
@@ -184,6 +184,7 @@
     "vr_tree_set_tuning": (C.c_int, [C.c_void_p, C.c_char_p, C.c_int]),
     "vr_sched_stats": (C.c_int, [C.c_void_p, C.POINTER(C.c_uint64 * 8), C.c_int]),
     "vr_tree_cull_stats": (C.c_int, [C.c_void_p, C.POINTER(C.c_uint64 * 2), C.c_int]),
+    "vr_tree_head_stats": (C.c_int, [C.c_void_p, C.POINTER(C.c_uint64 * 3), C.c_int]),
     "vr_touch_enable": (C.c_int, [C.c_void_p, C.c_int]),
     "vr_touch_count": (C.c_int, [C.c_void_p, C.POINTER(C.c_uint64 * 4), C.c_int]),
     "vr_touch_read": (C.c_int, [C.c_void_p, C.c_int, C.c_void_p, C.c_uint64, C.POINTER(C.c_uint64),
diff --git a/volrend_amd/_tree.py b/volrend_amd/_tree.py
--- a/volrend_amd/_tree.py
+++ b/volrend_amd/_tree.py
@@ -252,6 +252,11 @@
         _abi.check(_abi.lib().vr_tree_cull_stats(self.handle, C.byref(out), 1 if reset else 0))
         return {"blocks": int(out[0]), "culled": int(out[1])}
 
+    def head_stats(self, reset: bool = False) -> dict:
+        out = (C.c_uint64 * 3)()
+        _abi.check(_abi.lib().vr_tree_head_stats(self.handle, C.byref(out), 1 if reset else 0))
+        return {"entered": int(out[0]), "retired": int(out[1]), "samples": int(out[2])}
+
     def touch_enable(self, enable: bool = True) -> None:
         _abi.check(_abi.lib().vr_touch_enable(self.handle, 1 if enable else 0))
 
diff --git a/volrend_amd/csrc/vr_api.cpp b/volrend_amd/csrc/vr_api.cpp
--- a/volrend_amd/csrc/vr_api.cpp
+++ b/volrend_amd/csrc/vr_api.cpp
@@ -33,6 +33,9 @@
     {"max_iter", "VR_MAX_ITER", &Tuning::max_iter, kClamp, 1, INT_MAX, false},
     {"weights_check", "VR_WEIGHTS_CHECK", &Tuning::weights_check, kFlag, 0, 0, false},
     {"block_cull", "VR_BLOCK_CULL", &Tuning::block_cull, kFlag, 0, 0, false},
+    {"head_march", "VR_HEAD_MARCH", &Tuning::head_march, kFlag, 0, 0, false},
+    {"head_min_lanes", "VR_HEAD_MIN_LANES", &Tuning::head_min_lanes, kClamp, 0, 64, false},
+    {"head_max", "VR_HEAD_MAX", &Tuning::head_max, kClamp, 0, INT_MAX, false},
 };
 
 const Knob* find_knob(const char* key) {
@@ -219,6 +222,19 @@
     return VR_OK;
 }
 
+int vr_tree_head_stats(vr_tree_t t, uint64_t out[3], int reset) {
+    if (!t || !out) return fail(VR_ERR_INVALID_ARGUMENT, "NULL argument");
+    DeviceGuard guard(t->device);
+    uint64_t lines[vr::kCullStatLines * vr::kCullStatStride];
+    HIP_TRY(hipMemcpy(lines, t->head_stats.get(), sizeof(lines), hipMemcpyDeviceToHost));
+    if (reset) HIP_TRY(hipMemset(t->head_stats.get(), 0, sizeof(lines)));
+    for (int k = 0; k < vr::kHeadStatWords; ++k) {
+        out[k] = 0;
+        for (int i = 0; i < vr::kCullStatLines; ++i) out[k] += lines[i * vr::kCullStatStride + k];
+    }
+    return VR_OK;
+}
+
 int vr_tree_status(vr_tree_t t, uint32_t* status, int reset) {
     if (!t || !status) return fail(VR_ERR_INVALID_ARGUMENT, "NULL argument");
     DeviceGuard guard(t->device);
diff --git a/volrend_amd/csrc/vr_dev_march.h b/volrend_amd/csrc/vr_dev_march.h
--- a/volrend_amd/csrc/vr_dev_march.h
+++ b/volrend_amd/csrc/vr_dev_march.h
@@ -187,6 +187,31 @@
     return leaf;
 }
 
+template <int FMA, int QUERY>
+__device__ __forceinline__ uint32_t head_march(const KParams& p, const HeadParams& head, Ray& nr) {
+    Cursor cur;
+    bool go = nr.alive;
+    uint32_t samples = 0;
+    for (int r = 0; r < head.max_rounds; ++r) {
+        const unsigned long long m_go = __builtin_amdgcn_ballot_w64(go);
+        if (__builtin_popcountll(m_go) < head.min_lanes) break;
+        bool stepped = false;
+        if (go) {
+            float delta_t, sigma;
+            march_sample<FMA, QUERY>(p, nr.t, nr.cen, nr.dir, nr.invdir, cur, delta_t, sigma);
+            if (sigma > p.sigma_thresh) {
+                go = false;
+            } else {
+                nr.t += delta_t;
+                stepped = true;
+                if (!(nr.t < nr.tmax)) go = nr.alive = false;
+            }
+        }
+        samples += (uint32_t)__builtin_popcountll(__builtin_amdgcn_ballot_w64(stepped));
+    }
+    return samples;
+}
+
 __device__ __forceinline__ float sample_weight(float light, float delta_t, float delta_scale, float sigma, float& att) {
     att = vr_expf_nonan(-delta_t * delta_scale * sigma);
     return light * (1.f - att);
diff --git a/volrend_amd/csrc/vr_host.h b/volrend_amd/csrc/vr_host.h
--- a/volrend_amd/csrc/vr_host.h
+++ b/volrend_amd/csrc/vr_host.h
@@ -55,6 +55,7 @@
     DeviceBuffer extra, status, sched_stats;
     DeviceBuffer occ;
     DeviceBuffer cull_stats;
+    DeviceBuffer head_stats;
     DeviceBuffer touch[4];
     DeviceBuffer touch_out;
     DeviceBuffer probe_buf;
diff --git a/volrend_amd/csrc/vr_internal.h b/volrend_amd/csrc/vr_internal.h
--- a/volrend_amd/csrc/vr_internal.h
+++ b/volrend_amd/csrc/vr_internal.h
@@ -190,6 +190,12 @@
     uint32_t nbx;
     unsigned long long* stats;
 };
+constexpr int kHeadStatWords = 3;
+struct HeadParams {
+    int32_t max_rounds;
+    int32_t min_lanes;
+    unsigned long long* stats;
+};
 struct MaskParams {
     uint32_t* mask;
     uint32_t words_per_frame, nbx, nby;
@@ -283,12 +289,12 @@
 hipError_t launch_step_values(const StepArgs& a, int n_cus, hipStream_t stream);
 
 hipError_t launch_prepare_aov(const AovParams& a, const AovTable& tbl, hipStream_t stream);
-hipError_t launch_render_aov(const KParams& p, const AovParams& a, const CullParams& cull, int fp_mode, int n_cus,
-                             int waves_override, int gen_waves, hipStream_t stream);
+hipError_t launch_render_aov(const KParams& p, const AovParams& a, const CullParams& cull, const HeadParams& head,
+                             int fp_mode, int n_cus, int waves_override, int gen_waves, hipStream_t stream);
 hipError_t launch_prepare(const KParams& p, const FrameTable& tbl, hipStream_t stream, uint32_t* mask = nullptr,
                           uint32_t words_per_frame = 0);
-hipError_t launch_render(const KParams& p, const CullParams& cull, int fp_mode, int n_cus, int waves_override,
-                         int gen_waves, hipStream_t stream, const RayList* rays = nullptr);
+hipError_t launch_render(const KParams& p, const CullParams& cull, const HeadParams& head, int fp_mode, int n_cus,
+                         int waves_override, int gen_waves, hipStream_t stream, const RayList* rays = nullptr);
 hipError_t launch_probe(const KParams& p, const float probe[3], float* out_dev,
                         hipStream_t stream);
 
diff --git a/volrend_amd/csrc/vr_launch.cpp b/volrend_amd/csrc/vr_launch.cpp
--- a/volrend_amd/csrc/vr_launch.cpp
+++ b/volrend_amd/csrc/vr_launch.cpp
@@ -233,7 +233,12 @@
 }
 bool needs_file_order(LaunchKind kind) { return kind == LaunchKind::kWeights || kind == LaunchKind::kBackward; }
 
-struct Turn { const vr::KParams& k; const Tuning& tn; int gen_waves; unsigned slot; hipStream_t hs; void* extra; };
+bool lead_in_applies(const VrTreeOpaque* t, const vr::KParams& k) {
+    return t->desc.N == 2 && t->top_levels > 0 && t->desc.format != VR_FORMAT_SG && t->desc.format != VR_FORMAT_ASG &&
+           !k.instrumented && !k.render_depth;
+}
+
+struct Turn { const vr::KParams& k; const Tuning& tn; const LaunchPlan& plan; int gen_waves; unsigned slot; hipStream_t hs; void* extra; };
 
 template <typename Enqueue>
 int run_launch(VrTreeOpaque* t, LaunchKind kind, const Views& v, size_t extra_bytes, vr::KParams& k, void* stream,
@@ -246,7 +251,7 @@
     if (k.n_frames == 0) return VR_OK;
     const Tuning tn = t->tn;
     const LaunchPlan plan = plan_launch(kind, v.is_list ? RaySource::kList : RaySource::kFrames, k.n_frames, v.list.n,
-                                        tn, t->arrays[kTop].bytes() + t->arrays[kBricks].bytes());
+                                        tn, t->arrays[kTop].bytes() + t->arrays[kBricks].bytes(), lead_in_applies(t, k));
     fill_tuning_params(k, t, tn, plan);
     const size_t records = ray_buffer_bytes(k.total_rays, record_words(kind, k.ray_tail_words));
     unsigned slot;
@@ -255,7 +260,7 @@
     SlotTurn turn;
     if (int rc = turn.begin(t->slots[slot], hs)) return rc;
     void* const extra = extra_bytes ? t->slots[slot].rays.get<char>() + records : nullptr;
-    return enqueue(Turn{k, tn, plan.raygen_waves, slot, hs, extra});
+    return enqueue(Turn{k, tn, plan, plan.raygen_waves, slot, hs, extra});
 }
 
 int validate_aov(int n_frames, const VrCamera* cams, const VrRenderOptions* opt, const VrFrame* frames,
@@ -326,6 +331,11 @@
     return block_mask_words(k) <= (uint32_t)vr::kMaskMaxWords;
 }
 
+vr::HeadParams head_params(const VrTreeOpaque* t, const vr::KParams& k, const LaunchPlan& plan) {
+    if (plan.head_max <= 0 || !vr::uses_lookup(k) || vr::needs_full(k)) return vr::HeadParams{};
+    return vr::HeadParams{plan.head_max, plan.head_min_lanes, t->head_stats.get<unsigned long long>()};
+}
+
 int render_launch(vr_tree_t t, int n_frames, const VrCamera* cams, const VrRenderOptions* opt,
                   const VrFrame* frames, const VrAov* aovs, int depth_units, bool want_aov, void* stream) {
     vr::KParams k;
@@ -357,10 +367,11 @@
         }
         if (int rc = enqueue_tables(u.k, v, u.hs, frames, want_aov ? aovs : nullptr, a, m)) return rc;
         if (m.mask) HIP_TRY(vr::launch_block_mask(u.k, m, u.hs));
+        const vr::HeadParams head = head_params(t, u.k, u.plan);
         if (want_aov)
-            HIP_TRY(vr::launch_render_aov(u.k, a, cull, frames[0].fp_mode, t->n_cus, u.tn.waves_per_cu, u.gen_waves, u.hs));
+            HIP_TRY(vr::launch_render_aov(u.k, a, cull, head, frames[0].fp_mode, t->n_cus, u.tn.waves_per_cu, u.gen_waves, u.hs));
         else
-            HIP_TRY(vr::launch_render(u.k, cull, frames[0].fp_mode, t->n_cus, u.tn.waves_per_cu, u.gen_waves, u.hs));
+            HIP_TRY(vr::launch_render(u.k, cull, head, frames[0].fp_mode, t->n_cus, u.tn.waves_per_cu, u.gen_waves, u.hs));
         return VR_OK;
     });
 }
@@ -584,7 +595,7 @@
     return run_launch(t, LaunchKind::kColour, v, pixel_bytes, k, stream, [&](const Turn& u) -> int {
         f.rgba = out->rgba ? out->rgba : u.extra;
         if (int rc = enqueue_tables(u.k, v, u.hs, &f)) return rc;
-        HIP_TRY(vr::launch_render(u.k, vr::CullParams{}, fp_mode, t->n_cus, u.tn.waves_per_cu, u.gen_waves, u.hs, v.rays()));
+        HIP_TRY(vr::launch_render(u.k, vr::CullParams{}, vr::HeadParams{}, fp_mode, t->n_cus, u.tn.waves_per_cu, u.gen_waves, u.hs, v.rays()));
         return VR_OK;
     });
 }
diff --git a/volrend_amd/csrc/vr_launch_plan.cpp b/volrend_amd/csrc/vr_launch_plan.cpp
--- a/volrend_amd/csrc/vr_launch_plan.cpp
+++ b/volrend_amd/csrc/vr_launch_plan.cpp
@@ -3,9 +3,11 @@
 namespace {
 
 constexpr int kColourChunkCap = 256, kGuidedChunkCap = 4096;
+constexpr uint64_t kBigLookup = 128ull << 20;
+constexpr int kAutoHeadMinLanes = 32, kAutoHeadMax = 32;
 
-int raygen_waves(const Tuning& tn, int n_frames) {
-    return tn.raygen_waves > 0 ? tn.raygen_waves : (n_frames <= 2 ? 4 : 16);
+int raygen_waves(const Tuning& tn, int n_frames, bool head) {
+    return tn.raygen_waves > 0 ? tn.raygen_waves : (head || n_frames <= 2 ? 4 : 16);
 }
 constexpr int64_t kRayListSmall = 2 * 800 * 800;
 int raygen_waves_list(const Tuning& tn, int64_t n) {
@@ -15,14 +17,18 @@
 }
 
 LaunchPlan plan_launch(LaunchKind kind, RaySource source, int n_frames, int64_t list_rays, const Tuning& tn,
-                       uint64_t lookup_bytes) {
+                       uint64_t lookup_bytes, bool lead_in) {
     const bool colour = kind == LaunchKind::kColour || kind == LaunchKind::kAov;
     const bool list = source == RaySource::kList;
     LaunchPlan p;
     p.chunk_max = tn.chunk_max > 0 ? tn.chunk_max : colour ? kColourChunkCap : kGuidedChunkCap;
     p.super_block = tn.super_block > 0 ? tn.super_block : (colour && !list && n_frames > 2) ? 4 : 1;
-    p.raygen_waves = list ? raygen_waves_list(tn, list_rays) : raygen_waves(tn, n_frames);
-    p.records_nt = tn.records_nt >= 0 ? tn.records_nt : lookup_bytes > (128ull << 20);
+    const bool head = lead_in && tn.head_march && colour && !list && tn.max_iter >= Tuning().max_iter &&
+                      (tn.head_max > 0 || lookup_bytes <= kBigLookup);
+    p.head_max = !head ? 0 : tn.head_max > 0 ? tn.head_max : kAutoHeadMax;
+    p.head_min_lanes = tn.head_min_lanes > 0 ? tn.head_min_lanes : kAutoHeadMinLanes;
+    p.raygen_waves = list ? raygen_waves_list(tn, list_rays) : raygen_waves(tn, n_frames, head);
+    p.records_nt = tn.records_nt >= 0 ? tn.records_nt : lookup_bytes > kBigLookup;
     p.frame_group = tn.frame_group < 1 || tn.frame_group > n_frames ? n_frames : tn.frame_group;
     p.n_queues = tn.xcd_queues ? kPlanQueues : 1;
     return p;
diff --git a/volrend_amd/csrc/vr_launch_plan.h b/volrend_amd/csrc/vr_launch_plan.h
--- a/volrend_amd/csrc/vr_launch_plan.h
+++ b/volrend_amd/csrc/vr_launch_plan.h
@@ -20,6 +20,9 @@
     int max_iter = 1 << 22;
     int weights_check = 1;
     int block_cull = 1;
+    int head_march = 1;
+    int head_min_lanes = 0;
+    int head_max = 0;
 };
 
 enum class LaunchKind { kColour, kAov, kWeights, kBackward };
@@ -30,9 +33,10 @@
 struct LaunchPlan {
     int chunk_max, super_block, records_nt, frame_group, n_queues;
     int raygen_waves;
+    int head_max, head_min_lanes;
 };
 
 LaunchPlan plan_launch(LaunchKind kind, RaySource source, int n_frames, int64_t list_rays, const Tuning& tn,
-                       uint64_t lookup_bytes);
+                       uint64_t lookup_bytes, bool lead_in = false);
 
 #pragma GCC visibility pop
diff --git a/volrend_amd/csrc/vr_render.hip b/volrend_amd/csrc/vr_render.hip
--- a/volrend_amd/csrc/vr_render.hip
+++ b/volrend_amd/csrc/vr_render.hip
@@ -4,6 +4,7 @@
 #include "vr_dev_shade.h"
 #include "vr_dev_query.h"
 #include "vr_dev_rays.h"
+#include "vr_dev_march.h"
 
 namespace vr {
 
@@ -491,9 +492,10 @@
 
 
 
-template <int FMA, bool FULL, int GW, typename... PLANES>
+template <int FMA, bool FULL, int GW, bool HEAD, typename... PLANES>
 __global__ __launch_bounds__(kWave* GW)
-void raygen_kernel(const KParams p, const PLANES... planes, const CullParams cull) {
+void raygen_kernel(const KParams p, const PLANES... planes, const CullParams cull, const HeadParams head) {
+    static_assert(!(HEAD && FULL), "the FULL flavours count every sample in the march kernel");
     constexpr bool AOV = sizeof...(PLANES) != 0;
     const AovParams aov = aov_arg(planes...);
     const int lane = threadIdx.x & (kWave - 1);
@@ -507,6 +509,17 @@
     uint32_t xy = 0;
     int frame = 0;
     float vdir[3] = {0.f, 0.f, 1.f};
+    auto keep_or_finish = [&]() {
+        if (nr.alive) {
+            valid = true;
+        } else {
+            RayCounters z;
+            finish_ray<FMA, FULL>(p, nr, z, px, xy, frame);
+            if constexpr (AOV) store_aov(aov, frame, xy, 0.f, 1.f);
+        }
+    };
+    bool has = false;
+    if constexpr (HEAD) nr.alive = false;
     if (id < p.total_rays) {
         const PixelRef r = locate(p, id);
         if constexpr (!FULL) {
@@ -522,19 +535,27 @@
             px = pixel_ptr(p, p.frames[r.frame], r);
             if (culled) reset_ray(nr);
             else setup_ray<FMA>(p, r, nr, vdir);
-            if (nr.alive) {
-                valid = true;
-            } else {
-                RayCounters z;
-                finish_ray<FMA, FULL>(p, nr, z, px, xy, frame);
-                if constexpr (AOV) store_aov(aov, frame, xy, 0.f, 1.f);
-            }
-        }
+            if constexpr (HEAD) has = true;
+            else keep_or_finish();
+        }
+    }
+    uint32_t head_n[kHeadStatWords] = {0u, 0u, 0u};
+    if constexpr (HEAD) {
+        head_n[0] = (uint32_t)__builtin_popcountll(__builtin_amdgcn_ballot_w64(nr.alive));
+        if (head_n[0] != 0u)
+            head_n[2] = p.brick_blocked ? head_march<FMA, kQueryN2Blocked>(p, head, nr)
+                                        : head_march<FMA, kQueryN2>(p, head, nr);
+        head_n[1] = head_n[0] - (uint32_t)__builtin_popcountll(__builtin_amdgcn_ballot_w64(nr.alive));
+        if (has) keep_or_finish();
     }
     const unsigned long long m_valid = __builtin_amdgcn_ballot_w64(valid);
     __shared__ uint32_t wave_culled[GW];
+    __shared__ uint32_t wave_head[HEAD ? GW : 1][kHeadStatWords];
     if constexpr (!FULL && GW > 1) {
         if (cull.mask && lane == 0) wave_culled[wave] = culled ? 1u : 0u;
+        if constexpr (HEAD) {
+            if (lane < kHeadStatWords) wave_head[wave][lane] = lane == 0 ? head_n[0] : lane == 1 ? head_n[1] : head_n[2];
+        }
     }
     const uint32_t my_base = reserve_ray_slots<GW>(p, m_valid, lane, wave);
     if constexpr (!FULL) {
@@ -552,6 +573,20 @@
             }
             if (n)
                 atomicAdd(cull.stats + (blockIdx.x & (uint32_t)(kCullStatLines - 1)) * kCullStatStride + threadIdx.x,
+                          (unsigned long long)n);
+        }
+    }
+    if constexpr (HEAD) {
+        if (threadIdx.x < (uint32_t)kHeadStatWords) {
+            uint32_t n = 0;
+            if constexpr (GW > 1) {
+#pragma unroll
+                for (int w = 0; w < GW; ++w) n += wave_head[w][threadIdx.x];
+            } else {
+                n = threadIdx.x == 0u ? head_n[0] : threadIdx.x == 1u ? head_n[1] : head_n[2];
+            }
+            if (n)
+                atomicAdd(head.stats + (blockIdx.x & (uint32_t)(kCullStatLines - 1)) * kCullStatStride + threadIdx.x,
                           (unsigned long long)n);
         }
     }
@@ -812,8 +847,9 @@
 }
 
 template <typename... PLANES>
-hipError_t launch_march(const KParams& p, const CullParams& cull, int fp_mode, int n_cus, int waves_override,
-                        int gen_waves, hipStream_t stream, const RayList* rays, const PLANES&... planes) {
+hipError_t launch_march(const KParams& p, const CullParams& cull, const HeadParams& head, int fp_mode, int n_cus,
+                        int waves_override, int gen_waves, hipStream_t stream, const RayList* rays,
+                        const PLANES&... planes) {
     const int64_t total_blocks = p.n_wave_blocks * p.n_frames;
     {
         const bool full = needs_full(p);
@@ -824,7 +860,9 @@
             if constexpr (sizeof...(PLANES) == 0 && GW_ >= 4)                                       \
                 hipLaunchKernelGGL((raygen_rays_kernel<FMA_, FULL_, GW_>), grid_, block_, 0, stream, p, *rays); \
         }                                                                                           \
-        else hipLaunchKernelGGL((raygen_kernel<FMA_, FULL_, GW_, PLANES...>), grid_, block_, 0, stream, p, planes..., cull); \
+        else if (!FULL_ && head.max_rounds > 0)                                                     \
+            hipLaunchKernelGGL((raygen_kernel<FMA_, FULL_, GW_, !FULL_, PLANES...>), grid_, block_, 0, stream, p, planes..., cull, head); \
+        else hipLaunchKernelGGL((raygen_kernel<FMA_, FULL_, GW_, false, PLANES...>), grid_, block_, 0, stream, p, planes..., cull, head); \
     } while (0)
 #define VR_GEN_GW(FMA_, FULL_)                                                                      \
     do {                                                                                            \
@@ -860,10 +898,10 @@
     return hipGetLastError();
 }
 
-hipError_t launch_render(const KParams& p, const CullParams& cull, int fp_mode, int n_cus, int waves_override,
-                         int gen_waves, hipStream_t stream, const RayList* rays) {
+hipError_t launch_render(const KParams& p, const CullParams& cull, const HeadParams& head, int fp_mode, int n_cus,
+                         int waves_override, int gen_waves, hipStream_t stream, const RayList* rays) {
     if (p.n_wave_blocks <= 0 || p.n_frames <= 0) return hipSuccess;
-    const hipError_t e = launch_march(p, cull, fp_mode, n_cus, waves_override, gen_waves, stream, rays);
+    const hipError_t e = launch_march(p, cull, head, fp_mode, n_cus, waves_override, gen_waves, stream, rays);
     if (e != hipSuccess || !p.enable_probe || p.probe_disp_size <= 0) return e;
     const int side = p.probe_disp_size + 5;
     const dim3 pgrid((unsigned)((side * side + 255) / 256), (unsigned)p.n_frames);
@@ -879,10 +917,10 @@
     return hipGetLastError();
 }
 
-hipError_t launch_render_aov(const KParams& p, const AovParams& a, const CullParams& cull, int fp_mode, int n_cus,
-                             int waves_override, int gen_waves, hipStream_t stream) {
+hipError_t launch_render_aov(const KParams& p, const AovParams& a, const CullParams& cull, const HeadParams& head,
+                             int fp_mode, int n_cus, int waves_override, int gen_waves, hipStream_t stream) {
     if (p.n_wave_blocks <= 0 || p.n_frames <= 0) return hipSuccess;
-    return launch_march(p, cull, fp_mode, n_cus, waves_override, gen_waves, stream,  nullptr, a);
+    return launch_march(p, cull, head, fp_mode, n_cus, waves_override, gen_waves, stream,  nullptr, a);
 }
 
 hipError_t launch_probe(const KParams& p, const float probe[3], float* out_dev,
diff --git a/volrend_amd/csrc/vr_upload.cpp b/volrend_amd/csrc/vr_upload.cpp
--- a/volrend_amd/csrc/vr_upload.cpp
+++ b/volrend_amd/csrc/vr_upload.cpp
@@ -89,6 +89,8 @@
     const size_t cull_sz = (size_t)vr::kCullStatLines * vr::kCullStatStride * sizeof(unsigned long long);
     if (e == hipSuccess) e = t->cull_stats.alloc(cull_sz);
     if (e == hipSuccess) e = hipMemset(t->cull_stats.get(), 0, cull_sz);
+    if (e == hipSuccess) e = t->head_stats.alloc(cull_sz);
+    if (e == hipSuccess) e = hipMemset(t->head_stats.get(), 0, cull_sz);
     if (e == hipSuccess) e = t->probe_buf.alloc(sizeof(float) * (size_t)t->desc.data_dim * kLaunchSlots);
     for (unsigned i = 0; i < kLaunchSlots && e == hipSuccess; ++i) e = t->slots[i].done.create();
     if (e == hipSuccess) e = t->slot_frames.alloc(sizeof(vr::FrameDesc) * vr::kMaxBatch * kLaunchSlots);
```

Measured after the change: 2992 Mrays/s, median of 6. 1.05x the previous value.
